# m1el/nemotron-speech.cpp

Measured on NVIDIA B200. Metric: rtfx, higher is better.
Workload: dtype bf16

## Files before the change

include/nsb200.h:

```cpp
#ifndef NSB200_H
#define NSB200_H

#include <stddef.h>
#include <stdint.h>

#ifdef __cplusplus
extern "C" {
#endif

#define NSB_OK 0
#define NSB_ERR_ARG (-1)
#define NSB_ERR_IO (-2)
#define NSB_ERR_FORMAT (-3)
#define NSB_ERR_CUDA (-4)
#define NSB_ERR_STATE (-5)
#define NSB_ERR_NOMEM (-6)

enum nsb_compute {
    NSB_COMPUTE_AUTO = 0,
    NSB_COMPUTE_F32 = 1,
    NSB_COMPUTE_F16 = 2,
    NSB_COMPUTE_BF16 = 3,
    NSB_COMPUTE_Q8_0 = 4,
    NSB_COMPUTE_Q8_0_STRICT = 5
// ... 22 lines not shown
} nsb_stats;

typedef struct nsb_model_info {
    int32_t n_mels, d_model, n_heads, d_head, d_ff, n_layers, kernel_size, vocab_size, decoder_dim, joint_dim;
    int32_t n_tensors;
    int32_t weight_type;
    char vocab[1025 * 8];
} nsb_model_info;
int nsb_gguf_probe(const char* gguf_path, nsb_model_info* info);
long long nsb_gguf_read_tensor(const char* gguf_path, const char* tensor_name, float* out, size_t cap_floats, int* ggml_type);

void nsb_default_config(nsb_engine_config* cfg);
int nsb_engine_create(const char* gguf_path, const nsb_engine_config* cfg, nsb_engine** out);
void nsb_engine_destroy(nsb_engine* e);
const char* nsb_last_error(void);

int nsb_engine_n_layers(const nsb_engine* e);
int nsb_engine_vocab_size(const nsb_engine* e);
const char* nsb_engine_vocab(const nsb_engine* e);
int nsb_engine_chunk_samples(const nsb_engine* e);
int nsb_engine_shift_samples(const nsb_engine* e);
int nsb_engine_compute(const nsb_engine* e);
int nsb_engine_set_cuda_graph(nsb_engine* e, int on);

int nsb_stream_open(nsb_engine* e);
int nsb_stream_close(nsb_engine* e, int stream);
int nsb_stream_reset(nsb_engine* e, int stream);

int nsb_stream_push_pcm(nsb_engine* e, int stream, const int16_t* pcm, int n_samples);
int nsb_push_pcm_batch(nsb_engine* e, int n_streams, const int32_t* streams, const int16_t* pcm, int row_stride, int n_samples);
int nsb_pop_tokens_batch(nsb_engine* e, int n_streams, const int32_t* streams, int32_t* out, int cap_per_stream, int32_t* counts);
int nsb_stream_ready(const nsb_engine* e, int stream);
int nsb_engine_step(nsb_engine* e);
int nsb_engine_step_begin(nsb_engine* e);
int nsb_engine_step_end(nsb_engine* e);
int nsb_engine_drain(nsb_engine* e);
int nsb_stream_pop_tokens(nsb_engine* e, int stream, int32_t* out, int cap);
int nsb_stream_chunks(const nsb_engine* e, int stream);

int nsb_detokenize(const nsb_engine* e, const int32_t* tokens, int n, char* out, int cap);

void nsb_engine_get_stats(const nsb_engine* e, nsb_stats* out);

int nsb_bench_prepare(nsb_engine* e, int n_streams, const int16_t* pcm, int samples_per_stream, int warm_chunks);
int nsb_bench_step(nsb_engine* e, float* ms);
int nsb_bench_steps(nsb_engine* e, int n, float* ms_each, float* total_ms);
#define NSB_PROFILE_CLASSES 8
int nsb_bench_profile(nsb_engine* e, float* ms_per_class, int* launches_per_class, float* total_ms);

int nsb_bench_gemm(nsb_engine* e, int kind, int rows, int bn, int stages, int splits, int rotate, int iters, float* us);

typedef struct nsb_trace_record { uint64_t t[6]; int32_t tag; int32_t grid; } nsb_trace_record;
int nsb_trace_enable(nsb_engine* e, int capacity);
int nsb_trace_fetch(nsb_engine* e, nsb_trace_record* out, int cap);

int nsb_profiler_range(int on);

int nsb_debug_enable(nsb_engine* e, int on);
int nsb_debug_get(nsb_engine* e, const char* name, float* out, size_t cap_floats);
int nsb_debug_get_cache(nsb_engine* e, int stream, int which , int layer, float* out, size_t cap);

int nsb_op_logmel(nsb_engine* e, const int16_t* pcm, int n_streams, int n_samples, float* mel_out, size_t cap_floats);
int nsb_op_gemm(nsb_engine* e, const char* weight_name, const float* x, int rows, float* y, size_t cap_floats);

enum nsb_epi { NSB_EPI_NONE = 0, NSB_EPI_RELU = 1, NSB_EPI_SILU = 2, NSB_EPI_RESID = 3, NSB_EPI_PARTIAL = 4 };
enum nsb_out_type { NSB_OUT_F32 = 0, NSB_OUT_F16 = 1, NSB_OUT_BF16 = 2 };
typedef struct nsb_gemm_op {
    const char* weight;
    int32_t rows;
    int32_t epi;
    float alpha;
    int32_t out_type;
    int32_t splits;
    int32_t c0;
    int32_t c_group, c_drop;
    int32_t force_bn, force_stages;
    int32_t rotate;
    const float* bias;
    const float* c_init;
} nsb_gemm_op;
int nsb_op_gemm_ex(nsb_engine* e, const nsb_gemm_op* op, const float* x, void* y, size_t y_bytes, long long* guard_bad);
int nsb_op_layernorm(nsb_engine* e, const float* x, int rows, const float* planes, int n_planes, float alpha, const float* g1, const float* b1,
                     const float* g2, const float* b2, int fused, int out_type, float* x_out, void* y);

int nsb_transcribe_full(nsb_engine* e, const int16_t* pcm, int n_samples, int32_t* tokens, int32_t* token_frames, int cap, int* n_frames,
                        float* enc_out, size_t enc_cap_floats);

#ifdef __cplusplus
}
#endif
#endif
```

nemotron-speech.cpp_b200/__init__.py:

```python
from __future__ import annotations

import ctypes as C
import os
import subprocess

import numpy as np

_DIR = os.path.dirname(os.path.abspath(__file__))
LIB_PATH = os.path.join(_DIR, "libnsb200.so")

EPI_NONE, EPI_RELU, EPI_SILU, EPI_RESID, EPI_PARTIAL = 0, 1, 2, 3, 4
OUT_F32, OUT_F16, OUT_BF16 = 0, 1, 2
COMPUTE_AUTO, COMPUTE_F32, COMPUTE_F16, COMPUTE_BF16, COMPUTE_Q8_0, COMPUTE_Q8_0_STRICT = 0, 1, 2, 3, 4, 5
KV_F32, KV_F16, KV_BF16 = 0, 1, 2


class NsbError(RuntimeError):
    pass


class EngineConfig(C.Structure):
    _fields_ = [("device", C.c_int32), ("compute", C.c_int32), ("kv_dtype", C.c_int32), ("att_right_context", C.c_int32),
                ("max_streams", C.c_int32), ("use_cuda_graph", C.c_int32), ("decode_overlap", C.c_int32), ("reserved", C.c_int32 * 5)]


class Stats(C.Structure):
    _fields_ = [("steps", C.c_int64), ("chunks", C.c_int64), ("kernel_launches", C.c_int64), ("device_ms", C.c_double),
                ("last_step_ms", C.c_double)]


class TraceRecord(C.Structure):
    _fields_ = [("t", C.c_uint64 * 6), ("tag", C.c_int32), ("grid", C.c_int32)]


TRACE_TAGS = {1: "logmel", 2: "stem", 3: "dwconv", 4: "melhist", 5: "gemm_f32", 6: "gemm_tc", 7: "gemm_q8", 8: "ln", 9: "ln2", 10: "attn",
              11: "convmod", 12: "advance", 13: "decode", 14: "other"}


class GemmOp(C.Structure):
    _fields_ = [("weight", C.c_char_p), ("rows", C.c_int32), ("epi", C.c_int32), ("alpha", C.c_float), ("out_type", C.c_int32),
                ("splits", C.c_int32), ("c0", C.c_int32), ("c_group", C.c_int32), ("c_drop", C.c_int32), ("force_bn", C.c_int32),
                ("force_stages", C.c_int32), ("rotate", C.c_int32), ("bias", C.c_void_p), ("c_init", C.c_void_p)]


class ModelInfo(C.Structure):
    _fields_ = [(n, C.c_int32) for n in ("n_mels", "d_model", "n_heads", "d_head", "d_ff", "n_layers", "kernel_size", "vocab_size",
                                         "decoder_dim", "joint_dim", "n_tensors", "weight_type")] + [("vocab", C.c_char * (1025 * 8))]


EXPORTS = ["nsb_gguf_probe", "nsb_gguf_read_tensor", "nsb_default_config", "nsb_engine_create", "nsb_engine_destroy", "nsb_last_error", "nsb_engine_n_layers",
           "nsb_engine_vocab_size", "nsb_engine_vocab", "nsb_engine_chunk_samples", "nsb_engine_shift_samples", "nsb_engine_compute", "nsb_engine_set_cuda_graph",
           "nsb_stream_open", "nsb_stream_close", "nsb_stream_reset", "nsb_stream_push_pcm", "nsb_push_pcm_batch", "nsb_pop_tokens_batch", "nsb_stream_ready", "nsb_engine_step", "nsb_engine_step_begin", "nsb_engine_step_end",
           "nsb_engine_drain", "nsb_stream_pop_tokens", "nsb_stream_chunks", "nsb_detokenize", "nsb_engine_get_stats",
           "nsb_bench_prepare", "nsb_bench_step", "nsb_bench_steps", "nsb_bench_profile", "nsb_profiler_range", "nsb_bench_gemm", "nsb_trace_enable", "nsb_trace_fetch", "nsb_debug_enable", "nsb_debug_get", "nsb_debug_get_cache", "nsb_op_logmel",
           "nsb_op_gemm", "nsb_op_gemm_ex", "nsb_op_layernorm", "nsb_transcribe_full"]


def build(force: bool = False) -> str:
    if force or not os.path.exists(LIB_PATH):
        subprocess.check_call(["make", "-C", _DIR, "-j8", "all"], stdout=subprocess.DEVNULL)
    return LIB_PATH


_lib = None
_f32p = np.ctypeslib.ndpointer(dtype=np.float32, flags="C_CONTIGUOUS")
_i16p = np.ctypeslib.ndpointer(dtype=np.int16, flags="C_CONTIGUOUS")
_i32p = np.ctypeslib.ndpointer(dtype=np.int32, flags="C_CONTIGUOUS")


def lib():
    global _lib
    if _lib is None:
        if not os.path.exists(LIB_PATH):
            raise NsbError(f"{LIB_PATH} is missing: run __graft_entry__.build() (there is no fallback path)")
        L = C.CDLL(LIB_PATH)
        vp, ci = C.c_void_p, C.c_int
        L.nsb_last_error.restype = C.c_char_p
        L.nsb_gguf_probe.argtypes = [C.c_char_p, C.POINTER(ModelInfo)]
        L.nsb_gguf_read_tensor.argtypes = [C.c_char_p, C.c_char_p, C.c_void_p, C.c_size_t, C.POINTER(C.c_int)]
        L.nsb_gguf_read_tensor.restype = C.c_longlong
        L.nsb_default_config.argtypes = [C.POINTER(EngineConfig)]
        L.nsb_engine_create.argtypes = [C.c_char_p, C.POINTER(EngineConfig), C.POINTER(vp)]
        L.nsb_engine_destroy.argtypes = [vp]
        for n in ("nsb_engine_n_layers", "nsb_engine_vocab_size", "nsb_engine_chunk_samples", "nsb_engine_shift_samples",
                  "nsb_engine_compute", "nsb_stream_open", "nsb_engine_step", "nsb_engine_step_begin", "nsb_engine_step_end", "nsb_engine_drain"):
            getattr(L, n).argtypes = [vp]
        L.nsb_engine_vocab.argtypes = [vp]
        L.nsb_engine_set_cuda_graph.argtypes = [vp, ci]
        L.nsb_engine_vocab.restype = vp
        for n in ("nsb_stream_close", "nsb_stream_reset", "nsb_stream_ready", "nsb_stream_chunks"):
            getattr(L, n).argtypes = [vp, ci]
        L.nsb_stream_push_pcm.argtypes = [vp, ci, _i16p, ci]
        L.nsb_stream_pop_tokens.argtypes = [vp, ci, _i32p, ci]
        L.nsb_push_pcm_batch.argtypes = [vp, ci, _i32p, _i16p, ci, ci]
        L.nsb_pop_tokens_batch.argtypes = [vp, ci, _i32p, _i32p, ci, _i32p]
        L.nsb_detokenize.argtypes = [vp, _i32p, ci, C.c_char_p, ci]
        L.nsb_engine_get_stats.argtypes = [vp, C.POINTER(Stats)]
        L.nsb_bench_prepare.argtypes = [vp, ci, _i16p, ci, ci]
        L.nsb_bench_step.argtypes = [vp, C.POINTER(C.c_float)]
        L.nsb_bench_steps.argtypes = [vp, ci, C.POINTER(C.c_float), C.POINTER(C.c_float)]
        L.nsb_bench_profile.argtypes = [vp, C.POINTER(C.c_float), C.POINTER(C.c_int), C.POINTER(C.c_float)]
        L.nsb_profiler_range.argtypes = [ci]
        L.nsb_trace_enable.argtypes = [vp, ci]
        L.nsb_trace_fetch.argtypes = [vp, C.POINTER(TraceRecord), ci]
        L.nsb_bench_gemm.argtypes = [vp, ci, ci, ci, ci, ci, ci, ci, C.POINTER(C.c_float)]
        L.nsb_debug_enable.argtypes = [vp, ci]
        L.nsb_debug_get.argtypes = [vp, C.c_char_p, _f32p, C.c_size_t]
        L.nsb_debug_get_cache.argtypes = [vp, ci, ci, ci, _f32p, C.c_size_t]
        L.nsb_op_logmel.argtypes = [vp, _i16p, ci, ci, _f32p, C.c_size_t]
        L.nsb_op_gemm.argtypes = [vp, C.c_char_p, _f32p, ci, _f32p, C.c_size_t]
        L.nsb_op_gemm_ex.argtypes = [vp, C.POINTER(GemmOp), _f32p, vp, C.c_size_t, C.POINTER(C.c_longlong)]
        L.nsb_op_layernorm.argtypes = [vp, _f32p, ci, vp, ci, C.c_float, _f32p, _f32p, vp, vp, ci, ci, _f32p, vp]
        L.nsb_transcribe_full.argtypes = [vp, _i16p, ci, _i32p, _i32p, ci, C.POINTER(C.c_int), C.c_void_p, C.c_size_t]
        _lib = L
    return _lib


def _check(rc: int) -> int:
    if rc < 0:
        raise NsbError(f"nsb error {rc}: {lib().nsb_last_error().decode(errors='replace')}")
    return rc


def probe(path: str) -> ModelInfo:
    info = ModelInfo()
    _check(lib().nsb_gguf_probe(path.encode(), C.byref(info)))
    return info


def read_tensor(path: str, name: str):
    t = C.c_int(0)
    n = _check(int(lib().nsb_gguf_read_tensor(path.encode(), name.encode(), None, 0, C.byref(t))))
    out = np.empty(n, dtype=np.float32)
    _check(int(lib().nsb_gguf_read_tensor(path.encode(), name.encode(), out.ctypes.data_as(C.c_void_p), out.size, C.byref(t))))
    return out, t.value


class Engine:

    def __init__(self, gguf_path: str, right_context: int = 0, max_streams: int = 1, compute: int = COMPUTE_AUTO,
                 kv_dtype: int = KV_F32, device: int = 0, cuda_graph: bool = True, decode_overlap: int = 0):
        cfg = EngineConfig()
        lib().nsb_default_config(C.byref(cfg))
        cfg.device, cfg.compute, cfg.kv_dtype = device, compute, kv_dtype
        cfg.att_right_context, cfg.max_streams = right_context, max_streams
        cfg.use_cuda_graph = 1 if cuda_graph else 0
        cfg.decode_overlap = decode_overlap
        h = C.c_void_p()
        _check(lib().nsb_engine_create(gguf_path.encode(), C.byref(cfg), C.byref(h)))
        self.h = h
        self.T = 1 + right_context
        self.max_streams = max_streams
        self.n_layers = lib().nsb_engine_n_layers(h)
        self.chunk_samples = lib().nsb_engine_chunk_samples(h)
        self.shift_samples = lib().nsb_engine_shift_samples(h)
        self.compute = lib().nsb_engine_compute(h)

    def close(self):
        if getattr(self, "h", None):
            lib().nsb_engine_destroy(self.h)
            self.h = None

    __del__ = close

    def set_cuda_graph(self, on: bool):
        _check(lib().nsb_engine_set_cuda_graph(self.h, 1 if on else 0))

    def open_stream(self) -> int:
        return _check(lib().nsb_stream_open(self.h))

    def close_stream(self, s: int):
        _check(lib().nsb_stream_close(self.h, s))

    def reset_stream(self, s: int):
        _check(lib().nsb_stream_reset(self.h, s))

    def push(self, s: int, pcm: np.ndarray):
        pcm = np.ascontiguousarray(pcm, dtype=np.int16)
        if len(pcm):
            _check(lib().nsb_stream_push_pcm(self.h, s, pcm, len(pcm)))

    def push_batch(self, streams, pcm: np.ndarray):
        ids = np.ascontiguousarray(streams, dtype=np.int32)
        pcm = np.ascontiguousarray(pcm, dtype=np.int16)
        assert pcm.ndim == 2 and pcm.shape[0] == len(ids)
        if pcm.shape[1]:
            _check(lib().nsb_push_pcm_batch(self.h, len(ids), ids, pcm.reshape(-1), pcm.shape[1], pcm.shape[1]))

    def pop_tokens_batch(self, streams, cap_per_stream: int = 256):
        ids = np.ascontiguousarray(streams, dtype=np.int32)
        out = np.empty((len(ids), cap_per_stream), dtype=np.int32)
        cnt = np.empty(len(ids), dtype=np.int32)
        _check(lib().nsb_pop_tokens_batch(self.h, len(ids), ids, out.reshape(-1), cap_per_stream, cnt))
        return out, cnt

# ... 69 lines not shown

    def trace_fetch(self, cap: int = 4096):
        buf = (TraceRecord * cap)()
        n = _check(lib().nsb_trace_fetch(self.h, buf, cap))
        return [(TRACE_TAGS.get(buf[i].tag, str(buf[i].tag)), buf[i].grid, [int(x) for x in buf[i].t]) for i in range(n)]

    def debug_enable(self, on: bool = True):
        _check(lib().nsb_debug_enable(self.h, 1 if on else 0))

    def debug_get(self, name: str, B: int) -> np.ndarray:
        rows = self.max_streams * self.T
        if name == "mel":
            M = 9 + 8 * self.T
            buf = np.empty(self.max_streams * M * 128, dtype=np.float32)
            _check(lib().nsb_debug_get(self.h, name.encode(), buf, buf.size))
            return buf.reshape(self.max_streams, M, 128)[:B].copy()
        if name == "logits":
            buf = np.empty((11 * self.T) * 1025, dtype=np.float32)
            n = _check(lib().nsb_debug_get(self.h, name.encode(), buf, buf.size))
            return buf[:n].reshape(-1, 1025).copy()
        buf = np.empty(rows * 1024, dtype=np.float32)
        _check(lib().nsb_debug_get(self.h, name.encode(), buf, buf.size))
        return buf.reshape(rows, 1024)[: B * self.T].copy()

    def debug_cache(self, stream: int, which: int, layer: int) -> np.ndarray:
        rows = 70 if which < 2 else 8
        buf = np.empty(rows * 1024, dtype=np.float32)
        _check(lib().nsb_debug_get_cache(self.h, stream, which, layer, buf, buf.size))
        return buf.reshape(rows, 1024)

    def op_logmel(self, pcm: np.ndarray) -> np.ndarray:
        pcm = np.ascontiguousarray(pcm, dtype=np.int16)
        if pcm.ndim == 1:
            pcm = pcm[None]
        ns, n = pcm.shape
        nf = (256 + n - 512 + 160) // 160 if 256 + n >= 512 else 0
        out = np.empty((ns, max(nf, 1), 128), dtype=np.float32)
        got = _check(lib().nsb_op_logmel(self.h, pcm.reshape(-1), ns, n, out.reshape(-1), out.size))
        assert got == nf, (got, nf)
        return out[:, :nf]

    def op_gemm(self, weight_name: str, x: np.ndarray) -> np.ndarray:
        x = np.ascontiguousarray(x, dtype=np.float32)
        y = np.empty((x.shape[0], 4096), dtype=np.float32)
        n_out = _check(lib().nsb_op_gemm(self.h, weight_name.encode(), x, x.shape[0], y.reshape(-1), y.size))
        return y.reshape(-1)[: x.shape[0] * n_out].reshape(x.shape[0], n_out).copy()

    def op_gemm_ex(self, weight_name: str, x: np.ndarray, *, epi: int = EPI_NONE, alpha: float = 1.0, bias=None, out_type: int = OUT_F32,
                   splits: int = 1, c0: bool = False, c_group: int = 0, c_drop: int = 0, force_bn: int = 0, force_stages: int = 0,
                   rotate: int = 1, c_init=None):
        x = np.ascontiguousarray(x, dtype=np.float32)
        rows = x.shape[0]
        m_out = rows // c_group * (c_group - c_drop) if c_group else rows
        keep = []
        def ptr(a):
            if a is None:
                return None
            a = np.ascontiguousarray(a, dtype=np.float32); keep.append(a)
            return a.ctypes.data_as(C.c_void_p)
        op = GemmOp(weight_name.encode(), rows, epi, alpha, out_type, splits, int(c0), c_group, c_drop, force_bn, force_stages, rotate,
                    ptr(bias), ptr(c_init))
        n_cap = 4096
        shape = (splits, m_out, n_cap) if epi == EPI_PARTIAL else (m_out, n_cap)
        y = np.empty(shape, dtype=np.float32 if out_type == OUT_F32 else np.uint16)
        bad = C.c_longlong(-1)
        n = _check(lib().nsb_op_gemm_ex(self.h, C.byref(op), x, y.ctypes.data_as(C.c_void_p), y.nbytes, C.byref(bad)))
        y = y.reshape(-1)[: int(np.prod(shape[:-1])) * n].reshape(shape[:-1] + (n,)).copy()
        return y, bad.value

    def op_layernorm(self, x: np.ndarray, g1, b1, *, planes=None, alpha: float = 1.0, fused: bool = False, g2=None, b2=None,
                     out_type: int = OUT_F32):
        x = np.ascontiguousarray(x, dtype=np.float32)
        rows = x.shape[0]
        f = lambda a: None if a is None else np.ascontiguousarray(a, dtype=np.float32)
        planes, g1, b1, g2, b2 = f(planes), f(g1), f(b1), f(g2), f(b2)
        vp = lambda a: None if a is None else a.ctypes.data_as(C.c_void_p)
        x_out = np.empty_like(x)
        y = np.zeros((rows, 1024), dtype=np.float32 if out_type == OUT_F32 else np.uint16)
        n_planes = 0 if planes is None else planes.shape[0]
        _check(lib().nsb_op_layernorm(self.h, x, rows, vp(planes), n_planes, alpha, g1, b1, vp(g2), vp(b2), int(fused), out_type, x_out,
                                      y.ctypes.data_as(C.c_void_p)))
        return x_out, y

    def transcribe_full(self, pcm: np.ndarray, want_enc: bool = True, want_frames: bool = False):
        pcm = np.ascontiguousarray(pcm, dtype=np.int16)
        frames_cap = len(pcm) // 1280 + 8
        toks = np.empty(10 * frames_cap, dtype=np.int32)
        frm = np.empty(10 * frames_cap, dtype=np.int32)
        enc = np.empty((frames_cap, 1024), dtype=np.float32) if want_enc else None
        nf = C.c_int(0)
        n = _check(lib().nsb_transcribe_full(self.h, pcm, len(pcm), toks, frm, len(toks), C.byref(nf),
                                             enc.ctypes.data_as(C.c_void_p) if want_enc else None, enc.size if want_enc else 0))
        out = (toks[:n].copy(), (enc[:nf.value].copy() if want_enc else None))
        return out + (frm[:n].copy(),) if want_frames else out
```

nemotron-speech.cpp_b200/csrc/c_api.cu:

```cuda
#include <algorithm>
#include <cstring>
#include <string>

#include <cuda_profiler_api.h>

#include "engine.h"

using nsb::Engine;

struct nsb_engine { Engine* impl; };

static thread_local std::string g_err;
static int fail(int code, const std::string& msg) { g_err = msg; return code; }

#define NSB_TRY try {
#define NSB_CATCH                                                                         \
    } catch (const nsb::CudaError& e) { return fail(NSB_ERR_CUDA, e.what());              \
    } catch (const std::invalid_argument& e) { return fail(NSB_ERR_ARG, e.what());        \
    } catch (const std::bad_alloc&) { return fail(NSB_ERR_NOMEM, "out of host memory");   \
    } catch (const std::exception& e) { return fail(NSB_ERR_STATE, e.what()); }

extern "C" {

const char* nsb_last_error(void) { return g_err.c_str(); }
// ... 66 lines not shown

int nsb_engine_n_layers(const nsb_engine* e) { return e ? e->impl->n_layers : NSB_ERR_ARG; }
int nsb_engine_vocab_size(const nsb_engine* e) { return e ? nsb::VOCAB : NSB_ERR_ARG; }
const char* nsb_engine_vocab(const nsb_engine* e) { return e ? e->impl->vocab.data() : nullptr; }
int nsb_engine_chunk_samples(const nsb_engine* e) { return e ? e->impl->chunk_samples() : NSB_ERR_ARG; }
int nsb_engine_shift_samples(const nsb_engine* e) { return e ? e->impl->shift_samples() : NSB_ERR_ARG; }
int nsb_engine_compute(const nsb_engine* e) { return e ? e->impl->compute : NSB_ERR_ARG; }

int nsb_engine_set_cuda_graph(nsb_engine* e, int on) { if (!e) return fail(NSB_ERR_ARG, "null engine"); NSB_TRY e->impl->set_cuda_graph(on != 0); return NSB_OK; NSB_CATCH }

int nsb_stream_open(nsb_engine* e) { if (!e) return fail(NSB_ERR_ARG, "null engine"); NSB_TRY return e->impl->open_stream(); NSB_CATCH }
int nsb_stream_close(nsb_engine* e, int s) { if (!e) return fail(NSB_ERR_ARG, "null engine"); NSB_TRY e->impl->close_stream(s); return NSB_OK; NSB_CATCH }
int nsb_stream_reset(nsb_engine* e, int s) { if (!e) return fail(NSB_ERR_ARG, "null engine"); NSB_TRY e->impl->reset_stream(s); return NSB_OK; NSB_CATCH }
int nsb_stream_push_pcm(nsb_engine* e, int s, const int16_t* pcm, int n) {
    if (!e) return fail(NSB_ERR_ARG, "null engine"); NSB_TRY e->impl->push_pcm(s, pcm, n); return NSB_OK; NSB_CATCH }
int nsb_push_pcm_batch(nsb_engine* e, int n_streams, const int32_t* streams, const int16_t* pcm, int row_stride, int n_samples) {
    if (!e || !streams || (!pcm && n_samples > 0) || n_streams < 0) return fail(NSB_ERR_ARG, "bad argument");
    NSB_TRY for (int i = 0; i < n_streams; ++i) e->impl->push_pcm(streams[i], pcm + (size_t)i * row_stride, n_samples); return NSB_OK; NSB_CATCH }
int nsb_pop_tokens_batch(nsb_engine* e, int n_streams, const int32_t* streams, int32_t* out, int cap_per_stream, int32_t* counts) {
    if (!e || !streams || !out || !counts || cap_per_stream < 0) return fail(NSB_ERR_ARG, "bad argument");
    NSB_TRY int total = 0;
    for (int i = 0; i < n_streams; ++i) { counts[i] = e->impl->pop_tokens(streams[i], out + (size_t)i * cap_per_stream, cap_per_stream); total += counts[i]; }
    return total; NSB_CATCH }
int nsb_stream_ready(const nsb_engine* e, int s) { if (!e || s < 0 || s >= e->impl->max_streams) return NSB_ERR_ARG; return e->impl->ready(s) ? 1 : 0; }
int nsb_engine_step(nsb_engine* e) { if (!e) return fail(NSB_ERR_ARG, "null engine"); NSB_TRY return e->impl->step(); NSB_CATCH }
int nsb_engine_step_begin(nsb_engine* e) { if (!e) return fail(NSB_ERR_ARG, "null engine"); NSB_TRY return e->impl->step_begin(); NSB_CATCH }
int nsb_engine_step_end(nsb_engine* e) { if (!e) return fail(NSB_ERR_ARG, "null engine"); NSB_TRY return e->impl->step_end(); NSB_CATCH }
int nsb_engine_drain(nsb_engine* e) {
    if (!e) return fail(NSB_ERR_ARG, "null engine");
    NSB_TRY int total = 0; for (;;) { int n = e->impl->step(); if (n <= 0) break; total += n; } return total; NSB_CATCH }
int nsb_stream_pop_tokens(nsb_engine* e, int s, int32_t* out, int cap) {
    if (!e || !out || cap < 0) return fail(NSB_ERR_ARG, "bad argument"); NSB_TRY return e->impl->pop_tokens(s, out, cap); NSB_CATCH }
int nsb_stream_chunks(const nsb_engine* e, int s) { if (!e) return NSB_ERR_ARG; NSB_TRY return e->impl->chunks(s); NSB_CATCH }

int nsb_detokenize(const nsb_engine* e, const int32_t* t, int n, char* out, int cap) {
    if (!e || (!t && n > 0) || !out) return fail(NSB_ERR_ARG, "bad argument");
    NSB_TRY const std::string r = e->impl->detok(t, n);
    if ((int)r.size() + 1 > cap) return -(int)r.size() - 1;
    memcpy(out, r.c_str(), r.size() + 1); return (int)r.size(); NSB_CATCH }

void nsb_engine_get_stats(const nsb_engine* e, nsb_stats* out) { if (e && out) *out = e->impl->stats; }

int nsb_bench_prepare(nsb_engine* e, int n, const int16_t* pcm, int sps, int warm) {
    if (!e || !pcm) return fail(NSB_ERR_ARG, "bad argument"); NSB_TRY e->impl->bench_prepare(n, pcm, sps, warm); return NSB_OK; NSB_CATCH }
int nsb_bench_step(nsb_engine* e, float* ms) {
    if (!e) return fail(NSB_ERR_ARG, "null engine"); NSB_TRY const float t = e->impl->bench_step(); if (ms) *ms = t; return NSB_OK; NSB_CATCH }

int nsb_bench_steps(nsb_engine* e, int n, float* ms_each, float* total_ms) {
    if (!e) return fail(NSB_ERR_ARG, "null engine"); NSB_TRY const float t = e->impl->bench_steps(n, ms_each); if (total_ms) *total_ms = t; return NSB_OK; NSB_CATCH }

int nsb_bench_profile(nsb_engine* e, float* ms_per_class, int* launches_per_class, float* total_ms) {
    if (!e || !ms_per_class || !launches_per_class) return fail(NSB_ERR_ARG, "bad argument");
    NSB_TRY const float t = e->impl->bench_profile(ms_per_class, launches_per_class); if (total_ms) *total_ms = t; return NSB_OK; NSB_CATCH }

int nsb_bench_gemm(nsb_engine* e, int kind, int rows, int bn, int stages, int splits, int rotate, int iters, float* us) {
    if (!e || !us) return fail(NSB_ERR_ARG, "bad argument"); NSB_TRY *us = e->impl->bench_gemm(kind, rows, bn, stages, splits, rotate, iters); return NSB_OK; NSB_CATCH }

int nsb_trace_enable(nsb_engine* e, int capacity) { if (!e) return fail(NSB_ERR_ARG, "null engine"); NSB_TRY e->impl->trace_enable(capacity); return NSB_OK; NSB_CATCH }
int nsb_trace_fetch(nsb_engine* e, nsb_trace_record* out, int cap) {
    if (!e || (!out && cap > 0)) return fail(NSB_ERR_ARG, "bad argument");
    static_assert(sizeof(nsb_trace_record) == sizeof(nsb::TraceRec), "trace record layout");
    NSB_TRY return e->impl->trace_fetch(reinterpret_cast<nsb::TraceRec*>(out), cap); NSB_CATCH }

int nsb_profiler_range(int on) { return (on ? cudaProfilerStart() : cudaProfilerStop()) == cudaSuccess ? NSB_OK : NSB_ERR_CUDA; }

int nsb_debug_enable(nsb_engine* e, int on) { if (!e) return fail(NSB_ERR_ARG, "null engine"); NSB_TRY e->impl->debug_enable(on != 0); return NSB_OK; NSB_CATCH }
int nsb_debug_get(nsb_engine* e, const char* name, float* out, size_t cap) {
    if (!e || !name || !out) return fail(NSB_ERR_ARG, "bad argument"); NSB_TRY return (int)e->impl->debug_get(name, out, cap); NSB_CATCH }
int nsb_debug_get_cache(nsb_engine* e, int s, int which, int layer, float* out, size_t cap) {
    if (!e || !out) return fail(NSB_ERR_ARG, "bad argument"); NSB_TRY return (int)e->impl->debug_get_cache(s, which, layer, out, cap); NSB_CATCH }

int nsb_op_logmel(nsb_engine* e, const int16_t* pcm, int ns, int n, float* out, size_t cap) {
    if (!e || !pcm || !out) return fail(NSB_ERR_ARG, "bad argument"); NSB_TRY return (int)e->impl->op_logmel(pcm, ns, n, out, cap); NSB_CATCH }
int nsb_op_gemm(nsb_engine* e, const char* name, const float* x, int rows, float* y, size_t cap) {
    if (!e || !name || !x || !y) return fail(NSB_ERR_ARG, "bad argument"); NSB_TRY return (int)e->impl->op_gemm(name, x, rows, y, cap); NSB_CATCH }

int nsb_op_gemm_ex(nsb_engine* e, const nsb_gemm_op* op, const float* x, void* y, size_t y_bytes, long long* guard_bad) {
    if (!e || !op || !op->weight || !x || !y) return fail(NSB_ERR_ARG, "bad argument");
    NSB_TRY return (int)e->impl->op_gemm_ex(*op, x, y, y_bytes, guard_bad); NSB_CATCH }
int nsb_op_layernorm(nsb_engine* e, const float* x, int rows, const float* planes, int n_planes, float alpha, const float* g1, const float* b1,
                     const float* g2, const float* b2, int fused, int out_type, float* x_out, void* y) {
    if (!e || !x || !x_out || !y) return fail(NSB_ERR_ARG, "bad argument");
    NSB_TRY e->impl->op_layernorm(x, rows, planes, n_planes, alpha, g1, b1, g2, b2, fused != 0, out_type, x_out, y); return NSB_OK; NSB_CATCH }

int nsb_transcribe_full(nsb_engine* e, const int16_t* pcm, int n, int32_t* tokens, int32_t* token_frames, int cap, int* n_frames, float* enc_out, size_t enc_cap) {
    if (!e || !pcm) return fail(NSB_ERR_ARG, "bad argument"); NSB_TRY return (int)e->impl->transcribe_full(pcm, n, tokens, token_frames, cap, n_frames, enc_out, enc_cap); NSB_CATCH }

}
```

nemotron-speech.cpp_b200/csrc/common.cuh:

```cuda
#pragma once
#include <cuda_bf16.h>
#include <cuda_fp16.h>
#include <cuda_runtime.h>

#include <atomic>
#include <cstdint>
#include <cstdio>
#include <stdexcept>
#include <string>
#include <utility>

namespace nsb {

constexpr int D_MODEL = 1024, D_FF = 4096, N_HEADS = 8, D_HEAD = 128;
constexpr int N_MELS = 128, N_FFT = 512, N_BINS = 257, HOP = 160, WIN = 400;
constexpr int ATT_L = 70;
constexpr int CONV_K = 9;
constexpr int PRE_CACHE = 9;
constexpr int DROP_PRE = 2;
constexpr int SUB_CH = 256, SUB_W = 17;
constexpr int HID = 640, JOINT = 640, VOCAB = 1025, BLANK = 1024;
constexpr int MAX_SYMBOLS = 10;

struct CudaError : std::runtime_error { using std::runtime_error::runtime_error; };

#define NSB_CUDA(expr)                                                                              \
    do {                                                                                            \
        cudaError_t _e = (expr);                                                                    \
        if (_e != cudaSuccess)                                                                      \
            throw ::nsb::CudaError(std::string(#expr) + ": " + cudaGetErrorString(_e) + " (" + __FILE__ + ":" + \
                                   std::to_string(__LINE__) + ")");                                 \
    } while (0)

__device__ __forceinline__ void pdl_wait() { asm volatile("griddepcontrol.wait;" ::: "memory"); }
__device__ __forceinline__ void pdl_trigger() { asm volatile("griddepcontrol.launch_dependents;" ::: "memory"); }

bool pdl_enabled();
inline bool& pdl_skip_flag() { static thread_local bool f = false; return f; }
inline void pdl_skip_next() { pdl_skip_flag() = true; }
inline bool pdl_take() { bool& f = pdl_skip_flag(); const bool on = pdl_enabled() && !f; f = false; return on; }

template <typename... P, typename... A>
inline void launch_k(void (*kern)(P...), dim3 grid, dim3 block, size_t smem, cudaStream_t st, A&&... args) {
    cudaLaunchConfig_t cfg{};
    cfg.gridDim = grid; cfg.blockDim = block; cfg.dynamicSmemBytes = smem; cfg.stream = st;
    cudaLaunchAttribute at[1];
    at[0].id = cudaLaunchAttributeProgrammaticStreamSerialization;
    at[0].val.programmaticStreamSerializationAllowed = 1;
    cfg.attrs = at; cfg.numAttrs = pdl_take() ? 1 : 0;
    NSB_CUDA(cudaLaunchKernelEx(&cfg, kern, P(std::forward<A>(args))...));
}

template <typename... P, typename... A>
inline void launch_k_cluster(void (*kern)(P...), dim3 grid, dim3 block, size_t smem, cudaStream_t st, int cluster_x, A&&... args) {
    cudaLaunchConfig_t cfg{};
    cfg.gridDim = grid; cfg.blockDim = block; cfg.dynamicSmemBytes = smem; cfg.stream = st;
    cudaLaunchAttribute at[2]; int n = 0;
    if (cluster_x > 1) { at[n].id = cudaLaunchAttributeClusterDimension; at[n].val.clusterDim.x = cluster_x; at[n].val.clusterDim.y = 1; at[n].val.clusterDim.z = 1; ++n; }
    if (pdl_take()) { at[n].id = cudaLaunchAttributeProgrammaticStreamSerialization; at[n].val.programmaticStreamSerializationAllowed = 1; ++n; }
    cfg.attrs = at; cfg.numAttrs = n;
    NSB_CUDA(cudaLaunchKernelEx(&cfg, kern, P(std::forward<A>(args))...));
}

constexpr int MAX_DEVICES = 64;
template <typename K>
inline void ensure_dyn_smem(K kern, size_t bytes, std::atomic<size_t>* slots, bool max_carveout = false) {
    int dev = 0;
    NSB_CUDA(cudaGetDevice(&dev));
    std::atomic<size_t>& done = slots[dev & (MAX_DEVICES - 1)];
    if (bytes <= done.load(std::memory_order_acquire)) return;
    NSB_CUDA(cudaFuncSetAttribute(kern, cudaFuncAttributeMaxDynamicSharedMemorySize, (int)bytes));
    if (max_carveout) NSB_CUDA(cudaFuncSetAttribute(kern, cudaFuncAttributePreferredSharedMemoryCarveout, (int)cudaSharedmemCarveoutMaxShared));
    done.store(bytes, std::memory_order_release);
}

struct TraceRec { unsigned long long t[6]; int tag; int grid; };
struct TraceBuf { unsigned n; unsigned cap; unsigned pad[2]; TraceRec rec[1]; };
enum TraceTag : int { TR_LOGMEL = 1, TR_STEM, TR_DWCONV, TR_MELHIST, TR_GEMM_SIMT, TR_GEMM_TC, TR_GEMM_Q8, TR_LN, TR_LN2, TR_ATTN, TR_CONVMOD, TR_ADVANCE, TR_DECODE, TR_OTHER };
static __constant__ TraceBuf* c_trace;
#define NSB_DEFINE_TRACE_BINDER(name) \
    void name(TraceBuf* p) { NSB_CUDA(cudaMemcpyToSymbol(c_trace, &p, sizeof(p))); }
__device__ __forceinline__ unsigned long long gtime() { unsigned long long t; asm volatile("mov.u64 %0, %%globaltimer;" : "=l"(t)); return t; }
__device__ __forceinline__ bool trace_thread() { return threadIdx.x == 0 && (blockIdx.x | blockIdx.y | blockIdx.z) == 0; }
__device__ __forceinline__ int trace_begin(int tag) {
    TraceBuf* tb = c_trace;
    if (!tb) return -1;
    const unsigned s = atomicAdd(&tb->n, 1u);
    if (s >= tb->cap) return -1;
    tb->rec[s].tag = tag; tb->rec[s].grid = (int)(gridDim.x * gridDim.y * gridDim.z); tb->rec[s].t[0] = gtime();
    return (int)s;
}
__device__ __forceinline__ void trace_mark(int slot, int i) { if (slot >= 0) c_trace->rec[slot].t[i] = gtime(); }
#define NSB_KERNEL_BEGIN(tag)                                      \
    int tr_slot = -1;                                              \
    if (trace_thread()) tr_slot = trace_begin(tag);
#define NSB_KERNEL_WAIT()                                          \
    pdl_wait(); pdl_trigger();                                     \
    if (tr_slot >= 0) trace_mark(tr_slot, 1);
#define NSB_KERNEL_PROLOGUE(tag) NSB_KERNEL_BEGIN(tag) NSB_KERNEL_WAIT()
#define NSB_KERNEL_EPILOGUE() do { if (tr_slot >= 0) trace_mark(tr_slot, 2); } while (0)

enum Epi : int {
    EPI_NONE = 0,
    EPI_RELU = 1,
    EPI_SILU = 2,
    EPI_RESID = 3,
    EPI_PARTIAL = 4
};
enum OutType : int { OUT_F32 = 0, OUT_F16 = 1, OUT_BF16 = 2 };

__device__ __forceinline__ float silu_f(float x) { return __fdividef(x, 1.0f + __expf(-x)); }
__device__ __forceinline__ float silu_exact(float x) { return x / (1.0f + expf(-x)); }
__device__ __forceinline__ float sigmoid_exact(float x) { return 1.0f / (1.0f + expf(-x)); }

__device__ __forceinline__ float warp_sum(float v) {
#pragma unroll
    for (int o = 16; o > 0; o >>= 1) v += __shfl_xor_sync(0xffffffffu, v, o);
    return v;
}
__device__ __forceinline__ float warp_max(float v) {
#pragma unroll
    for (int o = 16; o > 0; o >>= 1) v = fmaxf(v, __shfl_xor_sync(0xffffffffu, v, o));
    return v;
}

template <typename T> __device__ __forceinline__ T from_f32(float v);
template <> __device__ __forceinline__ float from_f32<float>(float v) { return v; }
template <> __device__ __forceinline__ __half from_f32<__half>(float v) { return __float2half_rn(v); }
template <> __device__ __forceinline__ __nv_bfloat16 from_f32<__nv_bfloat16>(float v) { return __float2bfloat16_rn(v); }
__device__ __forceinline__ float to_f32(float v) { return v; }
__device__ __forceinline__ float to_f32(__half v) { return __half2float(v); }
__device__ __forceinline__ float to_f32(__nv_bfloat16 v) { return __bfloat162float(v); }

__device__ __forceinline__ void store_out(void* p, size_t i, float v, int ot) {
    if (ot == OUT_F32) ((float*)p)[i] = v;
    else if (ot == OUT_F16) ((__half*)p)[i] = __float2half_rn(v);
    else ((__nv_bfloat16*)p)[i] = __float2bfloat16_rn(v);
}
__device__ __forceinline__ float load_kv(const void* p, size_t i, int kv) {
    if (kv == 0) return ((const float*)p)[i];
    if (kv == 1) return __half2float(((const __half*)p)[i]);
    return __bfloat162float(((const __nv_bfloat16*)p)[i]);
}
__device__ __forceinline__ float round_kv(float v, int kv) {
    if (kv == 0) return v;
    if (kv == 1) return __half2float(__float2half_rn(v));
    return __bfloat162float(__float2bfloat16_rn(v));
}
__device__ __forceinline__ void store_kv(void* p, size_t i, float v, int kv) {
    if (kv == 0) ((float*)p)[i] = v;
    else if (kv == 1) ((__half*)p)[i] = __float2half_rn(v);
    else ((__nv_bfloat16*)p)[i] = __float2bfloat16_rn(v);
}
__device__ __forceinline__ float to_tf32(float v) { uint32_t r; asm("cvt.rna.tf32.f32 %0, %1;" : "=r"(r) : "f"(v)); return __uint_as_float(r); }
__device__ __forceinline__ void split_tf32(float v, float& hi, float& lo) { hi = to_tf32(v); lo = to_tf32(v - hi); }
__device__ __forceinline__ void store_pixel(float* out, size_t pix, int c, float v, int split) {
    if (!split) { out[pix * 256 + c] = v; return; }
    float hi, lo; split_tf32(v, hi, lo);
    out[pix * 512 + c] = hi; out[pix * 512 + 256 + c] = lo;
}
inline size_t kv_elem_size(int kv) { return kv == 0 ? 4 : 2; }
// ... 4 lines not shown
```

nemotron-speech.cpp_b200/csrc/engine.cu:

```cuda
#include "engine.h"

#include <algorithm>
#include <cmath>
#include <cstddef>
#include <cstdlib>
#include <cstring>

namespace nsb {

void launch_gemm_tc(const GemmArgs& a, int in_type , cudaStream_t st);

constexpr int MAX_SPLITS = 8;
constexpr size_t SPLIT_CONSUMER_MAX_ROWS = 256;

bool tf32x3_enabled() {
    static const bool on = [] { const char* e = getenv("NSB_STEM_TF32"); return !(e && e[0] == '1'); }();
    return on;
}
bool pdl_enabled() {
    static const bool on = [] { const char* e = getenv("NSB_NO_PDL"); return !(e && e[0] == '1'); }();
    return on;
}

namespace {
// ... 348 lines not shown
        mat(L.ff1b, "feed_forward1.linear2.weight", D_MODEL, D_FF);
        mat(L.ff2a, "feed_forward2.linear1.weight", D_FF, D_MODEL);
        mat(L.ff2b, "feed_forward2.linear2.weight", D_MODEL, D_FF);
        load_layer_matrix(L.qkv, g, p + "self_attn.linear_qkv.weight",
                          {p + "self_attn.linear_q.weight", p + "self_attn.linear_k.weight", p + "self_attn.linear_v.weight"}, 3 * D_MODEL, D_MODEL);
        mat(L.out, "self_attn.linear_out.weight", D_MODEL, D_MODEL);
        mat(L.pw1, "conv.pointwise_conv1.weight", 2 * D_MODEL, D_MODEL);
        mat(L.pw2, "conv.pointwise_conv2.weight", D_MODEL, D_MODEL);
        vec(L.bias_u, p + "self_attn.pos_bias_u", D_MODEL); vec(L.bias_v, p + "self_attn.pos_bias_v", D_MODEL);
        {
            const GgufTensor& dw = g.require(p + "conv.depthwise_conv.weight");
            if (dw.ne.size() != 2 || dw.ne[0] != D_MODEL || dw.ne[1] != CONV_K)
                throw std::runtime_error("depthwise conv weight must be [1024, 9] (2-D, tap-major; reconvert old 3-D files)");
            vec(L.dw_w, p + "conv.depthwise_conv.weight", (size_t)CONV_K * D_MODEL);
        }
        vec(L.cln_g, p + "conv.batch_norm.weight", D_MODEL); vec(L.cln_b, p + "conv.batch_norm.bias", D_MODEL);
        for (Weight* w : {&L.ff1a, &L.ff1b, &L.ff2a, &L.ff2b, &L.qkv, &L.out, &L.pw1, &L.pw2}) named_[w->name] = w;
        { int k = 0; for (Weight* w : {&L.ff1a, &L.ff1b, &L.qkv, &L.out, &L.pw1, &L.pw2, &L.ff2a, &L.ff2b}) w->shadow_slot = k++; }
    }
    {
        const std::string d = "decoder.prediction.";
        vec(embed_, d + "embed.weight", (size_t)VOCAB * HID);
        for (int l = 0; l < 2; ++l) {
            vec(lstm_w_[2 * l], d + "dec_rnn.lstm.weight_ih_l" + std::to_string(l), (size_t)4 * HID * HID);
            vec(lstm_w_[2 * l + 1], d + "dec_rnn.lstm.weight_hh_l" + std::to_string(l), (size_t)4 * HID * HID);
            vec(lstm_b_[2 * l], d + "dec_rnn.lstm.bias_ih_l" + std::to_string(l), (size_t)4 * HID);
            vec(lstm_b_[2 * l + 1], d + "dec_rnn.lstm.bias_hh_l" + std::to_string(l), (size_t)4 * HID);
        }
        f32_weight(joint_enc_w_, "joint.enc.weight", JOINT, D_MODEL, g.read_f32("joint.enc.weight"));
        vec(joint_enc_b_, "joint.enc.bias", JOINT);
        vec(pred_w_, "joint.pred.weight", (size_t)JOINT * HID); vec(pred_b_, "joint.pred.bias", JOINT);
        vec(jout_w_, "joint.joint_net.2.weight", (size_t)VOCAB * JOINT); vec(jout_b_, "joint.joint_net.2.bias", VOCAB);
    }
}

int q8_dense_min_rows();
void Engine::alloc_state() {
    const int S = max_streams, Cap = ATT_L + T, M = PRE_CACHE + 8 * T;
    const int t1 = M / 2 + 1, t2 = t1 / 2 + 1, t3 = t2 / 2 + 1;
    if (t3 != T + DROP_PRE) throw std::runtime_error("unexpected subsampling length");
    const size_t SS = (size_t)S + 1;
    kv_.alloc(SS * n_layers * 2 * Cap * D_MODEL * kv_elem_size(kv_dtype));
    conv_cache_.alloc(SS * 2 * n_layers * (CONV_K - 1) * D_MODEL * 4); cc_par_.alloc(SS * 4);
    mel_hist_.alloc(SS * PRE_CACHE * N_MELS * 4);
    ring_pos_.alloc(SS * 4); valid_len_.alloc(SS * 4);
    dec_h_.alloc(SS * 4 * HID * 4); dec_c_.alloc(SS * 4 * HID * 4);
    dec_proj_.alloc(SS * JOINT * 4);
    prev_token_.alloc(SS * 4); cand_valid_.alloc(SS * 4); dec_par_.alloc(SS * 4);
    hs_.assign(S, HostStream());
    for (int s = 0; s <= S; ++s) zero_slot(s);

    rl_ = hs_row_len(T);
    const size_t Mrows = (size_t)S * T;
    ensure_q8s_scratch((int)std::max<size_t>(Mrows, ATT_L + 2 * T));
    for (StepIO& io : io_) io.d_pcm.alloc((size_t)S * rl_ * 2);
    d_slot_.alloc((size_t)S * 4);
    mel_new_.alloc((size_t)S * 8 * T * N_MELS * 4);
    const size_t sp = (!strict() && tf32x3_enabled()) ? 2 : 1;
    dw_.alloc(sp * S * t2 * 33 * SUB_CH * 4);
    pw_.alloc((size_t)S * t2 * 33 * SUB_CH * 4);
    if (sp == 2) a3_.alloc(std::max((size_t)S * t3 * SUB_W * SUB_CH, (size_t)S * T * D_MODEL) * 2 * 4, false);
    x_.alloc(Mrows * D_MODEL * 4);
    a_.alloc(Mrows * D_MODEL * act_size());
    big_.alloc(Mrows * D_FF * act_size());
    const size_t planes = Mrows <= SPLIT_CONSUMER_MAX_ROWS ? 4 : 1;
    consumer_planes_ = (int)planes;
    if (compute == NSB_COMPUTE_Q8_0) wscratch_.alloc((size_t)D_FF * D_MODEL * 2, false);
    if (compute == NSB_COMPUTE_Q8_0 && (int)Mrows >= q8_dense_min_rows()) {
        const size_t sz[8] = {(size_t)D_FF * D_MODEL, (size_t)D_MODEL * D_FF, (size_t)3 * D_MODEL * D_MODEL, (size_t)D_MODEL * D_MODEL,
                              (size_t)2 * D_MODEL * D_MODEL, (size_t)D_MODEL * D_MODEL, (size_t)D_FF * D_MODEL, (size_t)D_MODEL * D_FF};
        size_t off = 0; for (int k = 0; k < 8; ++k) { shadow_off_[k] = off; off += sz[k] * 2; }
        shadow_bytes_ = off;
        for (DevBuf& b : shadow_) b.alloc(off, false);
        NSB_CUDA(cudaStreamCreateWithFlags(&st_deq_, cudaStreamNonBlocking));
        ev_deq_.resize(n_layers); ev_lstart_.resize(n_layers + 1);
        for (cudaEvent_t& e : ev_deq_) NSB_CUDA(cudaEventCreateWithFlags(&e, cudaEventDisableTiming));
        for (cudaEvent_t& e : ev_lstart_) NSB_CUDA(cudaEventCreateWithFlags(&e, cudaEventDisableTiming));
    }
    qkv_.alloc(planes * Mrows * 3 * D_MODEL * 4);
    pw1_.alloc(planes * Mrows * 2 * D_MODEL * 4);
    encp_.alloc(Mrows * JOINT * 4);
    part_.alloc((size_t)MAX_SPLITS * std::min<size_t>(Mrows, 1024) * D_MODEL * 4);
    out_tok_.alloc((size_t)S * MAX_SYMBOLS * T * 4); out_cnt_.alloc((size_t)S * 4);
    dec_sync_.alloc(decode_sync_bytes(S));
    for (Side& sd : side_) {
        sd.slot.alloc((size_t)S * 4); sd.encp.alloc(Mrows * JOINT * 4); sd.out_tok.alloc((size_t)S * MAX_SYMBOLS * T * 4);
        sd.out_cnt.alloc((size_t)S * 4); sd.sync.alloc(decode_sync_bytes(S));
    }
    for (StepIO& io : io_) {
        io.h_pcm.alloc((size_t)S * rl_ * 2); io.h_slot.alloc((size_t)S * 4);
        io.h_tok.alloc((size_t)S * MAX_SYMBOLS * T * 4); io.h_cnt.alloc((size_t)S * 4);
    }
}

void Engine::zero_slot(int s) {
    NSB_CUDA(cudaSetDevice(device_));
    join_decode_stream();
    const int Cap = ATT_L + T;
    const size_t kvb = (size_t)n_layers * 2 * Cap * D_MODEL * kv_elem_size(kv_dtype);
    NSB_CUDA(cudaMemsetAsync((char*)kv_.p + (size_t)s * kvb, 0, kvb, st_));
    const size_t cb = (size_t)2 * n_layers * (CONV_K - 1) * D_MODEL * 4;
    NSB_CUDA(cudaMemsetAsync((char*)conv_cache_.p + (size_t)s * cb, 0, cb, st_));
    NSB_CUDA(cudaMemsetAsync((char*)cc_par_.p + (size_t)s * 4, 0, 4, st_));
    NSB_CUDA(cudaMemsetAsync((char*)mel_hist_.p + (size_t)s * PRE_CACHE * N_MELS * 4, 0, (size_t)PRE_CACHE * N_MELS * 4, st_));
    NSB_CUDA(cudaMemsetAsync((char*)dec_h_.p + (size_t)s * 4 * HID * 4, 0, (size_t)4 * HID * 4, st_));
    NSB_CUDA(cudaMemsetAsync((char*)dec_c_.p + (size_t)s * 4 * HID * 4, 0, (size_t)4 * HID * 4, st_));
    NSB_CUDA(cudaMemsetAsync((char*)dec_par_.p + (size_t)s * 4, 0, 4, st_));
    const int zero = 0, blank = BLANK;
    NSB_CUDA(cudaMemcpyAsync((char*)ring_pos_.p + (size_t)s * 4, &zero, 4, cudaMemcpyHostToDevice, st_));
    NSB_CUDA(cudaMemcpyAsync((char*)valid_len_.p + (size_t)s * 4, &zero, 4, cudaMemcpyHostToDevice, st_));
    NSB_CUDA(cudaMemcpyAsync((char*)cand_valid_.p + (size_t)s * 4, &zero, 4, cudaMemcpyHostToDevice, st_));
    NSB_CUDA(cudaMemcpyAsync((char*)prev_token_.p + (size_t)s * 4, &blank, 4, cudaMemcpyHostToDevice, st_));
    NSB_CUDA(cudaStreamSynchronize(st_));
    if (s < max_streams) hs_clear(hs_[s]);
}

void Engine::build_pos_tables(const GgufFile& g) {
    const int n_rel = ATT_L + 2 * T - 1;
    std::vector<float> tab((size_t)n_rel * D_MODEL);
    for (int r = 0; r < n_rel; ++r) pos_emb_row(r - (T - 1), &tab[(size_t)r * D_MODEL]);
    DevBuf d_tab; upload(d_tab, tab);
    DevBuf d_a; const void* A = d_tab.p;
    if (act_type() != OUT_F32) { d_a.alloc(tab.size() * 2, false); convert_to(d_tab.as<float>(), d_a.p, tab.size(), act_type(), st_); A = d_a.p; }
    for (int l = 0; l < n_layers; ++l) {
        const std::string n = "encoder.layers." + std::to_string(l) + ".self_attn.linear_pos.weight";
        Weight wpos; load_layer_matrix(wpos, g, n, {n}, D_MODEL, D_MODEL);
        layers_[l].pos_proj.alloc((size_t)n_rel * D_MODEL * kv_elem_size(kv_dtype), false);
        if (kv_dtype == 0) gemm(A, D_MODEL, wpos, n_rel, nullptr, layers_[l].pos_proj.p, D_MODEL, EPI_NONE, 1.f, OUT_F32);
        else {
            DevBuf tmp; tmp.alloc((size_t)n_rel * D_MODEL * 4, false);
            gemm(A, D_MODEL, wpos, n_rel, nullptr, tmp.p, D_MODEL, EPI_NONE, 1.f, OUT_F32);
            convert_to(tmp.as<float>(), layers_[l].pos_proj.p, (size_t)n_rel * D_MODEL, kv_dtype == 1 ? OUT_F16 : OUT_BF16, st_);
            NSB_CUDA(cudaStreamSynchronize(st_));
        }
        NSB_CUDA(cudaStreamSynchronize(st_));
    }
}

void Engine::gemm(const void* A, long long lda, const Weight& W, int M, const float* bias, void* C, long long ldc, int epi, float alpha,
                  int out_type) {
    GemmArgs a; a.A = A; a.lda = lda; a.M = M; a.bias = bias; a.C = C; a.ldc = ldc;
    a.epi = epi; a.alpha = alpha; a.out_type = out_type; a.pair = 1;
    gemm(a, W);
}

void Engine::gemm(GemmArgs& a, const Weight& W) {
    a.W = W.data.p; a.w_scales = W.scales.p; a.q4 = W.q4; a.N = W.n_out; a.K = W.n_in;
    ProfScope ps(this, PC_GEMM);
    if (cur_shadow_ && W.shadow_slot >= 0) { a.W = cur_shadow_ + shadow_off_[W.shadow_slot]; a.w_scales = nullptr; a.q4 = 0; }
    else q8_predequant(W, a.M, a);
    if (compute == NSB_COMPUTE_Q8_0_STRICT) { launch_gemm_q8_strict(a, q8s_scratch_.p, q8s_scratch_.bytes, st_); count_launch(); }
    else if (compute == NSB_COMPUTE_F32) launch_gemm_simt(a, st_);
    else launch_gemm_tc(a, act_type(), st_);
    count_launch();
}

void Engine::ensure_q8s_scratch(int rows) {
    if (compute != NSB_COMPUTE_Q8_0_STRICT) return;
    const size_t need = q8_strict_scratch_bytes(rows, D_FF);
    if (q8s_scratch_.bytes < need) { NSB_CUDA(cudaStreamSynchronize(st_)); q8s_scratch_.alloc(need, false); }
}

void Engine::gemm_f32w(GemmArgs& g, const Weight& W, bool a_presplit) {
    if (strict()) { launch_gemm_simt(g, st_); count_launch(); return; }
    if (W.scales.p) {
        const int K = W.n_in;
        if (!a_presplit) {
            if (g.lda != K || (size_t)g.M * 2 * K * 4 > a3_.bytes) throw std::runtime_error("gemm_f32w: split scratch too small / strided A");
            launch_split_tf32((const float*)g.A, a3_.as<float>(), (size_t)g.M, K, st_); count_launch();
            g.A = a3_.p;
        }
        g.lda = 2 * K; g.a_fold = K; g.K = 3 * K; g.W = W.scales.p;
    }
    launch_gemm_tc(g, OUT_F32, st_); count_launch();
}

int q8_dense_min_rows() {
    const char* e = getenv("NSB_Q8_PREDEQUANT_ROWS");
    return e ? atoi(e) : 1;
}
void Engine::q8_predequant(const Weight& W, int M, GemmArgs& a) {
    const int min_rows = q8_dense_min_rows();
    if (compute != NSB_COMPUTE_Q8_0 || !W.scales.p || M < min_rows) return;
    if (q8_pair256_enabled()) return;
    const size_t bytes = (size_t)W.n_out * W.n_in * 2;
    if (wscratch_.bytes < bytes) throw std::runtime_error("q8_predequant: scratch not allocated");
    launch_dequant_q8(W.data.p, W.scales.p, wscratch_.p, W.n_out, W.n_in, st_, W.q4);
    count_launch();
    a.W = wscratch_.p; a.w_scales = nullptr; a.w_dynamic = 1; a.pair = 0; a.q4 = 0;
}

bool Engine::shadow_mode(int rows) const {
    static const bool off = [] { const char* e = getenv("NSB_Q8_SHADOW"); return e && e[0] == '0'; }();
    const int min_rows = q8_dense_min_rows();
    return !off && !q8_pair256_enabled() && compute == NSB_COMPUTE_Q8_0 && shadow_bytes_ && rows >= min_rows && !profiling_;
}
void Engine::dequant_layer_async(int l, cudaStream_t s) {
    LayerW& L = layers_[l];
    char* base = shadow_[l & 1].as<char>();
    for (Weight* w : {&L.ff1a, &L.ff1b, &L.qkv, &L.out, &L.pw1, &L.pw2, &L.ff2a, &L.ff2b}) {
        launch_dequant_q8(w->data.p, w->scales.p, base + shadow_off_[w->shadow_slot], w->n_out, w->n_in, s, w->q4);
        count_launch();
    }
}

bool Engine::split_consumers(int rows) const {
    static const bool off = [] { const char* e = getenv("NSB_NO_SPLIT_CONSUMERS"); return e && e[0] == '1'; }();
    return !off && !pair_gemm_enabled() && consumer_planes_ >= 4 && (compute == NSB_COMPUTE_F16 || compute == NSB_COMPUTE_BF16) && rows <= 128;
}

void Engine::gemm_planes(const void* A, long long lda, const Weight& W, int M, void* C, int planes) {
    GemmArgs a; a.A = A; a.lda = lda; a.W = W.data.p; a.w_scales = W.scales.p; a.q4 = W.q4; a.M = M; a.N = W.n_out; a.K = W.n_in; a.C = C; a.ldc = W.n_out;
    a.epi = EPI_PARTIAL; a.out_type = OUT_F32; a.splits = planes; a.force_bn = 64; a.force_stages = 4;
    { ProfScope ps(this, PC_GEMM); launch_gemm_tc(a, act_type(), st_); }
    count_launch();
}

void Engine::gemm_residual(const void* A, long long lda, const Weight& W, int M, float* x, float alpha) {
    int splits = 1;
    if (!strict() && M <= 1024) {
        const int tiles = ((M + 127) / 128) * (W.n_out / (W.n_in >= 4096 ? 64 : 32));
        const int nk = W.n_in / 64;
        while (splits < MAX_SPLITS && tiles * splits < 120 && nk % (splits * 2) == 0 && nk / (splits * 2) >= 2) splits *= 2;
    }
    static const int big_split = [] { const char* e = getenv("NSB_FFDOWN_SPLIT"); return e ? atoi(e) : 2; }();
    if (!strict() && M > 1024 && W.n_in >= 4096 && big_split > 1 && (size_t)big_split * M * D_MODEL * 4 <= part_.bytes) splits = big_split;
    if (splits == 1) { gemm(A, lda, W, M, nullptr, x, D_MODEL, EPI_RESID, alpha, OUT_F32); return; }
    GemmArgs a; a.A = A; a.lda = lda; a.W = W.data.p; a.w_scales = W.scales.p; a.q4 = W.q4; a.M = M; a.N = W.n_out; a.K = W.n_in; a.C = part_.p; a.ldc = D_MODEL;
    a.epi = EPI_PARTIAL; a.out_type = OUT_F32; a.splits = splits;
    { ProfScope ps(this, PC_GEMM);
      if (cur_shadow_ && W.shadow_slot >= 0) { a.W = cur_shadow_ + shadow_off_[W.shadow_slot]; a.w_scales = nullptr; } else q8_predequant(W, M, a);
      launch_gemm_tc(a, act_type(), st_); }
    count_launch();
    pending_.part = part_.as<float>(); pending_.n = splits; pending_.alpha = alpha;
}

int Engine::open_stream() {
    collect_all();
    for (int s = 0; s < max_streams; ++s)
        if (!hs_[s].open) { zero_slot(s); hs_[s].open = true; return s; }
    throw std::runtime_error("no free stream slot (max_streams = " + std::to_string(max_streams) + ")");
}
void Engine::close_stream(int s) { collect_all(); if (s < 0 || s >= max_streams || !hs_[s].open) throw std::invalid_argument("bad stream id"); hs_release_pcm(hs_[s]); hs_[s].open = false; }
void Engine::reset_stream(int s) { collect_all(); if (s < 0 || s >= max_streams || !hs_[s].open) throw std::invalid_argument("bad stream id"); zero_slot(s); }

void Engine::push_pcm(int s, const int16_t* pcm, int n) {
    if (s < 0 || s >= max_streams || !hs_[s].open) throw std::invalid_argument("bad stream id");
    if (!pcm || n <= 0) return;
    hs_push(hs_[s], pcm, n);
}

bool Engine::ready(int s) const { return hs_ready(hs_[s], T); }

int Engine::step_begin() {
    if (n_inflight_ == MAX_INFLIGHT) throw std::runtime_error("step_begin: three steps are already in flight (call step_end)");
    NSB_CUDA(cudaSetDevice(device_));
    std::vector<int> batch;
    for (int s = 0; s < max_streams; ++s) if (ready(s)) batch.push_back(s);
    const int B = (int)batch.size();
    if (!B) return 0;
    StepIO& io = io_[io_next_];
    int16_t* hp = io.h_pcm.as<int16_t>(); int* hsl = io.h_slot.as<int>();
    for (int b = 0; b < B; ++b) {
        HostStream& h = hs_[batch[b]];
        hs_stage_row(h, T, rl_, hp + (size_t)b * rl_); hsl[b] = batch[b];
        hs_launched(h, T);
    }
    const int side = side_acquire();
    NSB_CUDA(cudaMemcpyAsync(io.d_pcm.p, hp, (size_t)B * rl_ * 2, cudaMemcpyHostToDevice, st_copy_));
    NSB_CUDA(cudaEventRecord(io.h2d, st_copy_));
    NSB_CUDA(cudaStreamWaitEvent(st_, io.h2d, 0));
    NSB_CUDA(cudaMemcpyAsync(side_[side].slot.p, hsl, (size_t)B * 4, cudaMemcpyHostToDevice, st_));
    NSB_CUDA(cudaEventRecord(io.ev0, st_));
    cudaStream_t tail = run_step(B, io.d_pcm.as<int16_t>(), side, n_inflight_ >= 1);
    NSB_CUDA(cudaEventRecord(io.ev1, tail));
    NSB_CUDA(cudaMemcpyAsync(io.h_cnt.p, side_[side].out_cnt.p, (size_t)B * 4, cudaMemcpyDeviceToHost, tail));
    NSB_CUDA(cudaMemcpyAsync(io.h_tok.p, side_[side].out_tok.p, (size_t)B * MAX_SYMBOLS * T * 4, cudaMemcpyDeviceToHost, tail));
    NSB_CUDA(cudaEventRecord(io.done, tail));
    if (tail != st_) { NSB_CUDA(cudaEventRecord(side_[side].dec_done, tail)); }
    io.batch = std::move(batch);
    io_next_ = (io_next_ + 1) % MAX_INFLIGHT; n_inflight_ += 1;
    return B;
}

int Engine::step_end() {
    if (n_inflight_ == 0) return 0;
    NSB_CUDA(cudaSetDevice(device_));
    StepIO& io = io_[(io_next_ + MAX_INFLIGHT - n_inflight_) % MAX_INFLIGHT];
    n_inflight_ -= 1;
    const int B = (int)io.batch.size();
    NSB_CUDA(cudaEventSynchronize(io.done));
    float ms = 0.f; NSB_CUDA(cudaEventElapsedTime(&ms, io.ev0, io.ev1));
    stats.steps += 1; stats.chunks += B; stats.device_ms += ms; stats.last_step_ms = ms;
    collect_tokens(io);
    io.batch.clear();
    return B;
}

void Engine::collect_all() { while (n_inflight_) step_end(); }

int Engine::step() {
    collect_all();
    const int B = step_begin();
    if (B) step_end();
    return B;
}

void Engine::collect_tokens(StepIO& io) {
    const int* cnt = io.h_cnt.as<int>(); const int* tok = io.h_tok.as<int>();
    const int B = (int)io.batch.size();
    for (int b = 0; b < B; ++b) {
        HostStream& h = hs_[io.batch[b]];
        for (int i = 0; i < cnt[b] && i < MAX_SYMBOLS * T; ++i) h.tokens.push_back(tok[(size_t)b * MAX_SYMBOLS * T + i]);
        h.chunks_done += 1;
    }
}

// ... 86 lines not shown
    cudaStream_t s = ov ? st_dec_ : st_;
    if (!(skip_mask() & 8u ))
        run_graphed(dec_graphs_, std::make_tuple(B, side, ov ? 1 : 0), s, [&] { run_decode_kernels(B, side, s, ov); });
    if (ov) { NSB_CUDA(cudaEventRecord(sd.dec_done, st_dec_)); sd.dec_pending = true; }
    side_next_ = (side + 1) % MAX_INFLIGHT;
    return s;
}

void Engine::run_encoder_kernels(int B, const int16_t* d_pcm, int side) {
    const unsigned skip = skip_mask();
    cur_shadow_ = nullptr;
    const int M = PRE_CACHE + 8 * T, t1 = M / 2 + 1, t2 = t1 / 2 + 1, t3 = t2 / 2 + 1;
    const int rows = B * T, at = act_type();
    const int* slot = side_[side].slot.as<int>();
    float* x = x_.as<float>();
    pending_ = PartialSum{};

    if (!(skip & SK_MEL)) { ProfScope ps(this, PC_MEL);
    launch_logmel(d_pcm, rl_, B, 8 * T, window_.as<float>(), cos_t_.as<float>(), sin_t_.as<float>(), fb_t_.as<float>(),
                  mel_new_.as<float>(), (size_t)8 * T * N_MELS, st_); }
    count_launch();
    if (debug_) { launch_mel_gather(mel_hist_.as<float>(), mel_new_.as<float>(), slot, B, T, dbg_mel_.as<float>(), st_); count_launch(); }
    const bool tc = !strict();
    const int split = tc && c3_w_.scales.p ? 1 : 0;
    if (!(skip & SK_SUB)) { ProfScope ps(this, PC_SUBSAMPLE);
    launch_stem_conv0_dw(mel_hist_.as<float>(), mel_new_.as<float>(), slot, B, T, c0_w_.as<float>(), c0_b_.as<float>(), c2_w_.as<float>(),
                         c2_b_.as<float>(), dw_.as<float>(), st_, split);
    launch_mel_hist_update(mel_hist_.as<float>(), mel_new_.as<float>(), slot, B, T, st_);
    count_launch(2);
    {
        GemmArgs g; g.A = dw_.p; g.lda = SUB_CH; g.W = c3_w_.data.p; g.M = B * t2 * 33; g.N = SUB_CH; g.K = SUB_CH; g.bias = c3_b_.as<float>();
        g.C = pw_.p; g.ldc = SUB_CH; g.epi = EPI_RELU; gemm_f32w(g, c3_w_, split);
    }
    launch_dwconv_s2(pw_.as<float>(), B, t2, 33, c5_w_.as<float>(), c5_b_.as<float>(), dw_.as<float>(), st_, split); count_launch();
    {
        GemmArgs g; g.A = dw_.p; g.lda = SUB_CH; g.W = c6_w_.data.p; g.M = B * t3 * SUB_W; g.N = SUB_CH; g.K = SUB_CH; g.bias = c6_b_.as<float>();
        g.C = pw_.p; g.ldc = SUB_CH; g.epi = EPI_RELU; gemm_f32w(g, c6_w_, split);
    }
    {
        GemmArgs g; g.W = sub_out_w_.data.p; g.N = D_MODEL; g.K = SUB_W * SUB_CH; g.bias = out_b_.as<float>(); g.ldc = D_MODEL; g.lda = SUB_W * SUB_CH;
        g.A = pw_.p;
        if (!tc) {
            g.group = T; g.group_stride = (long long)t3 * SUB_W * SUB_CH; g.row_off = DROP_PRE; g.M = rows; g.C = x; g.epi = EPI_NONE;
        } else {
            g.M = B * t3; g.c_group = t3; g.c_drop = DROP_PRE;
            constexpr int SUB_SPLITS = 8;
            if (rows <= 1024 && (size_t)(SUB_SPLITS - 1) * rows * D_MODEL * 4 <= part_.bytes) {
                g.splits = SUB_SPLITS; g.epi = EPI_PARTIAL; g.C0 = x; g.C = part_.p;
                pending_.part = part_.as<float>(); pending_.n = SUB_SPLITS - 1; pending_.alpha = 1.f;
            } else { g.C = x; g.epi = EPI_NONE; }
        }
        gemm_f32w(g, sub_out_w_, false);
    }
    }

    const long long kv_slot_stride = (long long)n_layers * 2 * (ATT_L + T) * D_MODEL;
    const long long cc_par_stride = (long long)n_layers * (CONV_K - 1) * D_MODEL, cc_slot_stride = 2 * cc_par_stride;
    auto ln = [&](const float* g_, const float* b_) {
        if (skip & SK_LN) { pending_ = PartialSum{}; return; }
        ProfScope ps(this, PC_LAYERNORM); launch_layernorm(x, rows, g_, b_, a_.p, at, pending_, st_); count_launch(); pending_ = PartialSum{};
    };
    const bool shadow = shadow_mode(rows);
    if (shadow) {
        NSB_CUDA(cudaEventRecord(ev_lstart_[n_layers], st_));
        NSB_CUDA(cudaStreamWaitEvent(st_deq_, ev_lstart_[n_layers], 0));
        pdl_skip_next(); dequant_layer_async(0, st_deq_);
        NSB_CUDA(cudaEventRecord(ev_deq_[0], st_deq_));
    }
    ln(layers_[0].ln[0].as<float>(), layers_[0].ln[1].as<float>());
    if (debug_) NSB_CUDA(cudaMemcpyAsync(dbg_sub_.p, x, (size_t)rows * D_MODEL * 4, cudaMemcpyDeviceToDevice, st_));
    for (int l = 0; l < n_layers; ++l) {
        LayerW& L = layers_[l];
        if (shadow) {
            NSB_CUDA(cudaEventRecord(ev_lstart_[l], st_));
            if (l + 1 < n_layers) {
                NSB_CUDA(cudaStreamWaitEvent(st_deq_, ev_lstart_[l], 0));
                pdl_skip_next(); dequant_layer_async(l + 1, st_deq_);
                NSB_CUDA(cudaEventRecord(ev_deq_[l + 1], st_deq_));
            }
            NSB_CUDA(cudaStreamWaitEvent(st_, ev_deq_[l], 0));
            cur_shadow_ = shadow_[l & 1].as<char>();
            pdl_skip_next();
        }
        if (!(skip & SK_FF)) {
        gemm(a_.p, D_MODEL, L.ff1a, rows, nullptr, big_.p, D_FF, EPI_SILU, 1.f, at);
        gemm_residual(big_.p, D_FF, L.ff1b, rows, x, 0.5f); }
        ln(L.ln[2].as<float>(), L.ln[3].as<float>());
        const int qkv_planes = split_consumers(rows) ? 2 : 1;
        const int pw1_planes = 1;
        if (!(skip & SK_QKV)) {
            if (qkv_planes == 1) gemm(a_.p, D_MODEL, L.qkv, rows, nullptr, qkv_.p, 3 * D_MODEL, EPI_NONE, 1.f, OUT_F32);
            else gemm_planes(a_.p, D_MODEL, L.qkv, rows, qkv_.p, qkv_planes);
        }
        if (!(skip & SK_ATTN)) {
            AttnArgs aa; aa.qkv = qkv_.as<float>(); aa.planes = qkv_planes; aa.plane_stride = (long long)rows * 3 * D_MODEL;
            const size_t es = kv_elem_size(kv_dtype);
            aa.k_ring = (char*)kv_.p + (size_t)l * 2 * (ATT_L + T) * D_MODEL * es;
            aa.v_ring = (char*)aa.k_ring + (size_t)(ATT_L + T) * D_MODEL * es;
            aa.slot_stride = kv_slot_stride; aa.kv_dtype = kv_dtype; aa.pos_proj = L.pos_proj.p;
            aa.bias_u = L.bias_u.as<float>(); aa.bias_v = L.bias_v.as<float>(); aa.ctx = a_.p; aa.out_type = at;
            aa.slot_of_b = slot; aa.ring_pos = ring_pos_.as<int>(); aa.valid_len = valid_len_.as<int>(); aa.B = B; aa.T = T;
            ProfScope ps(this, PC_ATTENTION); launch_attention(aa, st_); count_launch();
        }
        if (!(skip & SK_OUT)) gemm_residual(a_.p, D_MODEL, L.out, rows, x, 1.f);
        ln(L.ln[4].as<float>(), L.ln[5].as<float>());
        if (!(skip & SK_PW)) {
            if (pw1_planes == 1) gemm(a_.p, D_MODEL, L.pw1, rows, nullptr, pw1_.p, 2 * D_MODEL, EPI_NONE, 1.f, OUT_F32);
            else gemm_planes(a_.p, D_MODEL, L.pw1, rows, pw1_.p, pw1_planes);
        }
        if (!(skip & SK_CONV)) {
            ConvModArgs ca; ca.pw1 = pw1_.as<float>(); ca.planes = pw1_planes; ca.plane_stride = (long long)rows * 2 * D_MODEL; ca.conv_cache = conv_cache_.as<float>() + (size_t)l * (CONV_K - 1) * D_MODEL;
            ca.slot_stride = cc_slot_stride; ca.par_stride = cc_par_stride; ca.cc_par = cc_par_.as<int>();
            ca.dw_w = L.dw_w.as<float>(); ca.ln_g = L.cln_g.as<float>(); ca.ln_b = L.cln_b.as<float>();
            ca.out = a_.p; ca.out_type = at; ca.slot_of_b = slot; ca.B = B; ca.T = T;
            ProfScope ps(this, PC_CONVMOD); launch_conv_module(ca, st_); count_launch();
        }
        if (!(skip & SK_PW)) gemm_residual(a_.p, D_MODEL, L.pw2, rows, x, 1.f);
        ln(L.ln[6].as<float>(), L.ln[7].as<float>());
        if (!(skip & SK_FF)) {
        gemm(a_.p, D_MODEL, L.ff2a, rows, nullptr, big_.p, D_FF, EPI_SILU, 1.f, at);
        gemm_residual(big_.p, D_FF, L.ff2b, rows, x, 0.5f); }
        const bool last = l + 1 == n_layers;
        if (skip & SK_LN) pending_ = PartialSum{};
        else { ProfScope ps(this, PC_LAYERNORM);
          launch_layernorm2(x, rows, L.ln[8].as<float>(), L.ln[9].as<float>(), last ? nullptr : layers_[l + 1].ln[0].as<float>(),
                            last ? nullptr : layers_[l + 1].ln[1].as<float>(), last ? nullptr : a_.p, at, pending_, st_);
          count_launch(); pending_ = PartialSum{}; }
        if (debug_) NSB_CUDA(cudaMemcpyAsync(dbg_layers_.as<float>() + (size_t)l * dbg_B_ * T * D_MODEL, x, (size_t)rows * D_MODEL * 4,
                                             cudaMemcpyDeviceToDevice, st_));
    }
    cur_shadow_ = nullptr;
    { ProfScope ps(this, PC_MISC); launch_advance_streams(slot, B, T, ring_pos_.as<int>(), valid_len_.as<int>(), cc_par_.as<int>(), st_); count_launch(); }

    if (skip & SK_DECODE) return;
    ProfScope ps_dec(this, PC_DECODE);
    GemmArgs g; g.A = x; g.lda = D_MODEL; g.W = joint_enc_w_.data.p; g.M = rows; g.N = JOINT; g.K = D_MODEL; g.bias = joint_enc_b_.as<float>();
    g.C = side_[side].encp.p; g.ldc = JOINT; g.epi = EPI_NONE;
    constexpr int JS = 6;
    const bool jsplit = !strict() && joint_enc_w_.scales.p && rows <= 256 && (size_t)(JS - 1) * rows * JOINT * 4 <= part_.bytes;
    if (jsplit) { g.splits = JS; g.epi = EPI_PARTIAL; g.C0 = side_[side].encp.p; g.C = part_.p; }
    gemm_f32w(g, joint_enc_w_, false);
    if (jsplit) {
        const size_t n4 = (size_t)rows * JOINT / 4;
        launch_k(add_planes_kernel, dim3((unsigned)((n4 + 255) / 256)), dim3(256), 0, st_, side_[side].encp.as<float>(), part_.as<const float>(), JS - 1,
                 (size_t)rows * JOINT, n4);
        count_launch();
    }
}

void Engine::run_decode_kernels(int B, int side, cudaStream_t s, bool narrow) {
    ProfScope ps_dec(this, PC_DECODE);
    Side& sd = side_[side];
    DecodeArgs d{};
    d.w.embed = embed_.as<float>();
    for (int l = 0; l < 2; ++l) { d.w.w_ih[l] = lstm_w_[2 * l].as<float>(); d.w.w_hh[l] = lstm_w_[2 * l + 1].as<float>();
                                  d.w.b_ih[l] = lstm_b_[2 * l].as<float>(); d.w.b_hh[l] = lstm_b_[2 * l + 1].as<float>(); }
    d.w.pred_w = pred_w_.as<float>(); d.w.pred_b = pred_b_.as<float>(); d.w.out_w = jout_w_.as<float>(); d.w.out_b = jout_b_.as<float>();
    d.s.hbuf = dec_h_.as<float>(); d.s.cbuf = dec_c_.as<float>(); d.s.par = dec_par_.as<int>();
    d.s.dec_proj = dec_proj_.as<float>(); d.s.prev_token = prev_token_.as<int>(); d.s.cand_valid = cand_valid_.as<int>();
    d.enc_proj = sd.encp.as<float>(); d.slot_of_b = sd.slot.as<int>(); d.B = B; d.T = T;
    d.out_tokens = sd.out_tok.as<int>(); d.out_count = sd.out_cnt.as<int>();
    d.logits_tap = debug_ ? dbg_logits_.as<float>() : nullptr; d.logits_tap_cap = debug_ ? MAX_SYMBOLS * T + T : 0;
    d.logits_tap_n = debug_ ? dbg_logits_n_.as<int>() : nullptr;
    launch_decode(d, sd.sync.p, s, narrow ? decode_narrow_ctas() : 0); count_launch();
}

void Engine::bench_prepare(int n_streams, const int16_t* pcm, int samples_per_stream, int warm_chunks) {
    if (n_streams < 1 || n_streams > max_streams) throw std::invalid_argument("bench: n_streams out of range");
    const long long need_warm = warm_chunks > 0 ? (long long)HOP * (8LL * T * warm_chunks - 1) + N_FFT / 2 : 0;
    const long long need_all = (long long)HOP * (8LL * T * (warm_chunks + 1) - 1) + N_FFT / 2;
    if (samples_per_stream < need_all) throw std::invalid_argument("bench: need at least " + std::to_string(need_all) + " samples per stream");
    for (int s = 0; s < max_streams; ++s) if (hs_[s].open) hs_[s].open = false;
    std::vector<int> ids;
    for (int i = 0; i < n_streams; ++i) ids.push_back(open_stream());
    for (int i = 0; i < n_streams; ++i) if (need_warm) push_pcm(ids[i], pcm + (size_t)i * samples_per_stream, (int)need_warm);
    while (step() > 0) {}
    int n_chunks = 1;
    while (n_chunks < 16 && samples_per_stream >= (long long)HOP * (8LL * T * (warm_chunks + n_chunks + 1) - 1) + N_FFT / 2) ++n_chunks;
    const long long need_stage = (long long)HOP * (8LL * T * (warm_chunks + n_chunks) - 1) + N_FFT / 2;
    for (int i = 0; i < n_streams; ++i) push_pcm(ids[i], pcm + (size_t)i * samples_per_stream + need_warm, (int)(need_stage - need_warm));
    bench_pcm_.alloc((size_t)n_chunks * n_streams * rl_ * 2, false);
    int16_t* hp = io_[0].h_pcm.as<int16_t>(); int* hsl = io_[0].h_slot.as<int>();
    for (int k = 0; k < n_chunks; ++k) {
        for (int b = 0; b < n_streams; ++b) {
            HostStream& h = hs_[ids[b]];
            if (k == 0 && !ready(ids[b])) throw std::runtime_error("bench: stream not ready after staging");
            h.chunk_idx += k;
            hs_stage_row(h, T, rl_, hp + (size_t)b * rl_);
            h.chunk_idx -= k;
            hsl[b] = ids[b];
        }
        h2d_sync((char*)bench_pcm_.p + (size_t)k * n_streams * rl_ * 2, hp, (size_t)n_streams * rl_ * 2);
    }
    for (Side& sd : side_) h2d_sync(sd.slot.p, hsl, (size_t)n_streams * 4);
    bench_B_ = n_streams; bench_n_ = n_chunks; bench_i_ = 0;
}

const int16_t* Engine::bench_next_pcm() {
    const int16_t* p = bench_pcm_.as<int16_t>() + (size_t)(bench_i_ % bench_n_) * bench_B_ * rl_;
    bench_i_ += 1;
    return p;
}

float Engine::bench_step() {
    if (!bench_B_) throw std::runtime_error("bench_step before bench_prepare");
    collect_all();
    NSB_CUDA(cudaSetDevice(device_));
    NSB_CUDA(cudaEventRecord(ev0_, st_));
    cudaStream_t tail = run_step(bench_B_, bench_next_pcm(), side_acquire(), false);
    NSB_CUDA(cudaEventRecord(ev1_, tail));
// ... 344 lines not shown
        ln(L.ln[6].as<float>(), L.ln[7].as<float>());
        gemm(a_.p, D_MODEL, L.ff2a, rows, nullptr, big_.p, D_FF, EPI_SILU, 1.f, at);
        gemm_residual(big_.p, D_FF, L.ff2b, rows, x, 0.5f);
        const bool last = l + 1 == n_layers;
        launch_layernorm2(x, rows, L.ln[8].as<float>(), L.ln[9].as<float>(), last ? nullptr : layers_[l + 1].ln[0].as<float>(),
                          last ? nullptr : layers_[l + 1].ln[1].as<float>(), last ? nullptr : a_.p, at, pending_, st_);
        count_launch(); pending_ = PartialSum{};
    }

    {
        GemmArgs g; g.A = x; g.lda = D_MODEL; g.W = joint_enc_w_.data.p; g.M = rows; g.N = JOINT; g.K = D_MODEL; g.bias = joint_enc_b_.as<float>();
        g.C = encp_.p; g.ldc = JOINT; g.epi = EPI_NONE; gemm_f32w(g, joint_enc_w_, false);
    }
    DecodeArgs d{};
    d.w.embed = embed_.as<float>();
    for (int l = 0; l < 2; ++l) { d.w.w_ih[l] = lstm_w_[2 * l].as<float>(); d.w.w_hh[l] = lstm_w_[2 * l + 1].as<float>();
                                  d.w.b_ih[l] = lstm_b_[2 * l].as<float>(); d.w.b_hh[l] = lstm_b_[2 * l + 1].as<float>(); }
    d.w.pred_w = pred_w_.as<float>(); d.w.pred_b = pred_b_.as<float>(); d.w.out_w = jout_w_.as<float>(); d.w.out_b = jout_b_.as<float>();
    d.s.hbuf = dec_h_.as<float>(); d.s.cbuf = dec_c_.as<float>(); d.s.par = dec_par_.as<int>();
    d.s.dec_proj = dec_proj_.as<float>(); d.s.prev_token = prev_token_.as<int>(); d.s.cand_valid = cand_valid_.as<int>();
    d.enc_proj = encp_.as<float>(); d.slot_of_b = slot_dev; d.B = 1; d.T = rows;
    d.out_tokens = out_tok_.as<int>(); d.out_count = out_cnt_.as<int>(); d.out_frames = bw_.out_frm.as<int>();
    launch_decode(d, dec_sync_.p, st_); count_launch();
    NSB_CUDA(cudaStreamSynchronize(st_));

    int n_tok = 0;
    NSB_CUDA(cudaMemcpy(&n_tok, out_cnt_.p, 4, cudaMemcpyDeviceToHost));
    n_tok = std::max(0, std::min(n_tok, MAX_SYMBOLS * rows));
    if (std::min(n_tok, cap) > 0) NSB_CUDA(cudaMemcpy(tokens, out_tok_.p, (size_t)std::min(n_tok, cap) * 4, cudaMemcpyDeviceToHost));
    if (token_frames && std::min(n_tok, cap) > 0) NSB_CUDA(cudaMemcpy(token_frames, bw_.out_frm.p, (size_t)std::min(n_tok, cap) * 4, cudaMemcpyDeviceToHost));
    if (enc_out) NSB_CUDA(cudaMemcpy(enc_out, x, (size_t)rows * D_MODEL * 4, cudaMemcpyDeviceToHost));
    if (n_frames) *n_frames = rows;
    stats.chunks += 1;
    return n_tok;
}

const Weight& Engine::op_weight(const std::string& name) const {
    auto it = named_.find(name);
    if (it == named_.end()) throw std::invalid_argument("op_gemm: unknown weight '" + name + "'");
    return *it->second;
}
const void* Engine::op_operand(const Weight& W, const float* xh, int rows, DevBuf& dx, DevBuf& da) {
    dx.alloc((size_t)rows * W.n_in * 4, false);
    h2d_sync(dx.p, xh, dx.bytes);
    if (W.f32 || act_type() == OUT_F32) return dx.p;
    da.alloc((size_t)rows * W.n_in * 2, false);
    convert_to(dx.as<float>(), da.p, (size_t)rows * W.n_in, act_type(), st_);
    return da.p;
}
struct Engine::SplitScratch {
    Engine* e; DevBuf tmp; bool swapped = false;
    SplitScratch(Engine* e_, const Weight& W, int rows) : e(e_) {
        const size_t need = (size_t)rows * 2 * W.n_in * 4;
        if (!W.f32 || !W.scales.p || e->a3_.bytes >= need) return;
        tmp.alloc(need, false); std::swap(e->a3_, tmp); swapped = true;
    }
    ~SplitScratch() { if (swapped) { cudaStreamSynchronize(e->st_); std::swap(e->a3_, tmp); } }
};

long long Engine::op_gemm(const std::string& name, const float* xh, int rows, float* y, size_t cap) {
    const Weight& W = op_weight(name);
    NSB_CUDA(cudaSetDevice(device_));
    if (cap < (size_t)rows * W.n_out) return -(long long)((size_t)rows * W.n_out);
    ensure_q8s_scratch(rows);
    DevBuf dx, da, dy; dy.alloc((size_t)rows * W.n_out * 4, false);
    const void* A = op_operand(W, xh, rows, dx, da);
    if (W.f32) {
        SplitScratch sc(this, W, rows);
        GemmArgs g; g.A = A; g.lda = W.n_in; g.W = W.data.p; g.M = rows; g.N = W.n_out; g.K = W.n_in; g.C = dy.p; g.ldc = W.n_out; g.epi = EPI_NONE;
        gemm_f32w(g, W, false);
    } else gemm(A, W.n_in, W, rows, nullptr, dy.p, W.n_out, EPI_NONE, 1.f, OUT_F32);
    NSB_CUDA(cudaStreamSynchronize(st_));
    NSB_CUDA(cudaMemcpy(y, dy.p, dy.bytes, cudaMemcpyDeviceToHost));
    return W.n_out;
}

namespace {
constexpr int GUARD_ROWS = 128;
constexpr int GUARD_COLS = 32;
constexpr uint32_t GUARD_WORD = 0x7FDA7FDAu;

struct Guarded {
    DevBuf d; size_t es = 4, ld = 0, live = 0, cols = 0;
    void init(size_t live_rows, size_t n, size_t elem, const float* live_init) {
        es = elem; ld = n + GUARD_COLS; live = live_rows; cols = n;
        std::vector<uint8_t> h(bytes());
        for (size_t i = 0; i + 4 <= h.size(); i += 4) memcpy(&h[i], &GUARD_WORD, 4);
        if (live_init)
            for (size_t r = 0; r < live; ++r) memcpy(&h[((GUARD_ROWS + r) * ld) * es], live_init + r * n, n * 4);
        d.alloc(h.size(), false); h2d_sync(d.p, h.data(), h.size());
    }
    size_t bytes() const { return (2 * GUARD_ROWS + live) * ld * es; }
    void* at() const { return (char*)d.p + GUARD_ROWS * ld * es; }
    long long fetch(void* out) const {
        std::vector<uint8_t> h(bytes());
        NSB_CUDA(cudaMemcpy(h.data(), d.p, h.size(), cudaMemcpyDeviceToHost));
        long long bad = 0;
        for (size_t r = 0; r < 2 * GUARD_ROWS + live; ++r) {
            const bool live_row = r >= GUARD_ROWS && r < GUARD_ROWS + live;
            for (size_t c = live_row ? cols : 0; c < ld; ++c) bad += memcmp(&h[(r * ld + c) * es], &GUARD_WORD, es) != 0;
            if (live_row) memcpy((char*)out + (r - GUARD_ROWS) * cols * es, &h[r * ld * es], cols * es);
        }
        return bad;
    }
};
}

long long Engine::op_gemm_ex(const nsb_gemm_op& op, const float* xh, void* y, size_t y_bytes, long long* guard_bad) {
    const Weight& W = op_weight(op.weight);
    const int rows = op.rows, N = W.n_out;
    auto bad = [](const std::string& m) { throw std::invalid_argument("op_gemm_ex: " + m); };
    if (rows < 1) bad("rows must be >= 1");
    if (op.epi < EPI_NONE || op.epi > EPI_PARTIAL) bad("unknown epilogue");
    if (op.out_type < OUT_F32 || op.out_type > OUT_BF16) bad("unknown output type");
    if (op.out_type != OUT_F32 && (op.epi == EPI_RESID || op.epi == EPI_PARTIAL)) bad("residual and split-K outputs are f32");
    if (op.splits < 1 || op.splits > MAX_SPLITS || (op.splits > 1 && op.epi != EPI_PARTIAL)) bad("splits must be 1..8, > 1 only with the split-K epilogue");
    if (op.c0 && op.epi != EPI_PARTIAL) bad("c0 is a split-K destination");
    if (op.c_group < 0 || (op.c_group > 0 && (op.c_drop < 0 || op.c_drop >= op.c_group || rows % op.c_group != 0))) bad("bad output row map");
    if (op.epi == EPI_RESID && !op.c_init) bad("the residual epilogue needs c_init");
    if (strict() && (op.out_type != OUT_F32 || op.epi == EPI_PARTIAL || op.c_group || op.force_bn))
        bad("strict modes run the SIMT / Q8_0 block kernels: f32 output, no split-K, row map or tile config");
    NSB_CUDA(cudaSetDevice(device_));
    const int m_out = op.c_group > 0 ? rows / op.c_group * (op.c_group - op.c_drop) : rows;
    const bool partial = op.epi == EPI_PARTIAL;
    const size_t es = out_elem_size(op.out_type), need = partial ? (size_t)op.splits * m_out * N * 4 : (size_t)m_out * N * es;
    if (y_bytes < need) return -(long long)need;
    ensure_q8s_scratch(rows);
    DevBuf dx, da, dbias;
    const void* A = op_operand(W, xh, rows, dx, da);
    if (op.bias) { dbias.alloc((size_t)N * 4, false); h2d_sync(dbias.p, op.bias, dbias.bytes); }
    const int ws_planes = partial ? op.splits - (op.c0 ? 1 : 0) : 1;
    Guarded c, c0;
    c.init((size_t)ws_planes * m_out, N, partial ? 4 : es, op.epi == EPI_RESID ? op.c_init : nullptr);
    if (op.c0) c0.init(m_out, N, 4, nullptr);

    GemmArgs g; g.A = A; g.lda = W.n_in; g.W = W.data.p; g.M = rows; g.N = N; g.K = W.n_in; g.bias = op.bias ? dbias.as<float>() : nullptr;
    g.C = c.at(); g.ldc = (long long)c.ld; g.epi = op.epi; g.alpha = op.alpha; g.out_type = op.out_type; g.splits = op.splits;
    g.c_group = op.c_group; g.c_drop = op.c_drop; g.C0 = op.c0 ? c0.at() : nullptr; g.force_bn = op.force_bn; g.force_stages = op.force_stages;
    g.rotate = op.rotate; g.pair = 1;
    if (W.f32) { SplitScratch sc(this, W, rows); gemm_f32w(g, W, false); NSB_CUDA(cudaStreamSynchronize(st_)); }
    else gemm(g, W);
    NSB_CUDA(cudaStreamSynchronize(st_));
    long long nbad = 0;
    if (op.c0) nbad += c0.fetch(y);
    nbad += c.fetch((char*)y + (op.c0 ? (size_t)m_out * N * 4 : 0));
    if (guard_bad) *guard_bad = nbad;
    return N;
}

void Engine::op_layernorm(const float* xh, int rows, const float* planes, int n_planes, float alpha, const float* g1, const float* b1,
                          const float* g2, const float* b2, bool fused, int out_type, float* x_out, void* y) {
    if (rows < 1 || n_planes < 0 || n_planes > MAX_SPLITS || (n_planes && !planes) || !g1 || !b1 || (!g2) != (!b2) || (g2 && !fused))
        throw std::invalid_argument("op_layernorm: bad arguments (rows >= 1, 0..8 planes, g1 / b1, g2 / b2 together and only fused)");
    if (out_type < OUT_F32 || out_type > OUT_BF16) throw std::invalid_argument("op_layernorm: unknown output type");
    NSB_CUDA(cudaSetDevice(device_));
    const size_t n = (size_t)rows * D_MODEL;
    auto up = [](DevBuf& d, const float* h, size_t count) { d.alloc(count * 4, false); h2d_sync(d.p, h, count * 4); };
    DevBuf dx, dp, dg1, db1, dg2, db2, dy;
    up(dx, xh, n); up(dg1, g1, D_MODEL); up(db1, b1, D_MODEL);
    if (n_planes) up(dp, planes, (size_t)n_planes * n);
    if (g2) { up(dg2, g2, D_MODEL); up(db2, b2, D_MODEL); }
    dy.alloc(n * out_elem_size(out_type), false);
    PartialSum ps; ps.part = n_planes ? dp.as<float>() : nullptr; ps.n = n_planes; ps.alpha = alpha;
    if (!fused) launch_layernorm(dx.as<float>(), rows, dg1.as<float>(), db1.as<float>(), dy.p, out_type, ps, st_);
    else launch_layernorm2(dx.as<float>(), rows, dg1.as<float>(), db1.as<float>(), dg2.as<float>(), db2.as<float>(), g2 ? dy.p : nullptr,
                           out_type, ps, st_);
    NSB_CUDA(cudaStreamSynchronize(st_));
    NSB_CUDA(cudaMemcpy(x_out, dx.p, n * 4, cudaMemcpyDeviceToHost));
    if (y && (!fused || g2)) NSB_CUDA(cudaMemcpy(y, dy.p, dy.bytes, cudaMemcpyDeviceToHost));
}

}
```

nemotron-speech.cpp_b200/csrc/engine.h:

```cpp
#pragma once
#include <deque>
#include <map>
#include <memory>
#include <string>
#include <tuple>
#include <vector>

#include "../../include/nsb200.h"
#include "gguf_loader.h"
#include "host_stream.h"
#include "kernels.cuh"

namespace nsb {

struct DevBuf {
    void* p = nullptr; size_t bytes = 0;
    DevBuf() = default;
    DevBuf(const DevBuf&) = delete; DevBuf& operator=(const DevBuf&) = delete;
    DevBuf(DevBuf&& o) noexcept : p(o.p), bytes(o.bytes) { o.p = nullptr; o.bytes = 0; }
    DevBuf& operator=(DevBuf&& o) noexcept { if (this != &o) { if (p) cudaFree(p); p = o.p; bytes = o.bytes; o.p = nullptr; o.bytes = 0; } return *this; }
    ~DevBuf() { if (p) cudaFree(p); }
    void alloc(size_t n, bool zero = true) {
        if (p) { cudaFree(p); p = nullptr; }
        bytes = n; if (!n) return;
        NSB_CUDA(cudaMalloc(&p, n));
        if (zero) { NSB_CUDA(cudaMemset(p, 0, n)); NSB_CUDA(cudaDeviceSynchronize()); }
    }
    template <class T> T* as() const { return (T*)p; }
};

struct HostPinned {
    void* p = nullptr; size_t bytes = 0;
    ~HostPinned() { if (p) cudaFreeHost(p); }
    void alloc(size_t n) { if (p) { cudaFreeHost(p); p = nullptr; } bytes = n; if (n) NSB_CUDA(cudaMallocHost(&p, n)); }
    template <class T> T* as() const { return (T*)p; }
};

struct Weight {
    std::string name; int n_out = 0, n_in = 0;
    int q4 = 0;
    int shadow_slot = -1;
    bool f32 = false;
    DevBuf data;
    DevBuf scales;
};

struct LayerW {
    DevBuf ln[10];
    Weight ff1a, ff1b, qkv, out, pw1, pw2, ff2a, ff2b;
    DevBuf bias_u, bias_v, dw_w, cln_g, cln_b;
    DevBuf pos_proj;
};

class Engine {
public:
    Engine(const std::string& gguf_path, const nsb_engine_config& cfg);
    ~Engine();

    int open_stream(); void close_stream(int s); void reset_stream(int s);
    void push_pcm(int s, const int16_t* pcm, int n);
    bool ready(int s) const;
    int step();
    int step_begin();
    int step_end();
    int pop_tokens(int s, int32_t* out, int cap);
    int chunks(int s) const;
    std::string detok(const int32_t* t, int n) const;

    void bench_prepare(int n_streams, const int16_t* pcm, int samples_per_stream, int warm_chunks);
    float bench_step();
    float bench_steps(int n, float* ms_each);
    enum { PC_MEL = 0, PC_SUBSAMPLE, PC_LAYERNORM, PC_GEMM, PC_ATTENTION, PC_CONVMOD, PC_DECODE, PC_MISC, PC_COUNT };
    float bench_profile(float* ms_per_class, int* launches_per_class);
    float bench_gemm(int kind, int rows, int bn, int stages, int splits, int rotate, int iters);

    void trace_enable(int cap);
    int trace_fetch(TraceRec* out, int cap);

    void set_cuda_graph(bool on) { collect_all(); cfg_.use_cuda_graph = on ? 1 : 0; }
    void debug_enable(bool on);
    long long debug_get(const std::string& name, float* out, size_t cap);
    long long debug_get_cache(int stream, int which, int layer, float* out, size_t cap);
    long long op_logmel(const int16_t* pcm, int n_streams, int n_samples, float* out, size_t cap);
    long long op_gemm(const std::string& name, const float* x, int rows, float* y, size_t cap);
    long long op_gemm_ex(const nsb_gemm_op& op, const float* x, void* y, size_t y_bytes, long long* guard_bad);
    void op_layernorm(const float* x, int rows, const float* planes, int n_planes, float alpha, const float* g1, const float* b1,
                      const float* g2, const float* b2, bool fused, int out_type, float* x_out, void* y);
    long long transcribe_full(const int16_t* pcm, int n_samples, int32_t* tokens, int32_t* token_frames, int cap, int* n_frames, float* enc_out, size_t enc_cap);

    int n_layers = 0, T = 1, R = 0, compute = NSB_COMPUTE_F32, kv_dtype = NSB_KV_F32, max_streams = 0;
    std::vector<char> vocab;
    nsb_stats stats{};
    int chunk_samples() const { return (PRE_CACHE + 8 * T) * HOP; }
    int shift_samples() const { return 8 * T * HOP; }

private:
    void load_weights(const GgufFile& g);
    void upload_weight(Weight& w, const std::string& name, const std::vector<float>& host, int n_out, int n_in);
    void load_layer_matrix(Weight& w, const GgufFile& g, const std::string& out_name, const std::vector<std::string>& parts, int n_out, int n_in);
    void alloc_state();
    void stream_upload(void* dst, const uint8_t* src, size_t bytes);
    HostPinned up_[2]; cudaEvent_t up_ev_[2] = {nullptr, nullptr}; int up_k_ = 0; DevBuf d_raw_;
    void release_handles();
    void zero_slot(int slot);
    void build_pos_tables(const GgufFile& g);
    void ensure_full_pos(int frames);
    std::string gguf_path_;
    std::vector<DevBuf> full_pos_; int full_pos_cap_ = 0;
    void gemm(const void* A, long long lda, const Weight& W, int M, const float* bias, void* C, long long ldc, int epi, float alpha,
              int out_type);
    void gemm(GemmArgs& a, const Weight& W);
    void gemm_residual(const void* A, long long lda, const Weight& W, int M, float* x, float alpha);
    bool split_consumers(int rows) const;
    const Weight& op_weight(const std::string& name) const;
    const void* op_operand(const Weight& W, const float* xh, int rows, DevBuf& dx, DevBuf& da);
    struct SplitScratch;
    void q8_predequant(const Weight& W, int M, GemmArgs& a);
    void gemm_f32w(GemmArgs& g, const Weight& W, bool a_presplit);
    void gemm_planes(const void* A, long long lda, const Weight& W, int M, void* C, int planes);
    PartialSum pending_{};
    void run_encoder_kernels(int B, const int16_t* d_pcm, int side);
    void run_decode_kernels(int B, int side, cudaStream_t s, bool narrow);
    void join_decode_stream();
    int side_acquire();
    cudaStream_t run_step(int B, const int16_t* d_pcm, int side, bool pipelined);
    bool overlap_decode(int rows, bool pipelined) const;
    struct StepGraph { cudaGraphExec_t exec = nullptr; long long launches = 0; };
    std::map<std::tuple<int, const void*, int>, StepGraph> graphs_;
    std::map<std::tuple<int, int, int>, StepGraph> dec_graphs_;
    template <class Key, class Fn> void run_graphed(std::map<Key, StepGraph>& cache, const Key& key, cudaStream_t s, Fn&& body);
    struct Side { DevBuf slot, encp, out_tok, out_cnt, sync; cudaEvent_t enc_done = nullptr, dec_done = nullptr; bool dec_pending = false; };
    static constexpr int MAX_INFLIGHT = 3;
    Side side_[MAX_INFLIGHT]; int side_next_ = 0;
    cudaStream_t st_dec_ = nullptr;
    cudaStream_t st_copy_ = nullptr;
    struct StepIO {
        HostPinned h_pcm, h_slot, h_tok, h_cnt;
        DevBuf d_pcm;
        cudaEvent_t ev0 = nullptr, ev1 = nullptr, done = nullptr, h2d = nullptr;
        std::vector<int> batch;
    };
    StepIO io_[MAX_INFLIGHT]; int io_next_ = 0, n_inflight_ = 0;
    void collect_tokens(StepIO& io);
    void collect_all();
    bool strict() const { return compute == NSB_COMPUTE_F32 || compute == NSB_COMPUTE_Q8_0_STRICT; }
    bool q8_planes_mode() const { return compute == NSB_COMPUTE_Q8_0 || compute == NSB_COMPUTE_Q8_0_STRICT; }
    int act_type() const { return strict() ? OUT_F32 : (compute == NSB_COMPUTE_BF16 ? OUT_BF16 : OUT_F16); }
    size_t act_size() const { return strict() ? 4 : 2; }
    void ensure_q8s_scratch(int rows);
    void count_launch(int n = 1) { stats.kernel_launches += n; }

    nsb_engine_config cfg_{};
    int device_ = 0;
    cudaStream_t st_ = nullptr;
    cudaEvent_t ev0_ = nullptr, ev1_ = nullptr;

    std::vector<LayerW> layers_;
    std::map<std::string, Weight*> named_;
    DevBuf window_, cos_t_, sin_t_, fb_t_;
    DevBuf c0_w_, c0_b_, c2_w_, c2_b_, c3_b_, c5_w_, c5_b_, c6_b_, out_b_;
    Weight c3_w_, c6_w_, sub_out_w_;
    Weight joint_enc_w_; DevBuf joint_enc_b_;
    DevBuf embed_, lstm_w_[4], lstm_b_[4], pred_w_, pred_b_, jout_w_, jout_b_;

    DevBuf kv_;
    DevBuf conv_cache_, cc_par_;
    DevBuf mel_hist_;
    DevBuf ring_pos_, valid_len_;
    DevBuf dec_h_, dec_c_, dec_par_, dec_proj_, prev_token_, cand_valid_;
    std::vector<HostStream> hs_;

    int rl_ = 0;
    DevBuf d_slot_, mel_new_, dw_, pw_, a3_, x_, a_, big_, qkv_, pw1_, encp_, part_;
    DevBuf out_tok_, out_cnt_, dec_sync_;
    struct BatchWork { DevBuf dw, pw, a3, x, a, big, qkv, pw1, encp, part, out_tok, out_frm; int rows = 0; } bw_;
    void ensure_batch_work(int rows, int t2);
    void swap_batch_work();
    int consumer_planes_ = 1;

    DevBuf q8s_scratch_;
    DevBuf shadow_[2]; size_t shadow_off_[8] = {}; size_t shadow_bytes_ = 0;
    cudaStream_t st_deq_ = nullptr; std::vector<cudaEvent_t> ev_deq_, ev_lstart_;
    const char* cur_shadow_ = nullptr;
    bool shadow_mode(int rows) const;
    void dequant_layer_async(int l, cudaStream_t s);
    DevBuf wscratch_;
    DevBuf bench_pcm_; int bench_B_ = 0, bench_n_ = 1; long long bench_i_ = 0;
    const int16_t* bench_next_pcm();
    struct ProfRec { int cls; cudaEvent_t a, b; };
    bool profiling_ = false; std::vector<ProfRec> prof_; std::vector<cudaEvent_t> ev_pool_; size_t ev_used_ = 0;
    cudaEvent_t prof_event();
    struct ProfScope {
        Engine* e; cudaEvent_t b = nullptr;
        ProfScope(Engine* e_, int cls) : e(e_) {
            if (!e->profiling_) return;
            cudaEvent_t a = e->prof_event(); b = e->prof_event();
            cudaEventRecord(a, e->st_); e->prof_.push_back({cls, a, b});
        }
        ~ProfScope() { if (b) cudaEventRecord(b, e->st_); }
    };

    bool debug_ = false; int dbg_B_ = 0, last_B_ = 0;
    DevBuf dbg_mel_, dbg_sub_, dbg_layers_, dbg_logits_, dbg_logits_n_;
    DevBuf trace_; int trace_cap_ = 0;
};

}
```

nemotron-speech.cpp_b200/csrc/gemm_tc.cu:

```cuda
#include <cuda.h>

#include <algorithm>
#include <initializer_list>
#include <mutex>
#include <stdexcept>
#include <string>

#include "kernels.cuh"

namespace nsb {

NSB_DEFINE_TRACE_BINDER(trace_bind_gemm_tc)

bool pair_gemm_enabled() {
    static const bool on = [] { const char* e = getenv("NSB_PAIR_GEMM"); return !(e && e[0] == '0'); }();
    return on;
}

bool q8_pair256_enabled() {
    const char* e = getenv("NSB_Q8_PAIR");
    return e && e[0] == '1';
}

static bool pair256_enabled() {
    static const bool on = [] { const char* e = getenv("NSB_PAIR256"); return !(e && e[0] == '0'); }();
    return on;
}

static bool pair256_persist_enabled() {
    const char* e = getenv("NSB_PAIR256_PERSIST");
    return e ? e[0] == '1' : false;
}

static int pair256_min_tiles() {
    static const int v = [] { const char* e = getenv("NSB_PAIR256_MIN_TILES"); return e ? atoi(e) : 4; }();
    return v;
}

namespace {

constexpr int BM = 128, ROW_BYTES = 128, UMMA_K_BYTES = 32;
constexpr int TC_THREADS = 192;
constexpr int Q8_THREADS = 320, Q8_DEQ = 256;
constexpr int QP_THREADS = 192, QP_DEQ = 128;

__device__ __forceinline__ uint32_t smem_u32(const void* p) { return (uint32_t)__cvta_generic_to_shared(p); }

__device__ __forceinline__ void mbar_init(uint64_t* bar, uint32_t count) {
    asm volatile("mbarrier.init.shared::cta.b64 [%0], %1;" ::"r"(smem_u32(bar)), "r"(count));
}
__device__ __forceinline__ void mbar_expect_tx(uint64_t* bar, uint32_t bytes) {
    asm volatile("mbarrier.arrive.expect_tx.shared::cta.b64 _, [%0], %1;" ::"r"(smem_u32(bar)), "r"(bytes) : "memory");
}
__device__ __forceinline__ void mbar_wait(uint64_t* bar, uint32_t parity) {
    const uint32_t addr = smem_u32(bar);
    for (uint32_t it = 0; it < (1u << 26); ++it) {
        uint32_t done;
        asm volatile(
            "{\n\t.reg .pred p;\n\t"
            "mbarrier.try_wait.parity.shared::cta.b64 p, [%1], %2;\n\t"
            "selp.u32 %0, 1, 0, p;\n\t}"
            : "=r"(done) : "r"(addr), "r"(parity) : "memory");
        if (done) return;
    }
    __trap();
}
__device__ __forceinline__ void tma_load_2d(void* smem_dst, const CUtensorMap* tm, uint64_t* bar, int c0, int c1) {
    asm volatile(
        "cp.async.bulk.tensor.2d.shared::cluster.global.mbarrier::complete_tx::bytes [%0], [%1, {%3, %4}], [%2];"
        ::"r"(smem_u32(smem_dst)), "l"(tm), "r"(smem_u32(bar)), "r"(c0), "r"(c1) : "memory");
}
__device__ __forceinline__ void tma_prefetch_2d(const CUtensorMap* tm, int c0, int c1) {
    asm volatile("cp.async.bulk.prefetch.tensor.2d.L2.global [%0, {%1, %2}];" ::"l"(tm), "r"(c0), "r"(c1) : "memory");
}
__device__ __forceinline__ uint32_t cluster_ctarank() { uint32_t r; asm volatile("mov.u32 %0, %%cluster_ctarank;" : "=r"(r)); return r; }
__device__ __forceinline__ void cluster_sync_all() {
    asm volatile("barrier.cluster.arrive.release.aligned;" ::: "memory");
    asm volatile("barrier.cluster.wait.acquire.aligned;" ::: "memory");
}
__device__ __forceinline__ void tma_load_2d_mc(void* smem_dst, const CUtensorMap* tm, uint64_t* bar, int c0, int c1, uint16_t mask) {
    asm volatile(
        "cp.async.bulk.tensor.2d.shared::cluster.global.mbarrier::complete_tx::bytes.multicast::cluster [%0], [%1, {%3, %4}], [%2], %5;"
        ::"r"(smem_u32(smem_dst)), "l"(tm), "r"(smem_u32(bar)), "r"(c0), "r"(c1), "h"(mask) : "memory");
}
__device__ __forceinline__ void umma_commit_mc(uint64_t* bar, uint16_t mask) {
    asm volatile("tcgen05.commit.cta_group::1.mbarrier::arrive::one.shared::cluster.multicast::cluster.b64 [%0], %1;"
                 ::"r"(smem_u32(bar)), "h"(mask) : "memory");
}
__device__ __forceinline__ void tma_load_2d_pair(void* smem_dst, const CUtensorMap* tm, uint64_t* bar, int c0, int c1) {
    asm volatile(
        "cp.async.bulk.tensor.2d.cta_group::2.shared::cluster.global.mbarrier::complete_tx::bytes.L2::cache_hint [%0], [%1, {%3, %4}], [%2], %5;"
// ... 207 lines not shown
    using S = Smem<BN, STAGES>;
    S& s = *reinterpret_cast<S*>((reinterpret_cast<uintptr_t>(smem_raw) + 1023) & ~uintptr_t(1023));
    const int warp = threadIdx.x >> 5, lane = threadIdx.x & 31;
    const int n0 = blockIdx.x * BN, m0 = blockIdx.y * BM;
    constexpr int BK = ROW_BYTES / EB;
    const int nk = p.K / BK / (int)gridDim.z;
    const int kb0 = (int)blockIdx.z * nk;
    const int rot = p.rot ? (int)((blockIdx.x / CL) % (unsigned)nk) : 0;
    constexpr uint32_t TMEM_COLS = tmem_cols_for(BN);
    constexpr uint32_t STAGE_BYTES = (BM + BN) * ROW_BYTES;

    if (threadIdx.x == 0) {
        s.trace_slot = (blockIdx.x | blockIdx.y | blockIdx.z) == 0 ? trace_begin(TR_GEMM_TC) : -1;
        for (int i = 0; i < STAGES; ++i) { mbar_init(&s.full[i], 1); mbar_init(&s.empty[i], CL); }
        mbar_init(&s.tmem_full, 1);
        asm volatile("fence.mbarrier_init.release.cluster;" ::: "memory");
    }
    if (warp == 0 && lane == 0) {
        asm volatile("prefetch.tensormap [%0];" ::"l"(&tmA) : "memory");
        asm volatile("prefetch.tensormap [%0];" ::"l"(&tmB) : "memory");
    }
    if (warp == 2) tmem_alloc(&s.tmem_slot, TMEM_COLS);
    tc_fence_before();
    __syncthreads();
    if (CL > 1) cluster_sync_all();
    tc_fence_after();
    const uint32_t tmem_base = s.tmem_slot;
    if (threadIdx.x == 0) { pdl_trigger(); trace_mark(s.trace_slot, 1); }
    const uint32_t crank = CL > 1 ? cluster_ctarank() : 0;
    constexpr uint16_t MC_MASK = (uint16_t)((1u << CL) - 1);
    constexpr int A_SLICE_ROWS = BM / CL;
    auto load_a = [&](int st, int kc) {
        if (EB == 4 && p.a_fold) kc = kc < p.a_fold ? kc : kc - p.a_fold;
        if (CL > 1) tma_load_2d_mc(s.a[st] + crank * A_SLICE_ROWS * ROW_BYTES, &tmA, &s.full[st], kc, m0 + (int)crank * A_SLICE_ROWS, MC_MASK);
        else tma_load_2d(s.a[st], &tmA, &s.full[st], kc, m0);
    };

    if (warp == 0) {
        if (elect_one()) {
            const int pre = nk < STAGES ? nk : STAGES;
            if (p.w_dyn) pdl_wait();
            for (int kb = 0; kb < pre; ++kb) {
                mbar_expect_tx(&s.full[kb], STAGE_BYTES);
                tma_load_2d(s.b[kb], &tmB, &s.full[kb], (kb0 + (kb + rot) % nk) * BK, n0);
            }
            if (!p.w_dyn) {
                for (int kb = pre; kb < nk; ++kb) tma_prefetch_2d(&tmB, (kb0 + (kb + rot) % nk) * BK, n0);
                pdl_wait();
            }
            for (int kb = 0; kb < pre; ++kb) load_a(kb, (kb0 + (kb + rot) % nk) * BK);
            for (int kb = pre; kb < nk; ++kb) {
                const int st = kb % STAGES; const uint32_t ph = (kb / STAGES) & 1;
                mbar_wait(&s.empty[st], ph ^ 1);
                mbar_expect_tx(&s.full[st], STAGE_BYTES);
                const int kc = (kb0 + (kb + rot) % nk) * BK;
                load_a(st, kc);
                tma_load_2d(s.b[st], &tmB, &s.full[st], kc, n0);
            }
        }
    } else if (warp == 1) {
        if (elect_one()) {
            const uint32_t idesc = make_idesc(p.fmt, BN);
            for (int kb = 0; kb < nk; ++kb) {
                const int st = kb % STAGES; const uint32_t ph = (kb / STAGES) & 1;
                mbar_wait(&s.full[st], ph);
                tc_fence_after();
                const uint32_t a_addr = smem_u32(s.a[st]), b_addr = smem_u32(s.b[st]);
#pragma unroll
                for (int k = 0; k < ROW_BYTES / UMMA_K_BYTES; ++k) {
                    if (EB == 4) umma_tf32(tmem_base, make_desc(a_addr + k * UMMA_K_BYTES), make_desc(b_addr + k * UMMA_K_BYTES), idesc, (kb | k) ? 1u : 0u);
                    else umma_f16(tmem_base, make_desc(a_addr + k * UMMA_K_BYTES), make_desc(b_addr + k * UMMA_K_BYTES), idesc, (kb | k) ? 1u : 0u);
                }
                if (CL > 1) umma_commit_mc(&s.empty[st], MC_MASK);
                else umma_commit(&s.empty[st]);
            }
            umma_commit(&s.tmem_full);
        }
    } else {
        tc_epilogue<BN>(p, tmem_base, &s.tmem_full, warp, lane, m0, n0, s.trace_slot, s.a[0]);
    }
    tc_fence_before();
    __syncthreads();
    if (CL > 1) cluster_sync_all();
    if (warp == 2) tmem_dealloc(tmem_base, TMEM_COLS);
}


template <int BN, int STAGES>
struct SmemPair {
    static_assert(STAGES * 64 * ROW_BYTES >= EPI_STAGE_BYTES, "the epilogue patch lives in the A ring");
    alignas(1024) uint8_t a[STAGES][64 * ROW_BYTES];
    alignas(1024) uint8_t b[STAGES][(BN / 2) * ROW_BYTES];
    alignas(8) uint64_t full[STAGES];
    uint64_t empty[STAGES];
    uint64_t tmem_full;
    uint32_t tmem_slot;
    int trace_slot;
};

template <int BN, int STAGES>
__global__ void __launch_bounds__(TC_THREADS, 1)
gemm_tc_pair_kernel(const __grid_constant__ CUtensorMap tmA, const __grid_constant__ CUtensorMap tmB, const TcParams p) {
    static_assert(BN % 64 == 0 && BN <= 256, "pair tile: BN/2 accumulator columns per lane half, read 32 at a time");
    extern __shared__ uint8_t smem_raw[];
    using S = SmemPair<BN, STAGES>;
    S& s = *reinterpret_cast<S*>((reinterpret_cast<uintptr_t>(smem_raw) + 1023) & ~uintptr_t(1023));
    const int warp = threadIdx.x >> 5, lane = threadIdx.x & 31;
    const uint32_t rank = cluster_ctarank();
    const int n0 = (int)(blockIdx.x >> 1) * BN, m0 = blockIdx.y * BM;
    constexpr int BK = ROW_BYTES / 2;
    const int nk = p.K / BK / (int)gridDim.z;
    const int kb0 = (int)blockIdx.z * nk;
    constexpr uint32_t TMEM_COLS = BN / 2 < 32 ? 32 : BN / 2;
    constexpr uint32_t HALF_BYTES = (64 + BN / 2) * ROW_BYTES;

    if (threadIdx.x == 0) {
        s.trace_slot = (blockIdx.x | blockIdx.y | blockIdx.z) == 0 ? trace_begin(TR_GEMM_TC) : -1;
        for (int i = 0; i < STAGES; ++i) { mbar_init(&s.full[i], 1); mbar_init(&s.empty[i], 1); }
        mbar_init(&s.tmem_full, 1);
        asm volatile("fence.mbarrier_init.release.cluster;" ::: "memory");
    }
    if (warp == 0 && lane == 0) {
        asm volatile("prefetch.tensormap [%0];" ::"l"(&tmA) : "memory");
        asm volatile("prefetch.tensormap [%0];" ::"l"(&tmB) : "memory");
    }
    if (warp == 2) tmem_alloc_pair(&s.tmem_slot, TMEM_COLS);
    tc_fence_before();
    __syncthreads();
    cluster_sync_all();
    tc_fence_after();
    const uint32_t tmem_base = s.tmem_slot;
    if (threadIdx.x == 0) { pdl_trigger(); trace_mark(s.trace_slot, 1); }

    if (warp == 0) {
        if (elect_one()) {
            const int a_row = m0 + (int)rank * 64, b_row = n0 + (int)rank * (BN / 2);
            const int pre = nk < STAGES ? nk : STAGES;
            for (int kb = 0; kb < pre; ++kb) {
                if (rank == 0) mbar_expect_tx(&s.full[kb], 2 * HALF_BYTES);
                tma_load_2d_pair(s.b[kb], &tmB, &s.full[kb], (kb0 + kb) * BK, b_row);
            }
            for (int kb = pre; kb < nk; ++kb) tma_prefetch_2d(&tmB, (kb0 + kb) * BK, b_row);
            pdl_wait();
            for (int kb = 0; kb < pre; ++kb) tma_load_2d_pair(s.a[kb], &tmA, &s.full[kb], (kb0 + kb) * BK, a_row);
            for (int kb = pre; kb < nk; ++kb) {
                const int st = kb % STAGES; const uint32_t ph = (kb / STAGES) & 1;
                mbar_wait(&s.empty[st], ph ^ 1);
                if (rank == 0) mbar_expect_tx(&s.full[st], 2 * HALF_BYTES);
                tma_load_2d_pair(s.a[st], &tmA, &s.full[st], (kb0 + kb) * BK, a_row);
                tma_load_2d_pair(s.b[st], &tmB, &s.full[st], (kb0 + kb) * BK, b_row);
            }
        }
    } else if (warp == 1) {
        if (rank == 0 && elect_one()) {
            const uint32_t idesc = make_idesc(p.fmt, BN);
            for (int kb = 0; kb < nk; ++kb) {
                const int st = kb % STAGES; const uint32_t ph = (kb / STAGES) & 1;
                mbar_wait(&s.full[st], ph);
                tc_fence_after();
                const uint32_t a_addr = smem_u32(s.a[st]), b_addr = smem_u32(s.b[st]);
#pragma unroll
                for (int k = 0; k < ROW_BYTES / UMMA_K_BYTES; ++k)
                    umma_f16_pair(tmem_base, make_desc(a_addr + k * UMMA_K_BYTES), make_desc(b_addr + k * UMMA_K_BYTES), idesc, (kb | k) ? 1u : 0u);
                umma_commit_pair(&s.empty[st]);
            }
            umma_commit_pair(&s.tmem_full);
// ... 794 lines not shown
}
void launch_dequant_q8(const void* q, const void* scales, void* out_f16, int N, int K, cudaStream_t st, int q4) {
    if (K % 32 != 0) throw CudaError("dequant_q8: K must be a multiple of 32");
    if (q4) {
        const size_t nb = (size_t)N * K / 32;
        launch_k(dequant_q4_kernel, dim3((unsigned)std::min<size_t>((nb + 255) / 256, 148 * 8)), dim3(256), 0, st, (const uint4*)q, (const __half*)scales, (uint4*)out_f16, nb);
        return;
    }
    const size_t n_vec = (size_t)N * K / 16;
    const int blocks = (int)std::min<size_t>((n_vec + 255) / 256, 148 * 8);
    launch_k(dequant_q8_kernel, dim3(blocks), dim3(256), 0, st, (const uint4*)q, (const __half*)scales, (uint4*)out_f16, n_vec, K);
}

void launch_gemm_tc(const GemmArgs& a, int in_type, cudaStream_t st) {
    if (a.M <= 0) return;
    if (a.group != 0) throw CudaError("gemm_tc: row maps are not supported");
    const int fmt = in_type == OUT_F32 ? 2 : in_type == OUT_BF16 ? 1 : 0;
    const int BK = fmt == 2 ? 32 : 64;
    if (a.K % BK != 0 || a.N % 32 != 0 || (a.lda % (fmt == 2 ? 4 : 8)) != 0 || (a.ldc % 4) != 0)
        throw CudaError("gemm_tc: unsupported shape (need K % 64 == 0 (tf32: 32), N % 32 == 0, 16-byte aligned rows)");
    if (a.c_group > 0 && a.M % a.c_group != 0) throw CudaError("gemm_tc: M must be a multiple of the output row group");
    if (a.a_fold && (fmt != 2 || a.K != 3 * a.a_fold || a.a_fold % BK != 0)) throw CudaError("gemm_tc: 3xTF32 needs fp32 operands and K = 3 x the folded width");
    const int tiles_m = (a.M + BM - 1) / BM;
    if (a.w_scales) {
        if (fmt != 0) throw CudaError("gemm_q8: activations must be fp16");
        check_splits(a, BK);
        if (a.force_bn) { check_forced_config(a, fmt); launch_q8_pair256(a, a.force_bn, st); return; }
        if (tiles_m >= pair256_min_tiles() && q8_pair256_enabled()) {
            static const int split_bn = [] { const char* e = getenv("NSB_SPLIT_BN"); return e ? atoi(e) : 112; }();
            const int bn = a.splits > 1 ? (split_bn == 256 ? 208 : split_bn) : pick_q8_pair256_bn(a.M, a.N);
            if (bn) { launch_q8_pair256(a, bn, st); return; }
        }
        if (a.splits > 1) { if (a.N % 64 == 0 && a.K >= 4096) launch_cfg_q8<64, 4>(a, st); else launch_cfg_q8<32, 5>(a, st); return; }
        if (a.N % 128 == 0 && (long long)tiles_m * (a.N / 128) >= 120) launch_cfg_q8<128, 4>(a, st);
        else if (a.N % 64 == 0 && (long long)tiles_m * (a.N / 64) >= 120) launch_cfg_q8<64, 4>(a, st);
        else launch_cfg_q8<32, 5>(a, st);
        return;
    }
    if (a.force_bn) {
        check_splits(a, BK);
        check_forced_config(a, fmt);
        if (a.force_stages == 97) { launch_pair256(a, fmt, a.force_bn, st); return; }
        if (a.force_stages == 96) { launch_pair256_persist(a, fmt, a.force_bn, st); return; }
        const int key = a.force_bn * 100 + a.force_stages;
        switch (key) {
            case 3204: launch_cfg<32, 4>(a, fmt, st); break;
            case 3205: launch_cfg<32, 5>(a, fmt, st); break;
            case 3208: launch_cfg<32, 8>(a, fmt, st); break;
            case 6404: launch_cfg<64, 4>(a, fmt, st); break;
            case 6498: launch_cfg_pair<64, 8>(a, fmt, st); break;
            case 6406: launch_cfg<64, 6>(a, fmt, st); break;
            case 12803: launch_cfg<128, 3>(a, fmt, st); break;
            case 12804: launch_cfg<128, 4>(a, fmt, st); break;
            case 25602: launch_cfg<256, 2>(a, fmt, st); break;
            case 25603: launch_cfg<256, 3>(a, fmt, st); break;
            default: throw CudaError("gemm_tc: tile config not instantiated");
        }
        return;
    }
    if (a.splits > 1) {
        check_splits(a, BK);
        if (fmt != 2 && tiles_m >= 8 && pair256_enabled()) {
            static const int bn = [] { const char* e = getenv("NSB_SPLIT_BN"); return e ? atoi(e) : 112; }();
            if (pair256_persist_enabled()) launch_pair256_persist(a, fmt, bn, st); else launch_pair256(a, fmt, bn, st);
            return;
        }
        if (a.N % 128 == 0 && a.M > 128 && fmt == 2) { launch_cfg<128, 4>(a, fmt, st); return; }
        if (a.N % 64 == 0 && a.K >= 4096) launch_cfg<64, 4>(a, fmt, st); else launch_cfg<32, 5>(a, fmt, st);
        return;
    }
    if (fmt != 2 && a.pair && !a.w_dynamic && pair_gemm_enabled() && tiles_m == 1 && a.N % 64 == 0) { launch_cfg_pair<64, 8>(a, fmt, st); return; }
    if (fmt != 2 && tiles_m >= pair256_min_tiles() && pair256_enabled()) {
        const int bn = pick_pair256_bn(a.M, a.N);
        if (bn) { if (pair256_persist_enabled()) launch_pair256_persist(a, fmt, bn, st); else launch_pair256(a, fmt, bn, st); return; }
    }
    const long long t256 = a.N % 256 == 0 ? (long long)tiles_m * (a.N / 256) : 0, t128 = a.N % 128 == 0 ? (long long)tiles_m * (a.N / 128) : 0;
    if (t256 >= 200) launch_cfg<256, 2>(a, fmt, st);
    else if (t128 >= 200) launch_cfg<128, 3>(a, fmt, st);
    else if (t128 >= 100) launch_cfg<128, 4>(a, fmt, st);
    else if (a.N % 64 == 0 && (long long)tiles_m * (a.N / 64) >= 120) launch_cfg<64, 4>(a, fmt, st);
    else launch_cfg<32, 5>(a, fmt, st);
}

}
```

nemotron-speech.cpp_b200/csrc/kernels.cuh:

```cuda
#pragma once
#include "common.cuh"

namespace nsb {

void trace_bind_frontend(TraceBuf*); void trace_bind_layer(TraceBuf*); void trace_bind_simt(TraceBuf*);
void trace_bind_gemm_tc(TraceBuf*); void trace_bind_decode(TraceBuf*);

void launch_logmel(const int16_t* pcm, int pcm_row_stride, int B, int n_frames, const float* window512,
                   const float* cos_t, const float* sin_t, const float* fb_t , float* mel_out,
                   size_t out_batch_stride, cudaStream_t st);

void launch_conv0(const float* mel_hist, const float* mel_new, const int* slot_of_b, int B, int T, const float* w_t ,
                  const float* bias, float* out, cudaStream_t st);
void launch_stem_conv0_dw(const float* mel_hist, const float* mel_new, const int* slot_of_b, int B, int T, const float* w0_t,
                          const float* b0, const float* w2_t, const float* b2, float* out, cudaStream_t st, int split = 0);
void launch_stem_conv0_dw_full(const float* mel, int B, int M, const float* w0_t, const float* b0, const float* w2_t, const float* b2,
                               float* out, cudaStream_t st, int split = 0);
void launch_mel_hist_update(float* mel_hist, const float* mel_new, const int* slot_of_b, int B, int T, cudaStream_t st);
void launch_mel_gather(const float* mel_hist, const float* mel_new, const int* slot_of_b, int B, int T, float* out, cudaStream_t st);
void launch_dwconv_s2(const float* in, int B, int H, int W, const float* w_t , const float* bias, float* out,
                      cudaStream_t st, int split = 0);
void launch_split_tf32(const float* in, float* out, size_t rows, int K, cudaStream_t st);

struct GemmArgs {
    const void* A = nullptr;
    long long lda = 0;
    int group = 0; long long group_stride = 0; int row_off = 0;
    const void* W = nullptr;
    const void* w_scales = nullptr;
    int q4 = 0;
    int M = 0, N = 0, K = 0;
    const float* bias = nullptr;
    void* C = nullptr; long long ldc = 0;
    int epi = EPI_NONE; float alpha = 1.0f; int out_type = OUT_F32;
    int splits = 1;
    int c_group = 0, c_drop = 0; void* C0 = nullptr;
    int force_bn = 0, force_stages = 0;
    int pair = 0;
    int w_dynamic = 0;
    int multicast = 1;
    int a_fold = 0;
    int rotate = 1;
};
void launch_gemm_simt(const GemmArgs& a, cudaStream_t st);
void launch_gemm_q8_strict(const GemmArgs& a, void* scratch, size_t scratch_bytes, cudaStream_t st);
size_t q8_strict_scratch_bytes(int rows, int K);

struct PartialSum { const float* part = nullptr; int n = 0; float alpha = 0.f; };
void launch_layernorm(float* x, int rows, const float* g, const float* b, void* y, int out_type, const PartialSum& ps, cudaStream_t st);
void launch_layernorm2(float* x, int rows, const float* g1, const float* b1, const float* g2, const float* b2, void* y2,
                       int out_type, const PartialSum& ps, cudaStream_t st);

struct AttnArgs {
    const float* qkv;
    int planes = 1; long long plane_stride = 0;
    void* k_ring; void* v_ring;
    long long slot_stride;
    int kv_dtype;
    const void* pos_proj;
    const float* bias_u; const float* bias_v;
    void* ctx; int out_type;
    const int* slot_of_b; const int* ring_pos; const int* valid_len;
    int B, T;
};
void launch_attention(const AttnArgs& a, cudaStream_t st);
struct AttnFullArgs {
    const float* qkv; const void* pos_proj; int pos_center; int kv_dtype;
    const float* bias_u; const float* bias_v; void* ctx; int out_type; int T;
};
void launch_attention_full(const AttnFullArgs& a, cudaStream_t st);
void launch_dequant_q8(const void* q, const void* scales, void* out_f16, int N, int K, cudaStream_t st, int q4 = 0);
bool pair_gemm_enabled();
bool q8_pair256_enabled();

struct ConvModArgs {
    const float* pw1;
    int planes = 1; long long plane_stride = 0;
    float* conv_cache;
    long long slot_stride;
    const int* cc_par; long long par_stride;
    const float* dw_w;
    const float* ln_g; const float* ln_b;
    void* out; int out_type;
    const int* slot_of_b; int B, T;
};
void launch_conv_module(const ConvModArgs& a, cudaStream_t st);

void launch_advance_streams(const int* slot_of_b, int B, int T, int* ring_pos, int* valid_len, int* cc_par, cudaStream_t st);

struct DecodeWeights {
    const float* embed;
    const float* w_ih[2]; const float* w_hh[2]; const float* b_ih[2]; const float* b_hh[2];
    const float* pred_w; const float* pred_b;
    const float* out_w; const float* out_b;
};
struct DecodeState {
    float* hbuf; float* cbuf;
    int* par;
    float* dec_proj;
    int* prev_token; int* cand_valid;
};
struct DecodeArgs {
    DecodeWeights w; DecodeState s;
    const float* enc_proj;
    const int* slot_of_b; int B, T;
    int* out_tokens; int* out_count;
    int* out_frames;
    unsigned* barrier; unsigned long long* best;
    int pipe_min_n;
    float* logits_tap; int logits_tap_cap; int* logits_tap_n;
};
int launch_decode(const DecodeArgs& a, void* sync_buf, cudaStream_t st, int narrow_ctas = 0);
int decode_narrow_ctas();
size_t decode_sync_bytes(int B);

}
```

nemotron-speech.cpp_b200/csrc/kernels_layer.cu:

```cuda
#include <cstdlib>

#include "kernels.cuh"

namespace nsb {

NSB_DEFINE_TRACE_BINDER(trace_bind_layer)

__device__ __forceinline__ float block_sum_256(float v, float* red ) {
    v = warp_sum(v);
    const int w = threadIdx.x >> 5, l = threadIdx.x & 31;
    __syncthreads();
    if (l == 0) red[w] = v;
    __syncthreads();
    float t = 0.f;
#pragma unroll
    for (int i = 0; i < 8; ++i) t += red[i];
    return t;
}

__device__ __forceinline__ void block_mean_var_256(float v0, float v1, float v2, float v3, float* red , float& mean, float& var) {
    float m = ((v0 + v1) + (v2 + v3)) * 0.25f;
    float M2 = (v0 - m) * (v0 - m) + (v1 - m) * (v1 - m) + (v2 - m) * (v2 - m) + (v3 - m) * (v3 - m);
    float half_n = 2.0f;
#pragma unroll
    for (int o = 1; o < 32; o <<= 1) {
        const float mo = __shfl_xor_sync(0xffffffffu, m, o), M2o = __shfl_xor_sync(0xffffffffu, M2, o);
        const float d = mo - m;
        M2 = (M2 + M2o) + d * d * half_n; m = m + 0.5f * d; half_n *= 2.0f;
    }
    const int w = threadIdx.x >> 5, l = threadIdx.x & 31;
    __syncthreads();
    if (l == 0) { red[2 * w] = m; red[2 * w + 1] = M2; }
    __syncthreads();
    float mm[8], MM[8];
#pragma unroll
    for (int i = 0; i < 8; ++i) { mm[i] = red[2 * i]; MM[i] = red[2 * i + 1]; }
#pragma unroll
    for (int n = 8; n > 1; n >>= 1) {
#pragma unroll
        for (int i = 0; i < n / 2; ++i) {
            const float d = mm[2 * i + 1] - mm[2 * i];
            MM[i] = (MM[2 * i] + MM[2 * i + 1]) + d * d * half_n; mm[i] = mm[2 * i] + 0.5f * d;
        }
        half_n *= 2.0f;
    }
    mean = mm[0]; var = MM[0] * (1.0f / D_MODEL);
}

__device__ __forceinline__ float4 load_x_reduced(float* x, size_t o, const PartialSum& ps, int rows) {
    float4 v = *(const float4*)(x + o);
    if (ps.n > 0) {
        float4 t[8];
#pragma unroll
        for (int s = 0; s < 8; ++s) if (s < ps.n) t[s] = __ldcg((const float4*)(ps.part + (size_t)s * rows * D_MODEL + o));
        float4 acc = make_float4(0.f, 0.f, 0.f, 0.f);
#pragma unroll
        for (int s = 0; s < 8; ++s) if (s < ps.n) { acc.x += t[s].x; acc.y += t[s].y; acc.z += t[s].z; acc.w += t[s].w; }
        v.x += ps.alpha * acc.x; v.y += ps.alpha * acc.y; v.z += ps.alpha * acc.z; v.w += ps.alpha * acc.w;
        *(float4*)(x + o) = v;
    }
    return v;
}

__global__ void __launch_bounds__(256) layernorm_kernel(float* x, const float* __restrict__ g,
                                                        const float* __restrict__ b, void* y, int out_type, const PartialSum ps) {
    NSB_KERNEL_BEGIN(TR_LN)
    __shared__ float red[16];
    const int row = blockIdx.x, c = threadIdx.x * 4;
    const float4 gg = *(const float4*)(g + c), bb = *(const float4*)(b + c);
    NSB_KERNEL_WAIT()
    const float4 v = load_x_reduced(x, (size_t)row * D_MODEL + c, ps, gridDim.x);
    float mean, var;
    if (out_type == OUT_F32) {
        mean = block_sum_256(v.x + v.y + v.z + v.w, red) * (1.0f / D_MODEL);
        const float e0 = v.x - mean, e1 = v.y - mean, e2 = v.z - mean, e3 = v.w - mean;
        var = block_sum_256(e0 * e0 + e1 * e1 + e2 * e2 + e3 * e3, red) * (1.0f / D_MODEL);
    } else block_mean_var_256(v.x, v.y, v.z, v.w, red, mean, var);
    const float d0 = v.x - mean, d1 = v.y - mean, d2 = v.z - mean, d3 = v.w - mean;
    const float rs = 1.0f / sqrtf(var + 1e-5f);
    const size_t o = (size_t)row * D_MODEL + c;
    const float o0 = d0 * rs * gg.x + bb.x, o1 = d1 * rs * gg.y + bb.y, o2 = d2 * rs * gg.z + bb.z, o3 = d3 * rs * gg.w + bb.w;
    if (out_type == OUT_F32) *(float4*)((float*)y + o) = make_float4(o0, o1, o2, o3);
    else if (out_type == OUT_F16) { __half2* p = (__half2*)((__half*)y + o); p[0] = __floats2half2_rn(o0, o1); p[1] = __floats2half2_rn(o2, o3); }
    else { __nv_bfloat162* p = (__nv_bfloat162*)((__nv_bfloat16*)y + o); p[0] = __floats2bfloat162_rn(o0, o1); p[1] = __floats2bfloat162_rn(o2, o3); }
    NSB_KERNEL_EPILOGUE();
}

__device__ __forceinline__ void warp_mean_var_1024(const float4 (&v)[8], float& mean, float& var) {
    float s = 0.f;
#pragma unroll
    for (int j = 0; j < 8; ++j) s += (v[j].x + v[j].y) + (v[j].z + v[j].w);
    float m = s * (1.0f / 32.0f), M2 = 0.f;
#pragma unroll
    for (int j = 0; j < 8; ++j) { const float a = v[j].x - m, b = v[j].y - m, c = v[j].z - m, d = v[j].w - m; M2 += (a * a + b * b) + (c * c + d * d); }
    float half_n = 16.0f;
#pragma unroll
    for (int o = 1; o < 32; o <<= 1) {
        const float mo = __shfl_xor_sync(0xffffffffu, m, o), M2o = __shfl_xor_sync(0xffffffffu, M2, o);
        const float d = mo - m;
        M2 = (M2 + M2o) + d * d * half_n; m = m + 0.5f * d; half_n *= 2.0f;
    }
    mean = m; var = M2 * (1.0f / D_MODEL);
}
__device__ __forceinline__ void store4_out(void* y, size_t o, float4 r, int out_type) {
    if (out_type == OUT_F32) *(float4*)((float*)y + o) = r;
    else if (out_type == OUT_F16) { __half2* p = (__half2*)((__half*)y + o); p[0] = __floats2half2_rn(r.x, r.y); p[1] = __floats2half2_rn(r.z, r.w); }
    else { __nv_bfloat162* p = (__nv_bfloat162*)((__nv_bfloat16*)y + o); p[0] = __floats2bfloat162_rn(r.x, r.y); p[1] = __floats2bfloat162_rn(r.z, r.w); }
}

__global__ void __launch_bounds__(256) layernorm_rows_kernel(float* x, int rows, const float* __restrict__ g1, const float* __restrict__ b1,
                                                             const float* __restrict__ g2, const float* __restrict__ b2, void* y, int out_type,
                                                             const PartialSum ps) {
    NSB_KERNEL_BEGIN(g2 ? TR_LN2 : TR_LN)
    const int lane = threadIdx.x & 31, row = blockIdx.x * 8 + (threadIdx.x >> 5);
    NSB_KERNEL_WAIT()
    if (row >= rows) return;
    float* xr = x + (size_t)row * D_MODEL;
    float4 v[8];
#pragma unroll
    for (int j = 0; j < 8; ++j) v[j] = *(const float4*)(xr + 4 * (32 * j + lane));
    if (ps.n > 0) {
        float4 acc[8];
        for (int sl = 0; sl < ps.n; ++sl) {
            const float* pr = ps.part + ((size_t)sl * rows + row) * D_MODEL;
            float4 t[8];
#pragma unroll
            for (int j = 0; j < 8; ++j) t[j] = __ldcg((const float4*)(pr + 4 * (32 * j + lane)));
#pragma unroll
            for (int j = 0; j < 8; ++j) {
                if (sl == 0) { acc[j] = make_float4(0.f + t[j].x, 0.f + t[j].y, 0.f + t[j].z, 0.f + t[j].w); }
                else { acc[j].x += t[j].x; acc[j].y += t[j].y; acc[j].z += t[j].z; acc[j].w += t[j].w; }
            }
        }
#pragma unroll
        for (int j = 0; j < 8; ++j) { v[j].x += ps.alpha * acc[j].x; v[j].y += ps.alpha * acc[j].y; v[j].z += ps.alpha * acc[j].z; v[j].w += ps.alpha * acc[j].w; }
        if (!g2 && y) {
#pragma unroll
            for (int j = 0; j < 8; ++j) *(float4*)(xr + 4 * (32 * j + lane)) = v[j];
        }
    }
    float mean, var;
    warp_mean_var_1024(v, mean, var);
    float rs = 1.0f / sqrtf(var + 1e-5f);
#pragma unroll
    for (int j = 0; j < 8; ++j) {
        const float4 gg = *(const float4*)(g1 + 4 * (32 * j + lane)), bb = *(const float4*)(b1 + 4 * (32 * j + lane));
        v[j] = make_float4((v[j].x - mean) * rs * gg.x + bb.x, (v[j].y - mean) * rs * gg.y + bb.y, (v[j].z - mean) * rs * gg.z + bb.z, (v[j].w - mean) * rs * gg.w + bb.w);
    }
    if (!g2 && y) {
#pragma unroll
        for (int j = 0; j < 8; ++j) store4_out(y, (size_t)row * D_MODEL + 4 * (32 * j + lane), v[j], out_type);
        NSB_KERNEL_EPILOGUE();
        return;
    }
#pragma unroll
    for (int j = 0; j < 8; ++j) *(float4*)(xr + 4 * (32 * j + lane)) = v[j];
    if (g2) {
        warp_mean_var_1024(v, mean, var);
        rs = 1.0f / sqrtf(var + 1e-5f);
#pragma unroll
        for (int j = 0; j < 8; ++j) {
            const float4 gg = *(const float4*)(g2 + 4 * (32 * j + lane)), bb = *(const float4*)(b2 + 4 * (32 * j + lane));
            const float4 r = make_float4((v[j].x - mean) * rs * gg.x + bb.x, (v[j].y - mean) * rs * gg.y + bb.y, (v[j].z - mean) * rs * gg.z + bb.z, (v[j].w - mean) * rs * gg.w + bb.w);
            store4_out(y, (size_t)row * D_MODEL + 4 * (32 * j + lane), r, out_type);
        }
    }
    NSB_KERNEL_EPILOGUE();
}
static bool ln_rows_enabled(int rows, int out_type) {
    static const int min_rows = [] { const char* e = getenv("NSB_LN_ROWS_MIN"); return e ? atoi(e) : 1024; }();
    return out_type != OUT_F32 && rows >= min_rows;
}
void launch_layernorm(float* x, int rows, const float* g, const float* b, void* y, int out_type, const PartialSum& ps, cudaStream_t st) {
    if (rows > 0 && ln_rows_enabled(rows, out_type)) {
        launch_k(layernorm_rows_kernel, dim3((rows + 7) / 8), dim3(256), 0, st, x, rows, g, b, (const float*)nullptr, (const float*)nullptr, y, out_type, ps);
        return;
    }
    if (rows > 0) launch_k(layernorm_kernel, dim3(rows), dim3(256), 0, st, x, g, b, y, out_type, ps);
}

__global__ void __launch_bounds__(256) layernorm2_kernel(float* x, const float* __restrict__ g1, const float* __restrict__ b1,
                                                         const float* __restrict__ g2, const float* __restrict__ b2,
                                                         void* y2, int out_type, const PartialSum ps) {
    NSB_KERNEL_BEGIN(TR_LN2)
    __shared__ float red[16];
    const int row = blockIdx.x, c = threadIdx.x * 4;
    const size_t o = (size_t)row * D_MODEL + c;
    const bool one_pass = out_type != OUT_F32;
    float4 gg = *(const float4*)(g1 + c), bb = *(const float4*)(b1 + c);
    float4 gg2 = make_float4(0.f, 0.f, 0.f, 0.f), bb2 = gg2;
    if (y2 != nullptr) { gg2 = *(const float4*)(g2 + c); bb2 = *(const float4*)(b2 + c); }
    NSB_KERNEL_WAIT()
    float4 v = load_x_reduced(x, o, ps, gridDim.x);
    float mean, var, d0, d1, d2, d3;
    auto stats = [&]() {
        if (one_pass) block_mean_var_256(v.x, v.y, v.z, v.w, red, mean, var);
        else {
            mean = block_sum_256(v.x + v.y + v.z + v.w, red) * (1.0f / D_MODEL);
            const float e0 = v.x - mean, e1 = v.y - mean, e2 = v.z - mean, e3 = v.w - mean;
            var = block_sum_256(e0 * e0 + e1 * e1 + e2 * e2 + e3 * e3, red) * (1.0f / D_MODEL);
        }
        d0 = v.x - mean; d1 = v.y - mean; d2 = v.z - mean; d3 = v.w - mean;
    };
    stats();
    float rs = 1.0f / sqrtf(var + 1e-5f);
    v = make_float4(d0 * rs * gg.x + bb.x, d1 * rs * gg.y + bb.y, d2 * rs * gg.z + bb.z, d3 * rs * gg.w + bb.w);
    *(float4*)(x + o) = v;
    if (y2 == nullptr) { NSB_KERNEL_EPILOGUE(); return; }
    stats();
    rs = 1.0f / sqrtf(var + 1e-5f);
    gg = gg2; bb = bb2;
    const float o0 = d0 * rs * gg.x + bb.x, o1 = d1 * rs * gg.y + bb.y, o2 = d2 * rs * gg.z + bb.z, o3 = d3 * rs * gg.w + bb.w;
    if (out_type == OUT_F32) *(float4*)((float*)y2 + o) = make_float4(o0, o1, o2, o3);
    else if (out_type == OUT_F16) { __half2* p = (__half2*)((__half*)y2 + o); p[0] = __floats2half2_rn(o0, o1); p[1] = __floats2half2_rn(o2, o3); }
    else { __nv_bfloat162* p = (__nv_bfloat162*)((__nv_bfloat16*)y2 + o); p[0] = __floats2bfloat162_rn(o0, o1); p[1] = __floats2bfloat162_rn(o2, o3); }
    NSB_KERNEL_EPILOGUE();
}
void launch_layernorm2(float* x, int rows, const float* g1, const float* b1, const float* g2, const float* b2, void* y2, int out_type,
                       const PartialSum& ps, cudaStream_t st) {
    if (rows > 0 && ln_rows_enabled(rows, out_type)) {
        launch_k(layernorm_rows_kernel, dim3((rows + 7) / 8), dim3(256), 0, st, x, rows, g1, b1, g2, b2, y2, out_type, ps);
        return;
    }
    if (rows > 0) launch_k(layernorm2_kernel, dim3(rows), dim3(256), 0, st, x, g1, b1, g2, b2, y2, out_type, ps);
}

template <int KV> struct KvT { using type = float; };
template <> struct KvT<1> { using type = __half; };
template <> struct KvT<2> { using type = __nv_bfloat16; };

constexpr int ATT_MAX_T = 65, ATT_MAX_K = ATT_L + ATT_MAX_T + 1, ATT_MAX_REL = ATT_L + 2 * ATT_MAX_T;
constexpr int ATT_PROWS = 5;

__device__ __forceinline__ void load4(const float* p, float (&f)[4]) {
    const float4 v = *reinterpret_cast<const float4*>(p); f[0] = v.x; f[1] = v.y; f[2] = v.z; f[3] = v.w;
}
__device__ __forceinline__ void load4(const __half* p, float (&f)[4]) {
    const uint2 v = *reinterpret_cast<const uint2*>(p);
    const float2 a = __half22float2(*reinterpret_cast<const __half2*>(&v.x)), b = __half22float2(*reinterpret_cast<const __half2*>(&v.y));
    f[0] = a.x; f[1] = a.y; f[2] = b.x; f[3] = b.y;
}
__device__ __forceinline__ void load4(const __nv_bfloat16* p, float (&f)[4]) {
    const uint2 v = *reinterpret_cast<const uint2*>(p);
    const float2 a = __bfloat1622float2(*reinterpret_cast<const __nv_bfloat162*>(&v.x)), b = __bfloat1622float2(*reinterpret_cast<const __nv_bfloat162*>(&v.y));
    f[0] = a.x; f[1] = a.y; f[2] = b.x; f[3] = b.y;
}
__device__ __forceinline__ void load2(const float* p, float (&f)[2]) { const float2 v = *reinterpret_cast<const float2*>(p); f[0] = v.x; f[1] = v.y; }
__device__ __forceinline__ void load2(const __half* p, float (&f)[2]) { const float2 v = __half22float2(*reinterpret_cast<const __half2*>(p)); f[0] = v.x; f[1] = v.y; }
__device__ __forceinline__ void load2(const __nv_bfloat16* p, float (&f)[2]) { const float2 v = __bfloat1622float2(*reinterpret_cast<const __nv_bfloat162*>(p)); f[0] = v.x; f[1] = v.y; }
__device__ __forceinline__ void cp_async16(void* smem_dst, const void* gsrc) {
    asm volatile("cp.async.cg.shared.global [%0], [%1], 16;" ::"r"((uint32_t)__cvta_generic_to_shared(smem_dst)), "l"(gsrc) : "memory");
}

template <int MAXP>
__device__ __forceinline__ float4 ld4_planes(const float* p, int planes, long long stride) {
    float4 v = *reinterpret_cast<const float4*>(p);
    if (planes > 1) {
        float4 t[MAXP - 1];
#pragma unroll
        for (int z = 1; z < MAXP; ++z) if (z < planes) t[z - 1] = *reinterpret_cast<const float4*>(p + (size_t)z * stride);
#pragma unroll
        for (int z = 1; z < MAXP; ++z) if (z < planes) { v.x += t[z - 1].x; v.y += t[z - 1].y; v.z += t[z - 1].z; v.w += t[z - 1].w; }
    }
    return v;
}
constexpr int QKV_MAX_PLANES = 2, PW1_MAX_PLANES = 4;
__device__ __forceinline__ void load4_planes(const float* p, int planes, long long stride, float (&f)[4]) {
    const float4 v = ld4_planes<QKV_MAX_PLANES>(p, planes, stride); f[0] = v.x; f[1] = v.y; f[2] = v.z; f[3] = v.w;
}

template <int NV>
__device__ __forceinline__ float warp_sum_halving(float (&s)[NV], int lane, int& idx, bool& owner) {
    static_assert(NV == 1 || NV == 2 || NV == 4 || NV == 8 || NV == 16, "power of two");
    int n = NV, bit = 16;
    idx = 0;
#pragma unroll
    for (int step = 0; step < 5; ++step) {
        if (n > 1) {
            const bool hi = (lane & bit) != 0;
            n >>= 1;
#pragma unroll
            for (int k = 0; k < NV / 2; ++k) {
                if (k < n) {
                    const float send = hi ? s[k] : s[k + n], keep = hi ? s[k + n] : s[k];
                    s[k] = keep + __shfl_xor_sync(0xffffffffu, send, bit);
                }
            }
            idx = idx * 2 + (hi ? 1 : 0);
        } else {
            s[0] += __shfl_xor_sync(0xffffffffu, s[0], bit);
        }
        bit >>= 1;
    }
    owner = (lane & (32 / NV - 1)) == 0;
    return s[0];
}

template <int TQ> struct AttnSmemF {
// ... 1046 lines not shown
```

Before: 5686.

## Fuse split-K residual GEMM with following layernorm via chained kernel

Adds a gemm_chain path that runs the split-K residual GEMMs (ffn down, attention out, pointwise-2) and then performs the partial-sum reduction, residual add and layernorm (or double layernorm) inside the same launch. Completion is coordinated through per-layer, per-site counters in global memory. This removes the separate layernorm launch and a round trip of the partial planes for small row counts in 16-bit compute modes. The layernorm row logic moves into a shared header so both kernels can use it. The cost is extra complexity from inter-CTA counter synchronisation and possible tail serialisation in the last CTA per row tile.

```diff
diff --git a/include/nsb200.h b/include/nsb200.h
--- a/include/nsb200.h
+++ b/include/nsb200.h
@@ -128,6 +128,8 @@
 int nsb_op_gemm_ex(nsb_engine* e, const nsb_gemm_op* op, const float* x, void* y, size_t y_bytes, long long* guard_bad);
 int nsb_op_layernorm(nsb_engine* e, const float* x, int rows, const float* planes, int n_planes, float alpha, const float* g1, const float* b1,
                      const float* g2, const float* b2, int fused, int out_type, float* x_out, void* y);
+int nsb_op_gemm_chain(nsb_engine* e, const char* weight, const float* a, int rows, const float* x, float alpha, const float* g1, const float* b1,
+                      const float* g2, const float* b2, int norm2, float* x_out, void* y, float* planes, long long* guard_bad, unsigned* ctr_after);
 
 int nsb_transcribe_full(nsb_engine* e, const int16_t* pcm, int n_samples, int32_t* tokens, int32_t* token_frames, int cap, int* n_frames,
                         float* enc_out, size_t enc_cap_floats);
diff --git a/nemotron-speech.cpp_b200/__init__.py b/nemotron-speech.cpp_b200/__init__.py
--- a/nemotron-speech.cpp_b200/__init__.py
+++ b/nemotron-speech.cpp_b200/__init__.py
@@ -34,7 +34,7 @@
 
 
 TRACE_TAGS = {1: "logmel", 2: "stem", 3: "dwconv", 4: "melhist", 5: "gemm_f32", 6: "gemm_tc", 7: "gemm_q8", 8: "ln", 9: "ln2", 10: "attn",
-              11: "convmod", 12: "advance", 13: "decode", 14: "other"}
+              11: "convmod", 12: "advance", 13: "decode", 14: "other", 15: "chain"}
 
 
 class GemmOp(C.Structure):
@@ -53,7 +53,7 @@
            "nsb_stream_open", "nsb_stream_close", "nsb_stream_reset", "nsb_stream_push_pcm", "nsb_push_pcm_batch", "nsb_pop_tokens_batch", "nsb_stream_ready", "nsb_engine_step", "nsb_engine_step_begin", "nsb_engine_step_end",
            "nsb_engine_drain", "nsb_stream_pop_tokens", "nsb_stream_chunks", "nsb_detokenize", "nsb_engine_get_stats",
            "nsb_bench_prepare", "nsb_bench_step", "nsb_bench_steps", "nsb_bench_profile", "nsb_profiler_range", "nsb_bench_gemm", "nsb_trace_enable", "nsb_trace_fetch", "nsb_debug_enable", "nsb_debug_get", "nsb_debug_get_cache", "nsb_op_logmel",
-           "nsb_op_gemm", "nsb_op_gemm_ex", "nsb_op_layernorm", "nsb_transcribe_full"]
+           "nsb_op_gemm", "nsb_op_gemm_ex", "nsb_op_layernorm", "nsb_op_gemm_chain", "nsb_transcribe_full"]
 
 
 def build(force: bool = False) -> str:
@@ -111,6 +111,8 @@
         L.nsb_op_gemm.argtypes = [vp, C.c_char_p, _f32p, ci, _f32p, C.c_size_t]
         L.nsb_op_gemm_ex.argtypes = [vp, C.POINTER(GemmOp), _f32p, vp, C.c_size_t, C.POINTER(C.c_longlong)]
         L.nsb_op_layernorm.argtypes = [vp, _f32p, ci, vp, ci, C.c_float, _f32p, _f32p, vp, vp, ci, ci, _f32p, vp]
+        L.nsb_op_gemm_chain.argtypes = [vp, C.c_char_p, _f32p, ci, _f32p, C.c_float, _f32p, _f32p, vp, vp, ci, _f32p, vp, _f32p,
+                                        C.POINTER(C.c_longlong), C.POINTER(C.c_uint)]
         L.nsb_transcribe_full.argtypes = [vp, _i16p, ci, _i32p, _i32p, ci, C.POINTER(C.c_int), C.c_void_p, C.c_size_t]
         _lib = L
     return _lib
@@ -346,6 +348,23 @@
                                       y.ctypes.data_as(C.c_void_p)))
         return x_out, y
 
+    def op_gemm_chain(self, weight_name: str, a: np.ndarray, x: np.ndarray, g1, b1, *, alpha: float = 1.0, norm2: bool = False, g2=None, b2=None):
+        a = np.ascontiguousarray(a, dtype=np.float32)
+        x = np.ascontiguousarray(x, dtype=np.float32)
+        rows = x.shape[0]
+        f = lambda v: None if v is None else np.ascontiguousarray(v, dtype=np.float32)
+        g1, b1, g2, b2 = f(g1), f(b1), f(g2), f(b2)
+        vp = lambda v: None if v is None else v.ctypes.data_as(C.c_void_p)
+        x_out = np.empty_like(x)
+        y = np.zeros((rows, 1024), dtype=np.uint16)
+        splits = 8 if a.shape[1] >= 4096 else 4
+        planes = np.empty((splits, rows, 1024), dtype=np.float32)
+        bad = C.c_longlong(-1)
+        ctr = (C.c_uint * 2)(7, 7)
+        _check(lib().nsb_op_gemm_chain(self.h, weight_name.encode(), a, rows, x, alpha, g1, b1, vp(g2), vp(b2), int(norm2), x_out,
+                                       y.ctypes.data_as(C.c_void_p), planes.reshape(-1), C.byref(bad), ctr))
+        return x_out, y, planes, bad.value, (ctr[0], ctr[1])
+
     def transcribe_full(self, pcm: np.ndarray, want_enc: bool = True, want_frames: bool = False):
         pcm = np.ascontiguousarray(pcm, dtype=np.int16)
         frames_cap = len(pcm) // 1280 + 8
diff --git a/nemotron-speech.cpp_b200/csrc/c_api.cu b/nemotron-speech.cpp_b200/csrc/c_api.cu
--- a/nemotron-speech.cpp_b200/csrc/c_api.cu
+++ b/nemotron-speech.cpp_b200/csrc/c_api.cu
@@ -172,6 +172,10 @@
                      const float* g2, const float* b2, int fused, int out_type, float* x_out, void* y) {
     if (!e || !x || !x_out || !y) return fail(NSB_ERR_ARG, "bad argument");
     NSB_TRY e->impl->op_layernorm(x, rows, planes, n_planes, alpha, g1, b1, g2, b2, fused != 0, out_type, x_out, y); return NSB_OK; NSB_CATCH }
+int nsb_op_gemm_chain(nsb_engine* e, const char* weight, const float* a, int rows, const float* x, float alpha, const float* g1, const float* b1,
+                      const float* g2, const float* b2, int norm2, float* x_out, void* y, float* planes, long long* guard_bad, unsigned* ctr_after) {
+    if (!e || !weight || !a || !x || !x_out || !y || !planes) return fail(NSB_ERR_ARG, "bad argument");
+    NSB_TRY e->impl->op_gemm_chain(weight, a, rows, x, alpha, g1, b1, g2, b2, norm2 != 0, x_out, y, planes, guard_bad, ctr_after); return NSB_OK; NSB_CATCH }
 
 int nsb_transcribe_full(nsb_engine* e, const int16_t* pcm, int n, int32_t* tokens, int32_t* token_frames, int cap, int* n_frames, float* enc_out, size_t enc_cap) {
     if (!e || !pcm) return fail(NSB_ERR_ARG, "bad argument"); NSB_TRY return (int)e->impl->transcribe_full(pcm, n, tokens, token_frames, cap, n_frames, enc_out, enc_cap); NSB_CATCH }
diff --git a/nemotron-speech.cpp_b200/csrc/common.cuh b/nemotron-speech.cpp_b200/csrc/common.cuh
--- a/nemotron-speech.cpp_b200/csrc/common.cuh
+++ b/nemotron-speech.cpp_b200/csrc/common.cuh
@@ -76,7 +76,7 @@
 
 struct TraceRec { unsigned long long t[6]; int tag; int grid; };
 struct TraceBuf { unsigned n; unsigned cap; unsigned pad[2]; TraceRec rec[1]; };
-enum TraceTag : int { TR_LOGMEL = 1, TR_STEM, TR_DWCONV, TR_MELHIST, TR_GEMM_SIMT, TR_GEMM_TC, TR_GEMM_Q8, TR_LN, TR_LN2, TR_ATTN, TR_CONVMOD, TR_ADVANCE, TR_DECODE, TR_OTHER };
+enum TraceTag : int { TR_LOGMEL = 1, TR_STEM, TR_DWCONV, TR_MELHIST, TR_GEMM_SIMT, TR_GEMM_TC, TR_GEMM_Q8, TR_LN, TR_LN2, TR_ATTN, TR_CONVMOD, TR_ADVANCE, TR_DECODE, TR_OTHER, TR_CHAIN };
 static __constant__ TraceBuf* c_trace;
 #define NSB_DEFINE_TRACE_BINDER(name) \
     void name(TraceBuf* p) { NSB_CUDA(cudaMemcpyToSymbol(c_trace, &p, sizeof(p))); }
diff --git a/nemotron-speech.cpp_b200/csrc/engine.cu b/nemotron-speech.cpp_b200/csrc/engine.cu
--- a/nemotron-speech.cpp_b200/csrc/engine.cu
+++ b/nemotron-speech.cpp_b200/csrc/engine.cu
@@ -454,6 +454,7 @@
     encp_.alloc(Mrows * JOINT * 4);
     part_.alloc((size_t)MAX_SPLITS * std::min<size_t>(Mrows, 1024) * D_MODEL * 4);
     out_tok_.alloc((size_t)S * MAX_SYMBOLS * T * 4); out_cnt_.alloc((size_t)S * 4);
+    chain_ctr_.alloc((size_t)n_layers * 4 * CHAIN_CTR_WORDS * 4);
     dec_sync_.alloc(decode_sync_bytes(S));
     for (Side& sd : side_) {
         sd.slot.alloc((size_t)S * 4); sd.encp.alloc(Mrows * JOINT * 4); sd.out_tok.alloc((size_t)S * MAX_SYMBOLS * T * 4);
@@ -588,7 +589,7 @@
     count_launch();
 }
 
-void Engine::gemm_residual(const void* A, long long lda, const Weight& W, int M, float* x, float alpha) {
+int Engine::residual_splits(const Weight& W, int M) const {
     int splits = 1;
     if (!strict() && M <= 1024) {
         const int tiles = ((M + 127) / 128) * (W.n_out / (W.n_in >= 4096 ? 64 : 32));
@@ -597,6 +598,11 @@
     }
     static const int big_split = [] { const char* e = getenv("NSB_FFDOWN_SPLIT"); return e ? atoi(e) : 2; }();
     if (!strict() && M > 1024 && W.n_in >= 4096 && big_split > 1 && (size_t)big_split * M * D_MODEL * 4 <= part_.bytes) splits = big_split;
+    return splits;
+}
+
+void Engine::gemm_residual(const void* A, long long lda, const Weight& W, int M, float* x, float alpha) {
+    const int splits = residual_splits(W, M);
     if (splits == 1) { gemm(A, lda, W, M, nullptr, x, D_MODEL, EPI_RESID, alpha, OUT_F32); return; }
     GemmArgs a; a.A = A; a.lda = lda; a.W = W.data.p; a.w_scales = W.scales.p; a.q4 = W.q4; a.M = M; a.N = W.n_out; a.K = W.n_in; a.C = part_.p; a.ldc = D_MODEL;
     a.epi = EPI_PARTIAL; a.out_type = OUT_F32; a.splits = splits;
@@ -605,6 +611,21 @@
       launch_gemm_tc(a, act_type(), st_); }
     count_launch();
     pending_.part = part_.as<float>(); pending_.n = splits; pending_.alpha = alpha;
+}
+
+bool Engine::chain_ok(const Weight& W, int M) const {
+    const bool dense16 = compute == NSB_COMPUTE_F16 || compute == NSB_COMPUTE_BF16 || (cur_shadow_ && W.shadow_slot >= 0);
+    return !strict() && dense16 && M <= CHAIN_MAX_ROWS && W.n_out == D_MODEL && residual_splits(W, M) > 1;
+}
+
+void Engine::gemm_chain(const void* A, long long lda, const Weight& W, const void* w16, int M, float* x, float alpha, const float* g1,
+                        const float* b1, const float* g2, const float* b2, void* y, bool norm2, unsigned* ctr, void* planes) {
+    ChainArgs c; GemmArgs& a = c.g;
+    a.A = A; a.lda = lda; a.W = w16; a.M = M; a.N = W.n_out; a.K = W.n_in; a.C = planes; a.ldc = D_MODEL;
+    a.epi = EPI_PARTIAL; a.out_type = OUT_F32; a.splits = residual_splits(W, M);
+    c.x = x; c.alpha = alpha; c.g1 = g1; c.b1 = b1; c.g2 = g2; c.b2 = b2; c.y = y; c.out_type = act_type(); c.norm2 = norm2; c.ctr = ctr;
+    { ProfScope ps(this, PC_GEMM); launch_gemm_chain(c, act_type(), st_); }
+    count_launch();
 }
 
 int Engine::open_stream() {
@@ -857,10 +878,27 @@
             cur_shadow_ = shadow_[l & 1].as<char>();
             pdl_skip_next();
         }
-        if (!(skip & SK_FF)) {
-        gemm(a_.p, D_MODEL, L.ff1a, rows, nullptr, big_.p, D_FF, EPI_SILU, 1.f, at);
-        gemm_residual(big_.p, D_FF, L.ff1b, rows, x, 0.5f); }
-        ln(L.ln[2].as<float>(), L.ln[3].as<float>());
+        const bool last = l + 1 == n_layers;
+        auto resid_ln = [&](bool gemm_on, const void* A, long long lda, const Weight& W, float alpha, int site, const float* g1, const float* b1,
+                            bool norm2) {
+            const float* g2 = norm2 && !last ? layers_[l + 1].ln[0].as<float>() : nullptr;
+            const float* b2 = norm2 && !last ? layers_[l + 1].ln[1].as<float>() : nullptr;
+            void* y = norm2 && last ? nullptr : a_.p;
+            if (gemm_on && !(skip & SK_LN) && chain_ok(W, rows)) {
+                const void* w16 = cur_shadow_ && W.shadow_slot >= 0 ? cur_shadow_ + shadow_off_[W.shadow_slot] : W.data.p;
+                gemm_chain(A, lda, W, w16, rows, x, alpha, g1, b1, g2, b2, y, norm2, chain_ctr_.as<unsigned>() + (size_t)(l * 4 + site) * CHAIN_CTR_WORDS,
+                           part_.p);
+                return;
+            }
+            if (gemm_on) gemm_residual(A, lda, W, rows, x, alpha);
+            if (!norm2) { ln(g1, b1); return; }
+            if (skip & SK_LN) pending_ = PartialSum{};
+            else { ProfScope ps(this, PC_LAYERNORM);
+              launch_layernorm2(x, rows, g1, b1, g2, b2, y, at, pending_, st_);
+              count_launch(); pending_ = PartialSum{}; }
+        };
+        if (!(skip & SK_FF)) gemm(a_.p, D_MODEL, L.ff1a, rows, nullptr, big_.p, D_FF, EPI_SILU, 1.f, at);
+        resid_ln(!(skip & SK_FF), big_.p, D_FF, L.ff1b, 0.5f, 0, L.ln[2].as<float>(), L.ln[3].as<float>(), false);
         const int qkv_planes = split_consumers(rows) ? 2 : 1;
         const int pw1_planes = 1;
         if (!(skip & SK_QKV)) {
@@ -877,8 +915,7 @@
             aa.slot_of_b = slot; aa.ring_pos = ring_pos_.as<int>(); aa.valid_len = valid_len_.as<int>(); aa.B = B; aa.T = T;
             ProfScope ps(this, PC_ATTENTION); launch_attention(aa, st_); count_launch();
         }
-        if (!(skip & SK_OUT)) gemm_residual(a_.p, D_MODEL, L.out, rows, x, 1.f);
-        ln(L.ln[4].as<float>(), L.ln[5].as<float>());
+        resid_ln(!(skip & SK_OUT), a_.p, D_MODEL, L.out, 1.f, 1, L.ln[4].as<float>(), L.ln[5].as<float>(), false);
         if (!(skip & SK_PW)) {
             if (pw1_planes == 1) gemm(a_.p, D_MODEL, L.pw1, rows, nullptr, pw1_.p, 2 * D_MODEL, EPI_NONE, 1.f, OUT_F32);
             else gemm_planes(a_.p, D_MODEL, L.pw1, rows, pw1_.p, pw1_planes);
@@ -890,17 +927,9 @@
             ca.out = a_.p; ca.out_type = at; ca.slot_of_b = slot; ca.B = B; ca.T = T;
             ProfScope ps(this, PC_CONVMOD); launch_conv_module(ca, st_); count_launch();
         }
-        if (!(skip & SK_PW)) gemm_residual(a_.p, D_MODEL, L.pw2, rows, x, 1.f);
-        ln(L.ln[6].as<float>(), L.ln[7].as<float>());
-        if (!(skip & SK_FF)) {
-        gemm(a_.p, D_MODEL, L.ff2a, rows, nullptr, big_.p, D_FF, EPI_SILU, 1.f, at);
-        gemm_residual(big_.p, D_FF, L.ff2b, rows, x, 0.5f); }
-        const bool last = l + 1 == n_layers;
-        if (skip & SK_LN) pending_ = PartialSum{};
-        else { ProfScope ps(this, PC_LAYERNORM);
-          launch_layernorm2(x, rows, L.ln[8].as<float>(), L.ln[9].as<float>(), last ? nullptr : layers_[l + 1].ln[0].as<float>(),
-                            last ? nullptr : layers_[l + 1].ln[1].as<float>(), last ? nullptr : a_.p, at, pending_, st_);
-          count_launch(); pending_ = PartialSum{}; }
+        resid_ln(!(skip & SK_PW), a_.p, D_MODEL, L.pw2, 1.f, 2, L.ln[6].as<float>(), L.ln[7].as<float>(), false);
+        if (!(skip & SK_FF)) gemm(a_.p, D_MODEL, L.ff2a, rows, nullptr, big_.p, D_FF, EPI_SILU, 1.f, at);
+        resid_ln(!(skip & SK_FF), big_.p, D_FF, L.ff2b, 0.5f, 3, L.ln[8].as<float>(), L.ln[9].as<float>(), true);
         if (debug_) NSB_CUDA(cudaMemcpyAsync(dbg_layers_.as<float>() + (size_t)l * dbg_B_ * T * D_MODEL, x, (size_t)rows * D_MODEL * 4,
                                              cudaMemcpyDeviceToDevice, st_));
     }
@@ -1411,8 +1440,8 @@
 
 struct Guarded {
     DevBuf d; size_t es = 4, ld = 0, live = 0, cols = 0;
-    void init(size_t live_rows, size_t n, size_t elem, const float* live_init) {
-        es = elem; ld = n + GUARD_COLS; live = live_rows; cols = n;
+    void init(size_t live_rows, size_t n, size_t elem, const float* live_init, size_t pad_cols = GUARD_COLS) {
+        es = elem; ld = n + pad_cols; live = live_rows; cols = n;
         std::vector<uint8_t> h(bytes());
         for (size_t i = 0; i + 4 <= h.size(); i += 4) memcpy(&h[i], &GUARD_WORD, 4);
         if (live_init)
@@ -1499,4 +1528,42 @@
     if (y && (!fused || g2)) NSB_CUDA(cudaMemcpy(y, dy.p, dy.bytes, cudaMemcpyDeviceToHost));
 }
 
-}
+void Engine::op_gemm_chain(const std::string& name, const float* ah, int rows, const float* xh, float alpha, const float* g1, const float* b1,
+                           const float* g2, const float* b2, bool norm2, float* x_out, void* y, float* planes, long long* guard_bad, unsigned* ctr_after) {
+    const Weight& W = op_weight(name);
+    auto bad = [](const std::string& m) { throw std::invalid_argument("op_gemm_chain: " + m); };
+    if (strict() || W.f32) bad("16-bit compute or Q8_0 only, on a per-layer matrix");
+    if (rows < 1 || rows > CHAIN_MAX_ROWS) bad("rows must be 1.." + std::to_string(CHAIN_MAX_ROWS));
+    if (W.n_out != D_MODEL || residual_splits(W, rows) < 2) bad("not an N = 1024 split-K matrix (ffn down-projections, attention out, pointwise-2)");
+    if (!g1 || !b1 || (!g2) != (!b2) || (g2 && !norm2)) bad("g1 / b1 required, g2 / b2 together and only with norm2");
+    NSB_CUDA(cudaSetDevice(device_));
+    DevBuf dx, da, dg1, db1, dg2, db2, ctr;
+    const void* A = op_operand(W, ah, rows, dx, da);
+    const void* w16 = W.data.p;
+    if (W.scales.p) {
+        if (wscratch_.bytes < (size_t)W.n_out * W.n_in * 2) throw std::runtime_error("op_gemm_chain: scratch not allocated");
+        launch_dequant_q8(W.data.p, W.scales.p, wscratch_.p, W.n_out, W.n_in, st_, W.q4);
+        w16 = wscratch_.p;
+    }
+    auto up = [](DevBuf& d, const float* h) { d.alloc(D_MODEL * 4, false); h2d_sync(d.p, h, D_MODEL * 4); };
+    up(dg1, g1); up(db1, b1);
+    if (g2) { up(dg2, g2); up(db2, b2); }
+    ctr.alloc(CHAIN_CTR_WORDS * 4);
+    const int splits = residual_splits(W, rows);
+    Guarded gx, gy, gp;
+    gx.init(rows, D_MODEL, 4, xh, 0);
+    gy.init(rows, D_MODEL, out_elem_size(act_type()), nullptr, 0);
+    gp.init((size_t)splits * rows, D_MODEL, 4, nullptr, 0);
+    const bool has_y = !norm2 || g2;
+    gemm_chain(A, W.n_in, W, w16, rows, (float*)gx.at(), alpha, dg1.as<float>(), db1.as<float>(), g2 ? dg2.as<float>() : nullptr,
+               g2 ? db2.as<float>() : nullptr, has_y ? gy.at() : nullptr, norm2, ctr.as<unsigned>(), gp.at());
+    NSB_CUDA(cudaStreamSynchronize(st_));
+    std::vector<uint8_t> yh(has_y ? 0 : (size_t)rows * D_MODEL * gy.es);
+    long long nbad = gx.fetch(x_out) + gp.fetch(planes) + gy.fetch(has_y ? y : yh.data());
+    if (guard_bad) *guard_bad = nbad;
+    unsigned cw[CHAIN_CTR_WORDS];
+    NSB_CUDA(cudaMemcpy(cw, ctr.p, sizeof(cw), cudaMemcpyDeviceToHost));
+    if (ctr_after) { ctr_after[0] = cw[0]; ctr_after[1] = cw[CHAIN_CTR_WORDS / 2]; }
+}
+
+}
diff --git a/nemotron-speech.cpp_b200/csrc/engine.h b/nemotron-speech.cpp_b200/csrc/engine.h
--- a/nemotron-speech.cpp_b200/csrc/engine.h
+++ b/nemotron-speech.cpp_b200/csrc/engine.h
@@ -86,6 +86,8 @@
     long long op_gemm_ex(const nsb_gemm_op& op, const float* x, void* y, size_t y_bytes, long long* guard_bad);
     void op_layernorm(const float* x, int rows, const float* planes, int n_planes, float alpha, const float* g1, const float* b1,
                       const float* g2, const float* b2, bool fused, int out_type, float* x_out, void* y);
+    void op_gemm_chain(const std::string& weight, const float* a, int rows, const float* x, float alpha, const float* g1, const float* b1,
+                       const float* g2, const float* b2, bool norm2, float* x_out, void* y, float* planes, long long* guard_bad, unsigned* ctr_after);
     long long transcribe_full(const int16_t* pcm, int n_samples, int32_t* tokens, int32_t* token_frames, int cap, int* n_frames, float* enc_out, size_t enc_cap);
 
     int n_layers = 0, T = 1, R = 0, compute = NSB_COMPUTE_F32, kv_dtype = NSB_KV_F32, max_streams = 0;
@@ -111,6 +113,10 @@
               int out_type);
     void gemm(GemmArgs& a, const Weight& W);
     void gemm_residual(const void* A, long long lda, const Weight& W, int M, float* x, float alpha);
+    int residual_splits(const Weight& W, int M) const;
+    bool chain_ok(const Weight& W, int M) const;
+    void gemm_chain(const void* A, long long lda, const Weight& W, const void* w16, int M, float* x, float alpha, const float* g1, const float* b1,
+                    const float* g2, const float* b2, void* y, bool norm2, unsigned* ctr, void* planes);
     bool split_consumers(int rows) const;
     const Weight& op_weight(const std::string& name) const;
     const void* op_operand(const Weight& W, const float* xh, int rows, DevBuf& dx, DevBuf& da);
@@ -173,6 +179,7 @@
     int rl_ = 0;
     DevBuf d_slot_, mel_new_, dw_, pw_, a3_, x_, a_, big_, qkv_, pw1_, encp_, part_;
     DevBuf out_tok_, out_cnt_, dec_sync_;
+    DevBuf chain_ctr_;
     struct BatchWork { DevBuf dw, pw, a3, x, a, big, qkv, pw1, encp, part, out_tok, out_frm; int rows = 0; } bw_;
     void ensure_batch_work(int rows, int t2);
     void swap_batch_work();
diff --git a/nemotron-speech.cpp_b200/csrc/gemm_tc.cu b/nemotron-speech.cpp_b200/csrc/gemm_tc.cu
--- a/nemotron-speech.cpp_b200/csrc/gemm_tc.cu
+++ b/nemotron-speech.cpp_b200/csrc/gemm_tc.cu
@@ -7,6 +7,7 @@
 #include <string>
 
 #include "kernels.cuh"
+#include "layernorm_row.cuh"
 
 namespace nsb {
 
@@ -380,6 +381,144 @@
     tc_fence_before();
     __syncthreads();
     if (CL > 1) cluster_sync_all();
+    if (warp == 2) tmem_dealloc(tmem_base, TMEM_COLS);
+}
+
+constexpr int CHAIN_THREADS = 256;
+struct ChainParams {
+    TcParams p;
+    int n_tiles, splits;
+    float* x; const float* g1; const float* b1; const float* g2; const float* b2; void* y; int out_type, norm2;
+    unsigned* ctr;
+};
+template <int BN, int STAGES>
+struct SmemChain {
+    Smem<BN, STAGES> g;
+    float red[16];
+    int task;
+};
+__device__ __forceinline__ unsigned atom_add_acq_rel(unsigned* p, unsigned v) {
+    unsigned old;
+    asm volatile("atom.acq_rel.gpu.global.add.u32 %0, [%1], %2;" : "=r"(old) : "l"(p), "r"(v) : "memory");
+    return old;
+}
+__device__ __forceinline__ void red_add_release(unsigned* p, unsigned v) {
+    asm volatile("red.release.gpu.global.add.u32 [%0], %1;" ::"l"(p), "r"(v) : "memory");
+}
+constexpr int CHAIN_CTR_DONE = CHAIN_CTR_WORDS / 2;
+__device__ __forceinline__ unsigned ld_acquire(const unsigned* p) {
+    unsigned v;
+    asm volatile("ld.acquire.gpu.global.u32 %0, [%1];" : "=r"(v) : "l"(p) : "memory");
+    return v;
+}
+
+template <int BN, int STAGES>
+__global__ void __launch_bounds__(CHAIN_THREADS, 2)
+gemm_chain_kernel(const __grid_constant__ CUtensorMap tmA, const __grid_constant__ CUtensorMap tmB, const ChainParams c) {
+    extern __shared__ uint8_t smem_raw[];
+    using SC = SmemChain<BN, STAGES>;
+    SC& sc = *reinterpret_cast<SC*>((reinterpret_cast<uintptr_t>(smem_raw) + 1023) & ~uintptr_t(1023));
+    Smem<BN, STAGES>& s = sc.g;
+    const TcParams& p = c.p;
+    const int warp = threadIdx.x >> 5, lane = threadIdx.x & 31;
+    constexpr int BK = ROW_BYTES / 2;
+    const int nk = p.K / BK / c.splits;
+    const int n_gemm = c.n_tiles * c.splits, n_tasks = n_gemm + p.M;
+    constexpr uint32_t TMEM_COLS = tmem_cols_for(BN);
+    constexpr uint32_t STAGE_BYTES = (BM + BN) * ROW_BYTES;
+
+    if (threadIdx.x == 0) {
+        s.trace_slot = blockIdx.x == 0 ? trace_begin(TR_CHAIN) : -1;
+        for (int i = 0; i < STAGES; ++i) { mbar_init(&s.full[i], 1); mbar_init(&s.empty[i], 1); }
+        mbar_init(&s.tmem_full, 1);
+        asm volatile("fence.mbarrier_init.release.cluster;" ::: "memory");
+    }
+    if (warp == 0 && lane == 0) {
+        asm volatile("prefetch.tensormap [%0];" ::"l"(&tmA) : "memory");
+        asm volatile("prefetch.tensormap [%0];" ::"l"(&tmB) : "memory");
+    }
+    if (warp == 2) tmem_alloc(&s.tmem_slot, TMEM_COLS);
+    tc_fence_before();
+    __syncthreads();
+    tc_fence_after();
+    const uint32_t tmem_base = s.tmem_slot;
+    if (threadIdx.x == 0) {
+        pdl_trigger(); trace_mark(s.trace_slot, 1);
+        if ((int)blockIdx.x < n_gemm) {
+            const int tn = (int)blockIdx.x % c.n_tiles, z = (int)blockIdx.x / c.n_tiles;
+            for (int kb = 0; kb < nk; ++kb) tma_prefetch_2d(&tmB, (z * nk + kb) * BK, tn * BN);
+        }
+    }
+    pdl_wait();
+    int tiles_done = 0;
+    for (;;) {
+        if (threadIdx.x == 0) sc.task = (int)atom_add_acq_rel(&c.ctr[0], 1u);
+        __syncthreads();
+        const int t = sc.task;
+        if (t >= n_tasks) {
+            if (threadIdx.x == 0 && t == n_tasks + (int)gridDim.x - 1) { atomicExch(&c.ctr[0], 0u); atomicExch(&c.ctr[CHAIN_CTR_DONE], 0u); }
+            break;
+        }
+        if (t < n_gemm) {
+            const int tn = t % c.n_tiles, z = t / c.n_tiles, n0 = tn * BN, kb0 = z * nk;
+            const int rot = p.rot ? tn % nk : 0;
+            const int g0 = tiles_done * nk;
+            if (warp == 0) {
+                if (elect_one()) {
+                    for (int kb = 0; kb < nk; ++kb) {
+                        const int g = g0 + kb, st = g % STAGES; const uint32_t ph = (g / STAGES) & 1;
+                        mbar_wait(&s.empty[st], ph ^ 1);
+                        mbar_expect_tx(&s.full[st], STAGE_BYTES);
+                        const int kc = (kb0 + (kb + rot) % nk) * BK;
+                        tma_load_2d(s.b[st], &tmB, &s.full[st], kc, n0);
+                        tma_load_2d(s.a[st], &tmA, &s.full[st], kc, 0);
+                    }
+                }
+            } else if (warp == 1) {
+                if (elect_one()) {
+                    const uint32_t idesc = make_idesc(p.fmt, BN);
+                    for (int kb = 0; kb < nk; ++kb) {
+                        const int g = g0 + kb, st = g % STAGES; const uint32_t ph = (g / STAGES) & 1;
+                        mbar_wait(&s.full[st], ph);
+                        tc_fence_after();
+                        const uint32_t a_addr = smem_u32(s.a[st]), b_addr = smem_u32(s.b[st]);
+#pragma unroll
+                        for (int k = 0; k < ROW_BYTES / UMMA_K_BYTES; ++k)
+                            umma_f16(tmem_base, make_desc(a_addr + k * UMMA_K_BYTES), make_desc(b_addr + k * UMMA_K_BYTES), idesc, (kb | k) ? 1u : 0u);
+                        umma_commit(&s.empty[st]);
+                    }
+                    umma_commit(&s.tmem_full);
+                }
+            } else if (warp < 6) {
+                tc_epilogue_at<BN>(p, tmem_base, &s.tmem_full, warp, (warp & 3) * 32, n0, tiles_done == 0 ? s.trace_slot : -1, s.a[0],
+                                   (uint32_t)(tiles_done & 1), z);
+            }
+            ++tiles_done;
+            tc_fence_before();
+            __syncthreads();
+            tc_fence_after();
+            if (threadIdx.x == 0) red_add_release(&c.ctr[CHAIN_CTR_DONE], 1u);
+        } else {
+            if (threadIdx.x == 0) {
+                uint32_t it = 0;
+                while (ld_acquire(&c.ctr[CHAIN_CTR_DONE]) < (unsigned)n_gemm) {
+                    if (++it == (1u << 24)) __trap();
+                    __nanosleep(32);
+                }
+            }
+            __syncthreads();
+            const int ch = threadIdx.x * 4;
+            const float4 gg = *(const float4*)(c.g1 + ch), bb = *(const float4*)(c.b1 + ch);
+            float4 gg2 = make_float4(0.f, 0.f, 0.f, 0.f), bb2 = gg2;
+            if (c.norm2 && c.y) { gg2 = *(const float4*)(c.g2 + ch); bb2 = *(const float4*)(c.b2 + ch); }
+            PartialSum ps; ps.part = (const float*)p.C; ps.n = c.splits; ps.alpha = p.alpha;
+            layernorm_row_256(c.x, t - n_gemm, p.M, gg, bb, gg2, bb2, c.norm2 != 0, c.y, c.out_type, ps, sc.red);
+            __syncthreads();
+        }
+    }
+    if (threadIdx.x == 0) trace_mark(s.trace_slot, 5);
+    tc_fence_before();
+    __syncthreads();
     if (warp == 2) tmem_dealloc(tmem_base, TMEM_COLS);
 }
 
@@ -1340,4 +1479,33 @@
     else launch_cfg<32, 5>(a, fmt, st);
 }
 
-}
+namespace {
+template <int BN, int STAGES>
+void launch_chain_cfg(const ChainArgs& c, int fmt, cudaStream_t st) {
+    static std::atomic<size_t> attr_set[MAX_DEVICES];
+    const GemmArgs& a = c.g;
+    require_full_grid(a.N, BN);
+    const size_t smem = sizeof(SmemChain<BN, STAGES>) + 1024;
+    ensure_dyn_smem(gemm_chain_kernel<BN, STAGES>, smem, attr_set);
+    const CUtensorMap tmA = make_map(a.A, a.M, a.K, a.lda, BM, fmt);
+    const CUtensorMap tmB = make_map(a.W, a.N, a.K, a.K, BN, fmt);
+    ChainParams p{TcParams{a.M, a.N, a.K, nullptr, a.C, a.ldc, EPI_PARTIAL, c.alpha, OUT_F32, fmt, a.rotate, 0, 0, nullptr, a.M},
+                  a.N / BN, a.splits, c.x, c.g1, c.b1, c.g2, c.b2, c.y, c.out_type, c.norm2 ? 1 : 0, c.ctr};
+    launch_k(gemm_chain_kernel<BN, STAGES>, dim3((a.N / BN) * a.splits), dim3(CHAIN_THREADS), smem, st, tmA, tmB, p);
+}
+}
+
+void launch_gemm_chain(const ChainArgs& c, int in_type, cudaStream_t st) {
+    const GemmArgs& a = c.g;
+    if (in_type != OUT_F16 && in_type != OUT_BF16) throw CudaError("gemm_chain: 16-bit operands only");
+    if (a.M < 1 || a.M > CHAIN_MAX_ROWS || a.N != D_MODEL || a.K % 64 != 0 || a.w_scales || a.w_dynamic || a.bias || a.C0 || a.c_group || a.ldc != D_MODEL)
+        throw CudaError("gemm_chain: one row tile of an N = 1024 matrix with dense 16-bit weights, planes of row stride 1024");
+    check_splits(a, 64);
+    if (a.splits < 2) throw CudaError("gemm_chain: split-K only");
+    if (!c.x || !c.g1 || !c.b1 || !c.ctr || (!c.norm2 && !c.y) || (c.y && c.norm2 && (!c.g2 || !c.b2)))
+        throw CudaError("gemm_chain: bad LayerNorm arguments");
+    const int fmt = in_type == OUT_BF16 ? 1 : 0;
+    if (a.K >= 4096) launch_chain_cfg<64, 4>(c, fmt, st); else launch_chain_cfg<32, 5>(c, fmt, st);
+}
+
+}
diff --git a/nemotron-speech.cpp_b200/csrc/kernels.cuh b/nemotron-speech.cpp_b200/csrc/kernels.cuh
--- a/nemotron-speech.cpp_b200/csrc/kernels.cuh
+++ b/nemotron-speech.cpp_b200/csrc/kernels.cuh
@@ -50,6 +50,16 @@
 void launch_layernorm(float* x, int rows, const float* g, const float* b, void* y, int out_type, const PartialSum& ps, cudaStream_t st);
 void launch_layernorm2(float* x, int rows, const float* g1, const float* b1, const float* g2, const float* b2, void* y2,
                        int out_type, const PartialSum& ps, cudaStream_t st);
+
+struct ChainArgs {
+    GemmArgs g;
+    float* x = nullptr; float alpha = 1.f;
+    const float* g1 = nullptr; const float* b1 = nullptr; const float* g2 = nullptr; const float* b2 = nullptr;
+    void* y = nullptr; int out_type = OUT_F16; bool norm2 = false;
+    unsigned* ctr = nullptr;
+};
+void launch_gemm_chain(const ChainArgs& c, int in_type, cudaStream_t st);
+constexpr int CHAIN_MAX_ROWS = 128, CHAIN_CTR_WORDS = 64;
 
 struct AttnArgs {
     const float* qkv;
diff --git a/nemotron-speech.cpp_b200/csrc/kernels_layer.cu b/nemotron-speech.cpp_b200/csrc/kernels_layer.cu
--- a/nemotron-speech.cpp_b200/csrc/kernels_layer.cu
+++ b/nemotron-speech.cpp_b200/csrc/kernels_layer.cu
@@ -1,113 +1,39 @@
 #include <cstdlib>
 
 #include "kernels.cuh"
+#include "layernorm_row.cuh"
 
 namespace nsb {
 
 NSB_DEFINE_TRACE_BINDER(trace_bind_layer)
 
-__device__ __forceinline__ float block_sum_256(float v, float* red ) {
-    v = warp_sum(v);
-    const int w = threadIdx.x >> 5, l = threadIdx.x & 31;
-    __syncthreads();
-    if (l == 0) red[w] = v;
-    __syncthreads();
-    float t = 0.f;
-#pragma unroll
-    for (int i = 0; i < 8; ++i) t += red[i];
-    return t;
-}
-
-__device__ __forceinline__ void block_mean_var_256(float v0, float v1, float v2, float v3, float* red , float& mean, float& var) {
-    float m = ((v0 + v1) + (v2 + v3)) * 0.25f;
-    float M2 = (v0 - m) * (v0 - m) + (v1 - m) * (v1 - m) + (v2 - m) * (v2 - m) + (v3 - m) * (v3 - m);
-    float half_n = 2.0f;
+__global__ void __launch_bounds__(256) layernorm_kernel(float* x, const float* __restrict__ g,
+                                                        const float* __restrict__ b, void* y, int out_type, const PartialSum ps) {
+    NSB_KERNEL_BEGIN(TR_LN)
+    __shared__ float red[16];
+    const int c = threadIdx.x * 4;
+    const float4 gg = *(const float4*)(g + c), bb = *(const float4*)(b + c);
+    NSB_KERNEL_WAIT()
+    layernorm_row_256(x, blockIdx.x, gridDim.x, gg, bb, gg, bb, false, y, out_type, ps, red);
+    NSB_KERNEL_EPILOGUE();
+}
+
+__device__ __forceinline__ void warp_mean_var_1024(const float4 (&v)[8], float& mean, float& var) {
+    float s = 0.f;
+#pragma unroll
+    for (int j = 0; j < 8; ++j) s += (v[j].x + v[j].y) + (v[j].z + v[j].w);
+    float m = s * (1.0f / 32.0f), M2 = 0.f;
+#pragma unroll
+    for (int j = 0; j < 8; ++j) { const float a = v[j].x - m, b = v[j].y - m, c = v[j].z - m, d = v[j].w - m; M2 += (a * a + b * b) + (c * c + d * d); }
+    float half_n = 16.0f;
 #pragma unroll
     for (int o = 1; o < 32; o <<= 1) {
         const float mo = __shfl_xor_sync(0xffffffffu, m, o), M2o = __shfl_xor_sync(0xffffffffu, M2, o);
         const float d = mo - m;
         M2 = (M2 + M2o) + d * d * half_n; m = m + 0.5f * d; half_n *= 2.0f;
     }
-    const int w = threadIdx.x >> 5, l = threadIdx.x & 31;
-    __syncthreads();
-    if (l == 0) { red[2 * w] = m; red[2 * w + 1] = M2; }
-    __syncthreads();
-    float mm[8], MM[8];
-#pragma unroll
-    for (int i = 0; i < 8; ++i) { mm[i] = red[2 * i]; MM[i] = red[2 * i + 1]; }
-#pragma unroll
-    for (int n = 8; n > 1; n >>= 1) {
-#pragma unroll
-        for (int i = 0; i < n / 2; ++i) {
-            const float d = mm[2 * i + 1] - mm[2 * i];
-            MM[i] = (MM[2 * i] + MM[2 * i + 1]) + d * d * half_n; mm[i] = mm[2 * i] + 0.5f * d;
-        }
-        half_n *= 2.0f;
-    }
-    mean = mm[0]; var = MM[0] * (1.0f / D_MODEL);
-}
-
-__device__ __forceinline__ float4 load_x_reduced(float* x, size_t o, const PartialSum& ps, int rows) {
-    float4 v = *(const float4*)(x + o);
-    if (ps.n > 0) {
-        float4 t[8];
-#pragma unroll
-        for (int s = 0; s < 8; ++s) if (s < ps.n) t[s] = __ldcg((const float4*)(ps.part + (size_t)s * rows * D_MODEL + o));
-        float4 acc = make_float4(0.f, 0.f, 0.f, 0.f);
-#pragma unroll
-        for (int s = 0; s < 8; ++s) if (s < ps.n) { acc.x += t[s].x; acc.y += t[s].y; acc.z += t[s].z; acc.w += t[s].w; }
-        v.x += ps.alpha * acc.x; v.y += ps.alpha * acc.y; v.z += ps.alpha * acc.z; v.w += ps.alpha * acc.w;
-        *(float4*)(x + o) = v;
-    }
-    return v;
-}
-
-__global__ void __launch_bounds__(256) layernorm_kernel(float* x, const float* __restrict__ g,
-                                                        const float* __restrict__ b, void* y, int out_type, const PartialSum ps) {
-    NSB_KERNEL_BEGIN(TR_LN)
-    __shared__ float red[16];
-    const int row = blockIdx.x, c = threadIdx.x * 4;
-    const float4 gg = *(const float4*)(g + c), bb = *(const float4*)(b + c);
-    NSB_KERNEL_WAIT()
-    const float4 v = load_x_reduced(x, (size_t)row * D_MODEL + c, ps, gridDim.x);
-    float mean, var;
-    if (out_type == OUT_F32) {
-        mean = block_sum_256(v.x + v.y + v.z + v.w, red) * (1.0f / D_MODEL);
-        const float e0 = v.x - mean, e1 = v.y - mean, e2 = v.z - mean, e3 = v.w - mean;
-        var = block_sum_256(e0 * e0 + e1 * e1 + e2 * e2 + e3 * e3, red) * (1.0f / D_MODEL);
-    } else block_mean_var_256(v.x, v.y, v.z, v.w, red, mean, var);
-    const float d0 = v.x - mean, d1 = v.y - mean, d2 = v.z - mean, d3 = v.w - mean;
-    const float rs = 1.0f / sqrtf(var + 1e-5f);
-    const size_t o = (size_t)row * D_MODEL + c;
-    const float o0 = d0 * rs * gg.x + bb.x, o1 = d1 * rs * gg.y + bb.y, o2 = d2 * rs * gg.z + bb.z, o3 = d3 * rs * gg.w + bb.w;
-    if (out_type == OUT_F32) *(float4*)((float*)y + o) = make_float4(o0, o1, o2, o3);
-    else if (out_type == OUT_F16) { __half2* p = (__half2*)((__half*)y + o); p[0] = __floats2half2_rn(o0, o1); p[1] = __floats2half2_rn(o2, o3); }
-    else { __nv_bfloat162* p = (__nv_bfloat162*)((__nv_bfloat16*)y + o); p[0] = __floats2bfloat162_rn(o0, o1); p[1] = __floats2bfloat162_rn(o2, o3); }
-    NSB_KERNEL_EPILOGUE();
-}
-
-__device__ __forceinline__ void warp_mean_var_1024(const float4 (&v)[8], float& mean, float& var) {
-    float s = 0.f;
-#pragma unroll
-    for (int j = 0; j < 8; ++j) s += (v[j].x + v[j].y) + (v[j].z + v[j].w);
-    float m = s * (1.0f / 32.0f), M2 = 0.f;
-#pragma unroll
-    for (int j = 0; j < 8; ++j) { const float a = v[j].x - m, b = v[j].y - m, c = v[j].z - m, d = v[j].w - m; M2 += (a * a + b * b) + (c * c + d * d); }
-    float half_n = 16.0f;
-#pragma unroll
-    for (int o = 1; o < 32; o <<= 1) {
-        const float mo = __shfl_xor_sync(0xffffffffu, m, o), M2o = __shfl_xor_sync(0xffffffffu, M2, o);
-        const float d = mo - m;
-        M2 = (M2 + M2o) + d * d * half_n; m = m + 0.5f * d; half_n *= 2.0f;
-    }
     mean = m; var = M2 * (1.0f / D_MODEL);
 }
-__device__ __forceinline__ void store4_out(void* y, size_t o, float4 r, int out_type) {
-    if (out_type == OUT_F32) *(float4*)((float*)y + o) = r;
-    else if (out_type == OUT_F16) { __half2* p = (__half2*)((__half*)y + o); p[0] = __floats2half2_rn(r.x, r.y); p[1] = __floats2half2_rn(r.z, r.w); }
-    else { __nv_bfloat162* p = (__nv_bfloat162*)((__nv_bfloat16*)y + o); p[0] = __floats2bfloat162_rn(r.x, r.y); p[1] = __floats2bfloat162_rn(r.z, r.w); }
-}
-
 __global__ void __launch_bounds__(256) layernorm_rows_kernel(float* x, int rows, const float* __restrict__ g1, const float* __restrict__ b1,
                                                              const float* __restrict__ g2, const float* __restrict__ b2, void* y, int out_type,
                                                              const PartialSum ps) {
@@ -184,36 +110,12 @@
                                                          void* y2, int out_type, const PartialSum ps) {
     NSB_KERNEL_BEGIN(TR_LN2)
     __shared__ float red[16];
-    const int row = blockIdx.x, c = threadIdx.x * 4;
-    const size_t o = (size_t)row * D_MODEL + c;
-    const bool one_pass = out_type != OUT_F32;
-    float4 gg = *(const float4*)(g1 + c), bb = *(const float4*)(b1 + c);
+    const int c = threadIdx.x * 4;
+    const float4 gg = *(const float4*)(g1 + c), bb = *(const float4*)(b1 + c);
     float4 gg2 = make_float4(0.f, 0.f, 0.f, 0.f), bb2 = gg2;
     if (y2 != nullptr) { gg2 = *(const float4*)(g2 + c); bb2 = *(const float4*)(b2 + c); }
     NSB_KERNEL_WAIT()
-    float4 v = load_x_reduced(x, o, ps, gridDim.x);
-    float mean, var, d0, d1, d2, d3;
-    auto stats = [&]() {
-        if (one_pass) block_mean_var_256(v.x, v.y, v.z, v.w, red, mean, var);
-        else {
-            mean = block_sum_256(v.x + v.y + v.z + v.w, red) * (1.0f / D_MODEL);
-            const float e0 = v.x - mean, e1 = v.y - mean, e2 = v.z - mean, e3 = v.w - mean;
-            var = block_sum_256(e0 * e0 + e1 * e1 + e2 * e2 + e3 * e3, red) * (1.0f / D_MODEL);
-        }
-        d0 = v.x - mean; d1 = v.y - mean; d2 = v.z - mean; d3 = v.w - mean;
-    };
-    stats();
-    float rs = 1.0f / sqrtf(var + 1e-5f);
-    v = make_float4(d0 * rs * gg.x + bb.x, d1 * rs * gg.y + bb.y, d2 * rs * gg.z + bb.z, d3 * rs * gg.w + bb.w);
-    *(float4*)(x + o) = v;
-    if (y2 == nullptr) { NSB_KERNEL_EPILOGUE(); return; }
-    stats();
-    rs = 1.0f / sqrtf(var + 1e-5f);
-    gg = gg2; bb = bb2;
-    const float o0 = d0 * rs * gg.x + bb.x, o1 = d1 * rs * gg.y + bb.y, o2 = d2 * rs * gg.z + bb.z, o3 = d3 * rs * gg.w + bb.w;
-    if (out_type == OUT_F32) *(float4*)((float*)y2 + o) = make_float4(o0, o1, o2, o3);
-    else if (out_type == OUT_F16) { __half2* p = (__half2*)((__half*)y2 + o); p[0] = __floats2half2_rn(o0, o1); p[1] = __floats2half2_rn(o2, o3); }
-    else { __nv_bfloat162* p = (__nv_bfloat162*)((__nv_bfloat16*)y2 + o); p[0] = __floats2bfloat162_rn(o0, o1); p[1] = __floats2bfloat162_rn(o2, o3); }
+    layernorm_row_256(x, blockIdx.x, gridDim.x, gg, bb, gg2, bb2, true, y2, out_type, ps, red);
     NSB_KERNEL_EPILOGUE();
 }
 void launch_layernorm2(float* x, int rows, const float* g1, const float* b1, const float* g2, const float* b2, void* y2, int out_type,
diff --git a/nemotron-speech.cpp_b200/csrc/layernorm_row.cuh b/nemotron-speech.cpp_b200/csrc/layernorm_row.cuh
--- /dev/null
+++ b/nemotron-speech.cpp_b200/csrc/layernorm_row.cuh
@@ -0,0 +1,95 @@
+#pragma once
+#include "kernels.cuh"
+
+namespace nsb {
+
+__device__ __forceinline__ float block_sum_256(float v, float* red ) {
+    v = warp_sum(v);
+    const int w = threadIdx.x >> 5, l = threadIdx.x & 31;
+    __syncthreads();
+    if (l == 0) red[w] = v;
+    __syncthreads();
+    float t = 0.f;
+#pragma unroll
+    for (int i = 0; i < 8; ++i) t += red[i];
+    return t;
+}
+
+__device__ __forceinline__ void block_mean_var_256(float v0, float v1, float v2, float v3, float* red , float& mean, float& var) {
+    float m = ((v0 + v1) + (v2 + v3)) * 0.25f;
+    float M2 = (v0 - m) * (v0 - m) + (v1 - m) * (v1 - m) + (v2 - m) * (v2 - m) + (v3 - m) * (v3 - m);
+    float half_n = 2.0f;
+#pragma unroll
+    for (int o = 1; o < 32; o <<= 1) {
+        const float mo = __shfl_xor_sync(0xffffffffu, m, o), M2o = __shfl_xor_sync(0xffffffffu, M2, o);
+        const float d = mo - m;
+        M2 = (M2 + M2o) + d * d * half_n; m = m + 0.5f * d; half_n *= 2.0f;
+    }
+    const int w = threadIdx.x >> 5, l = threadIdx.x & 31;
+    __syncthreads();
+    if (l == 0) { red[2 * w] = m; red[2 * w + 1] = M2; }
+    __syncthreads();
+    float mm[8], MM[8];
+#pragma unroll
+    for (int i = 0; i < 8; ++i) { mm[i] = red[2 * i]; MM[i] = red[2 * i + 1]; }
+#pragma unroll
+    for (int n = 8; n > 1; n >>= 1) {
+#pragma unroll
+        for (int i = 0; i < n / 2; ++i) {
+            const float d = mm[2 * i + 1] - mm[2 * i];
+            MM[i] = (MM[2 * i] + MM[2 * i + 1]) + d * d * half_n; mm[i] = mm[2 * i] + 0.5f * d;
+        }
+        half_n *= 2.0f;
+    }
+    mean = mm[0]; var = MM[0] * (1.0f / D_MODEL);
+}
+
+__device__ __forceinline__ float4 load_x_reduced(float* x, size_t o, const PartialSum& ps, int rows) {
+    float4 v = *(const float4*)(x + o);
+    if (ps.n > 0) {
+        float4 t[8];
+#pragma unroll
+        for (int s = 0; s < 8; ++s) if (s < ps.n) t[s] = __ldcg((const float4*)(ps.part + (size_t)s * rows * D_MODEL + o));
+        float4 acc = make_float4(0.f, 0.f, 0.f, 0.f);
+#pragma unroll
+        for (int s = 0; s < 8; ++s) if (s < ps.n) { acc.x += t[s].x; acc.y += t[s].y; acc.z += t[s].z; acc.w += t[s].w; }
+        v.x += ps.alpha * acc.x; v.y += ps.alpha * acc.y; v.z += ps.alpha * acc.z; v.w += ps.alpha * acc.w;
+        *(float4*)(x + o) = v;
+    }
+    return v;
+}
+
+__device__ __forceinline__ void store4_out(void* y, size_t o, float4 r, int out_type) {
+    if (out_type == OUT_F32) *(float4*)((float*)y + o) = r;
+    else if (out_type == OUT_F16) { __half2* p = (__half2*)((__half*)y + o); p[0] = __floats2half2_rn(r.x, r.y); p[1] = __floats2half2_rn(r.z, r.w); }
+    else { __nv_bfloat162* p = (__nv_bfloat162*)((__nv_bfloat16*)y + o); p[0] = __floats2bfloat162_rn(r.x, r.y); p[1] = __floats2bfloat162_rn(r.z, r.w); }
+}
+
+__device__ __forceinline__ void layernorm_row_256(float* x, int row, int rows, float4 gg, float4 bb, float4 gg2, float4 bb2, bool norm2, void* y,
+                                                  int out_type, const PartialSum& ps, float* red ) {
+    const size_t o = (size_t)row * D_MODEL + threadIdx.x * 4;
+    float4 v = load_x_reduced(x, o, ps, rows);
+    float mean, var, d0, d1, d2, d3;
+    auto stats = [&]() {
+        if (out_type != OUT_F32) block_mean_var_256(v.x, v.y, v.z, v.w, red, mean, var);
+        else {
+            mean = block_sum_256(v.x + v.y + v.z + v.w, red) * (1.0f / D_MODEL);
+            const float e0 = v.x - mean, e1 = v.y - mean, e2 = v.z - mean, e3 = v.w - mean;
+            var = block_sum_256(e0 * e0 + e1 * e1 + e2 * e2 + e3 * e3, red) * (1.0f / D_MODEL);
+        }
+        d0 = v.x - mean; d1 = v.y - mean; d2 = v.z - mean; d3 = v.w - mean;
+    };
+    stats();
+    float rs = 1.0f / sqrtf(var + 1e-5f);
+    if (norm2) {
+        v = make_float4(d0 * rs * gg.x + bb.x, d1 * rs * gg.y + bb.y, d2 * rs * gg.z + bb.z, d3 * rs * gg.w + bb.w);
+        *(float4*)(x + o) = v;
+        if (y == nullptr) return;
+        stats();
+        rs = 1.0f / sqrtf(var + 1e-5f);
+        gg = gg2; bb = bb2;
+    }
+    store4_out(y, o, make_float4(d0 * rs * gg.x + bb.x, d1 * rs * gg.y + bb.y, d2 * rs * gg.z + bb.z, d3 * rs * gg.w + bb.w), out_type);
+}
+
+}
```

Result: slower. 4702, median of 6 (-17.3%).
